# maropu/spark-data-repair-plugin

Hardware: AMD Instinct MI355X
Metric: repaired cells/sec (higher is better)
Workload: dtype f32 gradients (LightGBM's score_t), exact int64 fixed-point histogram sums, f64 scores

## Files before the change

### include/rgbm.h

```cpp
#ifndef RGBM_H_
#define RGBM_H_

#include <stddef.h>
#include <stdint.h>

#ifdef __cplusplus
extern "C" {
#endif

#define RGBM_OK 0
#define RGBM_ERR_ARG (-1)
#define RGBM_ERR_PARAM (-2)
#define RGBM_ERR_LABEL (-3)
#define RGBM_ERR_NO_DEVICE (-10)
#define RGBM_ERR_HIP (-11)
#define RGBM_ERR_NOMEM (-12)
#define RGBM_ERR_FORMAT (-20)

#define RGBM_OBJ_BINARY 0
#define RGBM_OBJ_MULTICLASS 1
#define RGBM_OBJ_REGRESSION 2

typedef struct rgbm_model rgbm_model;
typedef struct rgbm_table rgbm_table;
// ... 35 lines not shown
    int64_t level_atomics_per_row;
} rgbm_train_stats;

int rgbm_device_count(void);
int rgbm_release_cache(void);
const char* rgbm_last_error(void);
int rgbm_version(void);

int rgbm_train(const int32_t* X_colmajor, int64_t n, int32_t f, const int32_t* n_codes,
               const int32_t* y_code, int32_t n_y_codes, const double* y_value,
               const double* class_weight, const double* sample_weight,
               const rgbm_params* p, rgbm_model** out, rgbm_train_stats* stats );

int rgbm_predict(const rgbm_model* m, const int32_t* X_colmajor, int64_t n, int32_t f,
                 int32_t device_id, double* out);

int rgbm_repair_chain(const rgbm_model* const* models, int32_t T, const int32_t* target_col,
                      const int32_t* feat_cols, const int32_t* feat_off,
                      const int32_t* class_code, const int32_t* class_off,
                      int32_t* table_colmajor, int64_t n, int32_t c, int32_t device_id,
                      int32_t* out_label, double* out_prob);

int rgbm_table_create(const int32_t* codes_colmajor, int64_t n, int32_t c, const int32_t* n_codes,
                      int32_t device_id, rgbm_table** out);
int rgbm_table_set_column_kind(rgbm_table* t, int32_t col, int32_t kind);
int rgbm_table_set_column_values(rgbm_table* t, int32_t col, const double* values, int32_t n);
int rgbm_host_alloc(size_t bytes, void** out);
void rgbm_host_free(void* p);
void rgbm_table_free(rgbm_table* t);
int rgbm_table_train(const rgbm_table* t, int32_t target_col, const int32_t* feat_cols, int32_t f,
                     const double* y_value ,
                     const double* class_weight ,
                     const rgbm_params* p, rgbm_model** out, rgbm_train_stats* stats);
int rgbm_table_set_row_multiplicity(rgbm_table* t, const uint8_t* mult );
int rgbm_table_read_row_multiplicity(const rgbm_table* t, uint8_t* mult_out );
int rgbm_table_distinct_rows(const rgbm_table* t, rgbm_table** out, int64_t* n_out, int64_t* inverse_out );
int rgbm_table_distinct_view_info(const rgbm_table* t, int32_t* state, int64_t* rows, int64_t* builds);
int rgbm_distinct_view_eligible(int64_t rows, int32_t f, const rgbm_params* p, int32_t table_has_mult, int64_t min_rows);
typedef struct {
    const rgbm_table* table;
    int32_t target_col, n_features;
    const int32_t* feat_cols;
    const double* y_value;
    const double* class_weight;
    const rgbm_params* params;
    const rgbm_table* valid_table;
    int32_t* valid_label_out;
    double* valid_value_out;
} rgbm_fit_spec;
int rgbm_table_train_batch(const rgbm_fit_spec* fits, int32_t n_fits, rgbm_model** out_models , int32_t* out_status );
int rgbm_table_repair_chain(rgbm_table* t, const rgbm_model* const* models, int32_t T,
                            const int32_t* target_col, const int32_t* feat_cols, const int32_t* feat_off,
                            int64_t row_begin, int64_t n_rows, int32_t* out_label, double* out_prob);
int rgbm_table_read_column(const rgbm_table* t, int32_t col, int32_t* out );

int rgbm_table_detect_nulls(rgbm_table* t, const int32_t* cols, int32_t n_cols, int64_t* n_cells_out);
int rgbm_table_detect_cells(rgbm_table* t, const int32_t* cols, int32_t n_cols, const uint8_t* null_is_error ,
                            const int32_t* keep_lo, const int32_t* keep_hi ,
                            const uint64_t* const* flag_bits , int64_t* n_cells_out);
int rgbm_table_detect_constraint(rgbm_table* t, const int32_t* eq_cols, int32_t n_eq, int32_t iq_col,
                                 const int32_t* cell_cols, int32_t n_cell_cols,
                                 int64_t* n_rows_out , int64_t* n_cells_out);
#define RGBM_DC_EQ 0
#define RGBM_DC_IQ 1
#define RGBM_DC_LT 2
#define RGBM_DC_GT 3
typedef struct rgbm_dc_pred {
    int32_t op;
    int32_t left_col;
    int32_t right_col;
    int32_t reserved;
    const int32_t* left_rank;
    const int32_t* right_rank;
} rgbm_dc_pred;
int rgbm_table_detect_dc(rgbm_table* t, const rgbm_dc_pred* preds, int32_t n_preds, const int32_t* cell_cols, int32_t n_cell_cols,
                         int64_t max_pairs, int64_t* n_rows_out , int64_t* n_cells_out);
int rgbm_table_detect_row_bits(rgbm_table* t, const int32_t* cols, int32_t n_cols, const uint64_t* const* bits ,
                               const int32_t* cell_cols, int32_t n_cell_cols, int64_t* n_rows_out , int64_t* n_cells_out);
int rgbm_table_rows_of_cells(rgbm_table* t, const int64_t* rows, int64_t n_cells, int64_t* n_rows_out);
int rgbm_table_cells_fetch(const rgbm_table* t, int64_t* rows_out , int32_t* cols_out );
int rgbm_table_null_cells(rgbm_table* t, const int64_t* rows, const int32_t* cols, int64_t n_cells,
                          const int32_t* target_cols, int32_t n_targets);
int rgbm_table_read_cells(const rgbm_table* t, const int64_t* rows, const int32_t* cols, int64_t n_cells, int32_t* codes_out);
int rgbm_table_write_cells(rgbm_table* t, const int64_t* rows, const int32_t* cols, const int32_t* codes, int64_t n_cells);
int rgbm_table_gather_rows(const rgbm_table* t, const int64_t* rows, int64_t n_rows, rgbm_table** out);
int rgbm_table_count_codes(const rgbm_table* t, int32_t col, int64_t* counts_out ,
                           int64_t* n_null_out );
int rgbm_table_column_stats(const rgbm_table* t, const int32_t* cols, int32_t n_cols, const int32_t* const* len_lut,
                            int32_t n_bins, int64_t* stats_out, int32_t* edges_out);
int rgbm_table_create_dict(const int32_t* idx_colmajor, int64_t n, int32_t c, const int32_t* const* remap,
                           const int32_t* dict_size , int32_t device_id, rgbm_table** out);
int rgbm_table_repair_pmf(rgbm_table* t, const rgbm_model* m, int32_t target_col, const int32_t* feat_cols, int32_t f,
                          int32_t top_k, double threshold, const int32_t* cur_code, int64_t cap, int64_t* n_cells_out,
                          int64_t* rows_out , int32_t* class_out ,
                          double* prob_out , double* cur_prob_out );
int rgbm_table_repair_pmf_weighted(rgbm_table* t, const rgbm_model* m, int32_t target_col, const int32_t* feat_cols, int32_t f,
                                   int32_t top_k, double threshold, const int32_t* cur_code ,
                                   const int32_t* cost_row , const double* cost ,
                                   int64_t n_cost_rows, double weight, int32_t renormalise, int64_t cap, int64_t* n_cells_out,
                                   int64_t* rows_out , int32_t* class_out , double* prob_out ,
                                   double* cur_prob_out , double* top1_cost_out );
int rgbm_edit_distance(int32_t device_id, const int32_t* a_cp, const int64_t* a_off, int64_t n_a, const int32_t* b_cp,
                       const int64_t* b_off, int64_t n_b, int32_t* dist_out);
int rgbm_table_pair_counts(rgbm_table* t, const int32_t* pair_cols, int32_t n_pairs, const int32_t* const* luts ,
                           const int32_t* n_bins , int64_t* counts_out);
int rgbm_table_cell_domains(rgbm_table* t, int32_t target_col, const int64_t* rows, int64_t n_cells, const int32_t* pair_idx, int32_t k,
                            const int64_t* min_cnt , const uint8_t* single_ok , double beta, int64_t row_count,
                            uint8_t* weak_out, int32_t* top_out, double* top_prob_out, double* probs_out );
int rgbm_table_fd_map(const rgbm_table* t, int32_t x_col, int32_t y_col, int32_t* map_out );
int rgbm_table_rule_fill(rgbm_table* t, int32_t y_col, int32_t x_col , const int32_t* lut, int32_t n_lut, int64_t row_begin,
                         int64_t n_rows, int32_t* out_label );
int rgbm_nearest_values(int32_t device_id, const int32_t* a_cp, const int64_t* a_off, int64_t n_a, const int32_t* b_cp, const int64_t* b_off,
                        int64_t n_b, const double* cost , double threshold, int32_t* nearest_out );
int rgbm_lof_1d(int32_t device_id, const double* values , const int64_t* counts ,
                int32_t d, int32_t k , double threshold ,
                double* score_out , uint64_t* flag_bits_out , int64_t* info_out );
int rgbm_table_kmeans_assign(rgbm_table* t, const int32_t* cols, int32_t n_cols, const int64_t* code_off ,
                             int32_t k, const double* p , int64_t d_tot, const double* h ,
                             int32_t first ,
                             int64_t* counts_out , int64_t* sizes_out , int64_t* n_changed_out);
int rgbm_table_kmeans_read(const rgbm_table* t, int32_t* assign_out );
int rgbm_table_shape(const rgbm_table* t, int64_t* n_out, int32_t* c_out, int32_t* n_codes_out );

#define RGBM_COMM_ID_BYTES 128
#define RGBM_FLAG_ROW_SHARDED 1
#define RGBM_FLAG_WHOLE_TABLE 4
#define RGBM_FLAG_NO_MODEL 2
int rgbm_comm_unique_id(void* id_out );
int rgbm_comm_init(const void* id, int32_t rank, int32_t nranks, int32_t device_id);
int rgbm_comm_finalize(void);
int rgbm_comm_info(int32_t* info );
int rgbm_comm_count(int32_t* n_out );
int rgbm_comm_all_gather_sizes(const int64_t* mine, int32_t n, int64_t* all );
int rgbm_comm_all_gather_bytes(const void* send, int64_t my_bytes, int64_t block_bytes , void* recv );
int rgbm_table_repair_chain_gather(rgbm_table* t, const rgbm_model* const* models, int32_t T, const int32_t* target_col,
                                   const int32_t* feat_cols, const int32_t* feat_off, int64_t row_begin, int64_t n_rows, int64_t max_rows,
                                   int32_t* out_label, double* out_prob);
int rgbm_comm_gather_stats(int64_t* out );
int rgbm_local_group_create(int32_t nranks, int32_t device_id, void** group_out);
void rgbm_local_group_free(void* group);
int rgbm_comm_init_local(void* group, int32_t rank);

int rgbm_fusion_create(int32_t n_members, void** fusion_out);
int rgbm_fusion_join(void* fusion, int32_t member );
int rgbm_fusion_leave(int32_t failed );
int rgbm_fusion_info(void* fusion, int64_t* info );
int rgbm_fusion_free(void* fusion);

int rgbm_model_save(const rgbm_model* m, void* buf, size_t* len);
int rgbm_model_load(const void* buf, size_t len, rgbm_model** out);
void rgbm_model_free(rgbm_model* m);
int rgbm_model_info(const rgbm_model* m, int32_t* info);
int rgbm_model_predict_form(const rgbm_model* m, int32_t* out);
int rgbm_model_importance(const rgbm_model* m, int32_t type, double* out );

#ifdef __cplusplus
}
#endif
#endif
```

### spark-data-repair-plugin_amd/csrc/rgbm.hip

```cpp
#include <hip/hip_runtime.h>
#include <algorithm>
#include <atomic>
#include <condition_variable>
#include <chrono>
#include <cmath>
#include <cstdio>
#include <cstdlib>
#include <cstring>
#include <deque>
#include <map>
#include <memory>
#include <stdexcept>
#include <mutex>
#include <string>
#include <thread>
#include <vector>

#include "rgbm_host.h"
#include "rgbm_kernels.h"
#include "rgbm_level.h"
#include "rgbm_small.h"


namespace {
// ... 239 lines not shown
        const std::vector<double>* cv = (size_t)cols[f] < tab.col_values.size() ? &tab.col_values[cols[f]] : nullptr;
        find_bin(cnt.data() + cnt_off[f], ncod[f], n_train, p, ft, (cv && (int32_t)cv->size() == ncod[f] && ncod[f] > 0) ? cv->data() : nullptr);
        if ((size_t)cols[f] < tab.col_kind.size() && tab.col_kind[cols[f]] == 1) {
            const unsigned int* cf = cnt.data() + cnt_off[f];
            bool any = false;
            for (int32_t c = 0; c < ncod[f]; ++c) any |= cf[c] == 0;
            if (any) {
                ft.unseen.assign((size_t)(ncod[f] + 31) / 32, 0u);
                for (int32_t c = 0; c < ncod[f]; ++c) if (cf[c] == 0) ft.unseen[(size_t)c >> 5] |= 1u << (c & 31);
            }
        }
        fmeta[f].V = ft.V; fmeta[f].has_nan = ft.has_nan; fmeta[f].nbins = std::max(ft.V + ft.has_nan, 1); fmeta[f].hoff = totbins;
        totbins += fmeta[f].nbins;
        trivial[f] = (ft.V + ft.has_nan <= 1) || ft.V == 0;
        miss[f] = (uint8_t)(ft.has_nan ? ft.V : 0);
        lut_off[f + 1] = lut_off[f] + std::max(ncod[f], 1);
    }
    std::vector<uint8_t>& lut = h.lut; lut.assign(lut_off[F], 0);
    for (int f = 0; f < F; ++f) {
        const Feat& ft = model->feats[f];
        int b = 0;
        for (int c = 0; c < ncod[f]; ++c) { while (b < ft.V - 1 && c > ft.ub[b]) ++b; lut[lut_off[f] + c] = (uint8_t)(ft.V > 0 ? b : 0); }
    }
    const int nchunk = (F + 15) / 16; h.nchunk = nchunk;
    std::vector<ChunkMeta>& cmeta = h.cmeta; cmeta.assign(nchunk, ChunkMeta());
    size_t& lds_hist = h.lds_hist; lds_hist = 0;
    for (int ch = 0; ch < nchunk; ++ch) {
        ChunkMeta& cm = cmeta[ch]; cm.first_feat = ch * 16; cm.nfeat = std::min(16, F - ch * 16); cm.fast_slots = 0; cm.wide_bins = 0;
        for (int j = 0; j < cm.nfeat; ++j) {
            FeatMeta& m = fmeta[ch * 16 + j];
            int sh = 0; while (sh < 5 && (m.nbins << (sh + 1)) <= 256) ++sh;
            m.rep_shift = sh; m.fast_base = cm.fast_slots; m.wide_off = cm.wide_bins;
            cm.fast_slots += m.nbins << sh; cm.wide_bins += m.nbins;
        }
        lds_hist = std::max(lds_hist, (size_t)cm.fast_slots * 16);
    }

    const int nl = std::max({n_y, obj == 0 ? 2 : 1, obj == 1 ? K : 1});
    std::vector<double> tot(nl, 0.0);
    double w_max = 0.0;
    if (hls && hls->valid) { tot = hls->tot; tot.resize(nl, 0.0); w_max = hls->w_max; }
    else {
        for (int c = 0; c < n_y; ++c) {
            const double cw32 = class_weight ? (double)(float)class_weight[c] : 1.0;
            tot[c] = (double)ycnt[c] * cw32;
            if (ycnt[c]) w_max = std::max(w_max, cw32);
        }
    }
    if (!(w_max > 0.0)) w_max = 1.0;
    double sumw = 0.0;
    for (int c = 0; c < nl; ++c) sumw += tot[c];
    std::vector<double>& init = h.init; init.assign(K, 0.0);
    double ymin = 0.0, ymax = 0.0;
    const double keps = k_eps();
    if (obj == 2) {
        bool first = true; double suml = 0.0;
        for (int c = 0; c < n_y; ++c) {
            if (!ycnt[c]) continue;
            if (first) { ymin = ymax = y_value[c]; first = false; }
            ymin = std::min(ymin, y_value[c]); ymax = std::max(ymax, y_value[c]);
        }
        if (hls && hls->valid) suml = hls->suml; else for (int c = 0; c < nl; ++c) suml += tot[c] * (c < n_y ? y_value[c] : 0.0);
        init[0] = suml / sumw;
    } else if (obj == 0) {
        double pavg = tot[1] / sumw;
        if (pavg > 1.0 - keps) pavg = 1.0 - keps;
        if (pavg < keps) pavg = keps;
        init[0] = std::log(pavg / (1.0 - pavg));
    } else {
        for (int k = 0; k < K; ++k) { double pr = tot[k] / sumw; init[k] = std::log(pr > keps ? pr : keps); }
    }
    const double factor = obj == 1 ? (double)K / (double)(K - 1) : 1.0;
    double bound_g, bound_h;
    if (obj == 2) { bound_g = (ymax - ymin) * w_max; if (!(bound_g > 0.0)) bound_g = 1.0; bound_h = w_max; }
    else if (obj == 0) { bound_g = w_max; bound_h = 0.25 * w_max; }
    else { bound_g = w_max; bound_h = factor * 0.25 * w_max; }
    double wr = sumw / w_max;
    long long q_mult = 1;
    if (const char* th = std::getenv("RGBM_TEST_HOOKS")) if (std::atoi(th) != 0) if (const char* ev = std::getenv("RGBM_FX_ROWS")) {
        const double R = std::atof(ev);
        if (R > (double)n_train && R <= 4294967296.0 && n_train > 0) {
            wr *= R / (double)n_train; q_mult = ((long long)R + n_train - 1) / n_train;
            static std::atomic<bool> said{false};
            if (!said.exchange(true)) fprintf(stderr, "[rgbm] TEST HOOK active: RGBM_FX_ROWS=%s coarsens the fixed-point grid of every model trained by this process\n", ev);
        }
    }
    const int e_g = rg::fx_exponent(bound_g, wr), e_h = rg::fx_exponent(bound_h, wr);

    TrainConst& tc = h.tc; memset(&tc, 0, sizeof(tc));
    tc.sg = std::ldexp(1.0, e_g); tc.sh = std::ldexp(1.0, e_h); tc.inv_sg = std::ldexp(1.0, -e_g); tc.inv_sh = std::ldexp(1.0, -e_h);
    tc.l1 = p.lambda_l1; tc.l2 = p.lambda_l2; tc.min_gain_to_split = p.min_gain_to_split; tc.min_sum_hessian = p.min_sum_hessian_in_leaf;
    tc.learning_rate = p.learning_rate; tc.factor = factor; tc.min_data_in_leaf = p.min_data_in_leaf; tc.max_depth = p.max_depth;
    tc.num_leaves = p.num_leaves; tc.F = F; tc.K = K; tc.totbins = std::max(totbins, 1); tc.nchunk = nchunk; tc.objective = obj;
    tc.N = N; tc.n_train = n_train; tc.NG = N;
    tc.fx.c_g = 24 - rg::fx_ceil_log2(bound_g); tc.fx.c_h = 24 - rg::fx_ceil_log2(bound_h);
    tc.fx.e_g_min = e_g; tc.fx.e_h_min = e_h;
    tc.fx.e_g_max = 50 - rg::fx_ceil_log2(bound_g); tc.fx.e_h_max = 50 - rg::fx_ceil_log2(bound_h);
    tc.fx.q_mult = q_mult;
}

struct HostTrees { const int32_t *L, *feat, *theta, *dleft, *left, *right, *cnt; const double *gain, *val; const int32_t* any; };
size_t model_trees_begin(rgbm_model* model, const HostTrees& h, int NE, int K) {
    int n_iter = NE;
    for (int it = 0; it < NE; ++it) if (!h.any[it]) { n_iter = it > 0 ? it : 1; break; }
    model->n_iter = n_iter;
    const size_t nt = (size_t)n_iter * K;
    model->trees.clear(); model->trees.resize(nt);
    size_t total = 0;
    for (size_t t = 0; t < nt; ++t) total += Tree::doubles(std::max(h.L[t], 1));
    model->tree_arena.reset(new double[std::max<size_t>(total, 1)]);
    size_t off = 0;
    for (size_t t = 0; t < nt; ++t) { const int L = std::max(h.L[t], 1); model->trees[t].place(model->tree_arena.get() + off, L); off += Tree::doubles(L); }
    return nt;
}
void model_trees_fill(rgbm_model* model, const HostTrees& h, int NL, size_t t0, size_t t1) {
    for (size_t t = t0; t < t1; ++t) {
        Tree& tr = model->trees[t];
        const size_t n = (size_t)tr.L - 1, nb = t * (NL - 1), lb = t * NL;
        memcpy(tr.feat, h.feat + nb, 4 * n); memcpy(tr.theta, h.theta + nb, 4 * n); memcpy(tr.dleft, h.dleft + nb, 4 * n);
        memcpy(tr.left, h.left + nb, 4 * n); memcpy(tr.right, h.right + nb, 4 * n); memcpy(tr.gain, h.gain + nb, 8 * n);
        memcpy(tr.leaf_value, h.val + lb, 8 * (size_t)tr.L); memcpy(tr.leaf_count, h.cnt + lb, 4 * (size_t)tr.L);
    }
}
void model_from_trees(rgbm_model* model, const HostTrees& h, int NE, int K, int NL) {
    const size_t n = model_trees_begin(model, h, NE, K);
    model_trees_fill(model, h, NL, 0, n);
}

std::vector<uint8_t> make_used_masks(const rgbm_params& p, size_t NT, int F, const std::vector<uint8_t>& trivial) {
    std::vector<uint8_t> used(NT * F, 0);
    LgbRand sr((uint32_t)p.seed);
    sr.rnd16(); sr.rnd16(); sr.rnd16();
    LgbRand ff((uint32_t)sr.rnd16());
    std::vector<int> valid; for (int f = 0; f < F; ++f) if (!trivial[f]) valid.push_back(f);
    for (size_t t = 0; t < NT; ++t) {
        uint8_t* u = used.data() + t * F;
        if (p.feature_fraction < 1.0) {
            int cntf = (int)std::floor((double)valid.size() * p.feature_fraction + 0.5);
            if (cntf < 1) cntf = 1;
            for (int i : ff.sample((int)valid.size(), cntf)) u[valid[i]] = 1;
        } else for (int f : valid) u[f] = 1;
    }
    return used;
}

struct MtLaunch { int ch, slot0, nslots, route, T, G, gx, acc2, rot; };
struct LevelPassPlan {
    int root_gx = 8;
    std::vector<std::vector<MtLaunch>> mt;
    std::vector<int> mt_gx;
    size_t part_items = 0;
};

LevelPassPlan plan_level_passes(const RunSwitches& sw, const std::vector<rg::FeatMeta>& fmeta, const std::vector<rg::ChunkMeta>& cmeta,
                                long long N, int K, int max_depth, bool wm , int lds_bytes) {
    using namespace rg;
    const int nchunk = (int)cmeta.size();
    LevelPassPlan P;
    P.mt.resize(LV_MAX_DEPTH + 1); P.mt_gx.assign(LV_MAX_DEPTH + 1, 8);
    const long long ntiles = (N + LV_TILE - 1) / LV_TILE;
    {
        const long long cu_slots = 256, per = (long long)K * nchunk;
        const long long gmin = std::max<long long>(1, (N + (1ll << 22) - 1) >> 22);
        auto eff_of = [&](long long g) { const long long tot = g * per, rounds = (tot + cu_slots - 1) / cu_slots; return (double)tot / (double)(rounds * cu_slots); };
        const long long gfloor = std::max<long long>(8, (gmin + 7) / 8 * 8), gcap = std::max<long long>(gfloor, std::min<long long>(512, (ntiles + 7) / 8 * 8));
        long long g2 = gfloor; double best2 = -1.0;
        for (long long g = gfloor; g <= gcap; g += 8) {
            if (per >= 16 && (g * per < 3 * cu_slots || g * per > 5 * cu_slots)) continue;
            const double e = eff_of(g);
            if (e > best2 + 1e-9) { best2 = e; g2 = g; }
            if (e >= 0.99) break;
        }
        if (best2 < 0.0) for (long long g = gfloor; g <= gcap; g += 8) { const double e = eff_of(g); if (e > best2 + 1e-9) { best2 = e; g2 = g; } if (e >= 0.99) break; }
        if (sw.lv_blocks >= 1) g2 = (sw.lv_blocks + 7) / 8 * 8;
        P.root_gx = (int)g2;
    }
    for (int ch = 0; ch < nchunk; ++ch)
        if ((long long)lv_slots(fmeta.data() + cmeta[ch].first_feat, cmeta[ch].nfeat, 0) * 16 + LV_ROOT_FIXED > lds_bytes)
            throw std::invalid_argument("histogram of one node exceeds LDS");
    P.part_items = (size_t)K * P.root_gx;
    for (int level = 1; level < max_depth; ++level) {
        const int worst = 1 << (level - 1);
        int G_first = 1;
        bool acc2 = nchunk == 2 && sw.mt_acc2;
        if (acc2) {
            const long long nb2 = ((long long)lv_slots(fmeta.data() + cmeta[0].first_feat, cmeta[0].nfeat, 0) + lv_slots(fmeta.data() + cmeta[1].first_feat, cmeta[1].nfeat, 0)) * 16;
            if (nb2 > mt_hist_bytes(lds_bytes, MT_THREADS_ACC2, true, true, cmeta[1].nfeat > 15 || wm)) acc2 = false;
        }
        if (wm && nchunk == 2 && !acc2) throw std::invalid_argument("a two-chunk table with row multiplicities needs the one-pass level form (the multiplicity rides in the second record)");
        for (int ch = 0; ch < (acc2 ? 1 : nchunk); ++ch) {
            const FeatMeta* fm = fmeta.data() + cmeta[ch].first_feat;
            long long node_bytes = (long long)lv_slots(fm, cmeta[ch].nfeat, 0) * 16;
            if (acc2) node_bytes += (long long)lv_slots(fmeta.data() + cmeta[1].first_feat, cmeta[1].nfeat, 0) * 16;
            const int mt_thr = acc2 ? MT_THREADS_ACC2 : LV_THREADS;
            const bool li_arr = cmeta[acc2 ? 1 : ch].nfeat > 15 || wm;
            const long long hist_room = mt_hist_bytes(lds_bytes, mt_thr, acc2, acc2 , li_arr);
            long long cap = hist_room / std::max<long long>(node_bytes, 1);
            cap = std::min<long long>(cap, MT_MAX_NODES);
            if (cap < 1) throw std::invalid_argument("histogram of one node exceeds LDS");
            const int win = (int)std::min<long long>(worst, cap);
            const long long rep_target = std::max(1, sw.mt_rep);
            const long long t_nodes = std::max<long long>(win, cap / rep_target);
            int T = (int)std::max<long long>(1, std::min<long long>(std::min<long long>(t_nodes / win, MT_MAX_T), std::min<long long>(K, MT_RT_BUDGET / (2 * worst))));
            if (sw.mt_T >= 1) T = std::max(1, std::min(T, sw.mt_T));
            const bool plain1 = nchunk == 1 || acc2;
            const bool rot_full = cmeta[ch].nfeat >= 12 && (!acc2 || cmeta[1].nfeat >= 12);
            const long long rot_node_bytes = node_bytes + mt_rot_dummy(true) * 16;
            const long long cap_rot = std::min<long long>(hist_room / rot_node_bytes, MT_MAX_NODES);
            const long long T_rot = std::min<long long>(std::min<long long>(cap_rot / win, MT_MAX_T), std::min<long long>(K, MT_RT_BUDGET / (2 * worst)));
            const bool few_trees = T < sw.mt_rot_tmin && T_rot >= 2 * (long long)T;
            const bool rot = plain1 && (sw.mt_rot == 1 || (sw.mt_rot < 0 && rot_full && (cap * 2 < (long long)sw.mt_rot_copies2 * T * win || few_trees))) &&
                             (long long)T * win * rot_node_bytes <= hist_room;
            if (rot && sw.mt_T < 1) T = (int)std::max<long long>(T, T_rot);
            const int G = (K + T - 1) / T;
            if (ch == 0) G_first = G;
            for (int s0 = 0; s0 < worst; s0 += win)
                P.mt[level].push_back(MtLaunch{ch, s0, win, (ch == 0 && s0 == 0) ? 1 : 0, T, G, 0, acc2 ? 1 : 0, rot ? 1 : 0});
        }
        const long long gmin = std::max<long long>(1, (N + (1ll << 22) - 1) >> 22);
        const long long nwt = (N + MT_WT_ROWS - 1) / MT_WT_ROWS;
        const long long gx_lo = std::max<long long>(8, (gmin + 7) / 8 * 8), gx_hi = std::max<long long>(gx_lo, std::min<long long>(512, (nwt / (4 * (LV_THREADS / 64)) + 7) / 8 * 8));
        long long gx = gx_lo; double best = -1.0;
        for (long long g = gx_lo; g <= gx_hi; g += 8) {
            const long long tot = g * G_first, rounds = (tot + 255) / 256;
            const double eff = (double)tot / (double)(rounds * 256) - 0.01 * (double)rounds;
            if (eff > best + 1e-9) { best = eff; gx = g; }
            if (tot >= 256 && (double)tot / (double)(rounds * 256) >= 0.97) break;
        }
        if (sw.mt_blocks >= 1) gx = (sw.mt_blocks + 7) / 8 * 8;
        P.mt_gx[level] = (int)gx;
        for (auto& L : P.mt[level]) L.gx = (int)gx;
        P.part_items = std::max(P.part_items, (size_t)K * (size_t)gx * (size_t)worst);
    }
    return P;
}

struct JointRootPlan {
    bool on = false;
    std::vector<std::vector<int>> groups;
    std::vector<rg::FeatMeta> vfm; rg::ChunkMeta vcm;
    std::vector<rg::JointFeat> jf;
    std::vector<int16_t> binfeat;
};
JointRootPlan plan_joint_root(const std::vector<rg::FeatMeta>& fmeta, int totbins, bool wm, int lds_bytes) {
    using namespace rg;
    const int F = (int)fmeta.size();
    JointRootPlan J;
    std::vector<int> order(F); for (int f = 0; f < F; ++f) order[f] = f;
    std::stable_sort(order.begin(), order.end(), [&](int a, int b) { return fmeta[a].nbins > fmeta[b].nbins; });
    std::vector<int> prod;
    for (int f : order) {
        int best = -1;
        for (size_t g = 0; g < J.groups.size(); ++g)
            if ((long long)prod[g] * fmeta[f].nbins <= 256 && (best < 0 || prod[g] > prod[best])) best = (int)g;
        if (best < 0) { J.groups.emplace_back(); prod.push_back(1); best = (int)J.groups.size() - 1; }
        J.groups[best].push_back(f); prod[best] *= fmeta[f].nbins;
    }
    const int VF = (int)J.groups.size();
    if (VF > (wm ? 15 : 16) || VF > F - 2) return J;
    J.vfm.resize(VF); J.jf.resize(F); J.binfeat.assign(totbins, 0);
    ChunkMeta& vcm = J.vcm; vcm.first_feat = 0; vcm.nfeat = VF; vcm.fast_slots = 0; vcm.wide_bins = 0;
    for (int v = 0; v < VF; ++v) {
        FeatMeta& m = J.vfm[v]; memset(&m, 0, sizeof(m));
        m.V = prod[v]; m.has_nan = 0; m.nbins = prod[v]; m.hoff = vcm.wide_bins; m.wide_off = vcm.wide_bins;
        int sh = 0; while (sh < 5 && (m.nbins << (sh + 1)) <= 256) ++sh;
        m.rep_shift = sh; m.fast_base = vcm.fast_slots; vcm.fast_slots += m.nbins << sh; vcm.wide_bins += m.nbins;
        int stride = 1;
        for (int f : J.groups[v]) {
            JointFeat& j = J.jf[f]; memset(&j, 0, sizeof(j));
            j.voff = m.hoff; j.stride = stride; j.nbins = fmeta[f].nbins; j.nbv = prod[v]; j.hoff = fmeta[f].hoff; j.vbyte = v;
            stride *= fmeta[f].nbins;
            for (int b = 0; b < fmeta[f].nbins; ++b) J.binfeat[fmeta[f].hoff + b] = (int16_t)f;
        }
    }
    J.on = (long long)lv_slots(J.vfm.data(), VF, 0) * 16 + LV_ROOT_FIXED <= lds_bytes;
    return J;
}

#define RGBM_MT_FORMS(X) \
    X(0, rg::LV_THREADS, false, false, false)  \
    X(1, rg::LV_THREADS, false, false, false)  \
    X(1, rg::LV_THREADS, false, false, true)   \
    X(2, rg::LV_THREADS, false, false, false)  \
    X(2, rg::MT_THREADS_ACC2, true, true, false)  \
    X(2, rg::MT_THREADS_ACC2, true, true, true)
struct MtForm { int nchr, threads; bool acc2, spec, rot; };
constexpr MtForm MT_FORMS[] = {
#define RGBM_MT_FORM_ENTRY(NCHR, THR, ACC, SPEC, ROT) {NCHR, THR, ACC, SPEC, ROT},
    RGBM_MT_FORMS(RGBM_MT_FORM_ENTRY)
#undef RGBM_MT_FORM_ENTRY
};
using MtKernel = decltype(&rg::k_level_mt<1, false, true, rg::LV_THREADS, false, false, false>);
MtKernel mt_kernel(const MtForm& f, bool bag, bool route) {
#define RGBM_MT_FORM_KERNEL(NCHR, THR, ACC, SPEC, ROT) \
    if (f.nchr == NCHR && f.threads == THR && f.acc2 == ACC && f.spec == SPEC && f.rot == ROT) \
        return bag ? (route ? rg::k_level_mt<NCHR, true, true, THR, ACC, SPEC, ROT> : rg::k_level_mt<NCHR, true, false, THR, ACC, SPEC, ROT>) \
                   : (route ? rg::k_level_mt<NCHR, false, true, THR, ACC, SPEC, ROT> : rg::k_level_mt<NCHR, false, false, THR, ACC, SPEC, ROT>);
    RGBM_MT_FORMS(RGBM_MT_FORM_KERNEL)
#undef RGBM_MT_FORM_KERNEL
    throw std::logic_error("level pass: no such launch form");
}
void launch_level_mt(const MtForm& f, bool bag, bool route, dim3 grid, hipStream_t s, const uint4* rec, const float2* gh, uint8_t* node, const uint8_t* inbag,
                     const rg::LvPlan* plan, rg::HistBin* part, int32_t* count, const rg::FeatMeta* fmeta, const rg::ChunkMeta* cmeta, int32_t* err_flag,
                     const rg::FxScale* fxs, const rg::LevelConst& c) {
    hipLaunchKernelGGL(mt_kernel(f, bag, route), grid, dim3(f.threads), rg::LV_LDS_BYTES, s, rec, gh, node, inbag, plan, part, count, fmeta, cmeta, err_flag, fxs, c);
}
struct HistTimers {
    bool on; hipStream_t s;
    std::deque<rgh::Event> ev; std::vector<char> root;
    template <typename Fn> void timed(bool is_root, Fn&& fn) {
        if (!on) { fn(); return; }
        HIPCHK(hipEventRecord(ev.emplace_back().e, s));
        fn();
        HIPCHK(hipEventRecord(ev.emplace_back().e, s));
        root.push_back(is_root ? 1 : 0);
    }
};

struct LevelTrace {
    struct Rec { std::string name; int it, level; size_t off, bytes; };
    const char* dir; bool on; hipStream_t s;
    int lo = 44, hi = 44, cur_it = 0;
    std::vector<Rec> idx; size_t used = 0;
    DevBuf<unsigned char> buf;
    LevelTrace(bool level_mode, int K, hipStream_t stream) : dir(getenv("RGBM_TRACE")), s(stream) {
        on = dir && level_mode && (!getenv("RGBM_TRACE_K") || atoi(getenv("RGBM_TRACE_K")) == K);
        if (on && getenv("RGBM_TRACE_ITERS")) sscanf(getenv("RGBM_TRACE_ITERS"), "%d:%d", &lo, &hi);
    }
    void copy(const char* name, int level, const void* src, size_t bytes) {
        if (!on || cur_it < lo || cur_it > hi) return;
        if (used + bytes > buf.n) return;
        HIPCHK(hipMemcpyAsync(buf.p + used, src, bytes, hipMemcpyDeviceToDevice, s));
        idx.push_back({name, cur_it, level, used, bytes}); used += (bytes + 15) & ~(size_t)15;
    }
    void sum(const char* name, const void* src, size_t bytes) {
        if (!on || used + 16 > buf.n) return;
        HIPCHK(hipMemsetAsync(buf.p + used, 0, 8, s));
        rgh::trace_sum(src, bytes, (unsigned long long*)(buf.p + used), s);
        idx.push_back({name, cur_it, -1, used, 8}); used += 16;
    }
    void write(int target_col) {
        if (!on || !used) return;
        std::vector<unsigned char> h(used);
        HIPCHK(hipMemcpy(h.data(), buf.p, used, hipMemcpyDeviceToHost));
        char path[512];
        snprintf(path, sizeof(path), "%s/target%d.bin", dir, target_col);
        if (FILE* f = fopen(path, "wb")) { fwrite(h.data(), 1, h.size(), f); fclose(f); }
        snprintf(path, sizeof(path), "%s/target%d.idx", dir, target_col);
        if (FILE* f = fopen(path, "w")) { for (const auto& r : idx) fprintf(f, "%s %d %d %zu %zu\n", r.name.c_str(), r.it, r.level, r.off, r.bytes); fclose(f); }
    }
};

void fill_train_stats(rgbm_train_stats* stats, float total_ms, const HistTimers& timers, const HostTrees& h, const rgbm_params& p, bool level_mode, bool use_bagging,
                      int nranks , int64_t N, int64_t n_train, int F, int root_feats ,
                      int K, unsigned long long statrows) {
    const int NE = p.n_estimators, NL = p.num_leaves;
    memset(stats, 0, sizeof(*stats));
    stats->total_ms = total_ms;
    stats->hist_launches = (int64_t)timers.root.size();
    for (size_t i = 0; i < timers.root.size(); ++i) {
        float m2 = 0.f; HIPCHK(hipEventElapsedTime(&m2, timers.ev[2 * i].e, timers.ev[2 * i + 1].e));
        stats->hist_ms += m2; if (timers.root[i]) stats->root_ms += m2;
    }
    stats->trees = (int64_t)NE * K;
    const bool root_done = n_train >= (int64_t)p.min_data_in_leaf * 2;
    if (level_mode) {
        const int64_t root_rows = (root_done && !use_bagging) ? (int64_t)NE * K * n_train : 0;
        const int64_t rows_acc = (int64_t)(statrows / (unsigned long long)nranks);
        stats->hist_rows = rows_acc; stats->root_rows = root_rows / nranks;
        stats->root_atomics_per_row = 2 * (int64_t)root_feats; stats->level_atomics_per_row = 2 * (int64_t)F;
        stats->hist_bytes = rows_acc * ((int64_t)F + 8);
        return;
    }
    int64_t rows = 0, root_rows = 0;
    for (size_t t = 0; t < (size_t)NE * K; ++t) {
        const int L = h.L[t];
        const int32_t* left = h.left + t * (NL - 1); const int32_t* right = h.right + t * (NL - 1);
        if (root_done) { rows += N; root_rows += N; }
        std::vector<int64_t> fin(h.cnt + t * NL, h.cnt + t * NL + NL);
        std::vector<int64_t> nodecnt(std::max(L - 1, 1), 0);
        auto sub = [&](int ch) -> int64_t { return ch < 0 ? fin[~ch] : nodecnt[ch]; };
        for (int j = L - 2; j >= 0; --j) nodecnt[j] = sub(left[j]) + sub(right[j]);
        std::vector<int> node_depth(std::max(L - 1, 1), 0);
        for (int j = 0; j < L - 1; ++j) {
            const int lc = left[j], rc = right[j];
            if (lc >= 0) node_depth[lc] = node_depth[j] + 1;
            if (rc >= 0) node_depth[rc] = node_depth[j] + 1;
            const int64_t a = sub(lc), b = sub(rc);
            bool go = j + 2 < NL;
            if (p.max_depth > 0 && node_depth[j] + 1 >= p.max_depth) go = false;
            if (a < (int64_t)p.min_data_in_leaf * 2 && b < (int64_t)p.min_data_in_leaf * 2) go = false;
            if (go) rows += std::min(a, b);
        }
    }
    stats->hist_rows = rows; stats->root_rows = root_rows;
    stats->hist_bytes = rows * ((int64_t)F + 8) + (rows - root_rows) * 4;
}

void check_fit_args(const rgbm_table& tab, int32_t target_col, const int32_t* feat_cols, int32_t F, const double* y_value, const rgbm_params& p) {
    check_params(p);
    if (F <= 0) throw std::invalid_argument("no feature columns");
    if (target_col < 0 || target_col >= tab.c) throw std::invalid_argument("target column out of range");
    for (int f = 0; f < F; ++f) if (feat_cols[f] < 0 || feat_cols[f] >= tab.c) throw std::invalid_argument("feature column out of range");
    const int obj = p.objective, n_y = tab.n_codes[target_col];
    if (obj == 1 && n_y > p.num_class) throw std::out_of_range("target has more label codes than num_class");
    if (obj == 0 && n_y > 2) throw std::out_of_range("binary objective with more than 2 label codes");
    if (obj == 2 && !y_value) throw std::out_of_range("regression needs the y_value dictionary");
}

struct BinRecords {
    DevBuf<int32_t> cols, ncod; DevBuf<long long> cnt_off; DevBuf<unsigned int> cnt;
    DevBuf<rg::FeatMeta> fmeta; DevBuf<rg::ChunkMeta> cmeta; DevBuf<long long> lut_off; DevBuf<uint8_t> lut, miss; DevBuf<uint4> rec;
    void count_codes(const rgbm_table& tab, int32_t target_col, const int32_t* feat_cols, int32_t F, FitHost& h, hipStream_t s) {
        h.cols.assign(feat_cols, feat_cols + F); h.cols.push_back(target_col);
        h.ncod.resize(F + 1); h.cnt_off.assign(F + 2, 0);
        for (int f = 0; f <= F; ++f) { h.ncod[f] = tab.n_codes[h.cols[f]]; h.cnt_off[f + 1] = h.cnt_off[f] + std::max(h.ncod[f], 1); }
        cols.alloc(F + 1); ncod.alloc(F + 1); cnt_off.alloc(F + 2); cnt.alloc(h.cnt_off[F + 1]);
        cols.upload(h.cols.data(), F + 1, s); ncod.upload(h.ncod.data(), F + 1, s); cnt_off.upload(h.cnt_off.data(), F + 2, s); cnt.zero(s);
        const int gx = (int)std::min<int64_t>((tab.n + 255) / 256, 1024);
        hipLaunchKernelGGL(rg::k_count_codes, dim3(gx, F + 1), dim3(256), 0, s, tab.codes.p, (long long)tab.n, tab.codes.p + (long long)target_col * tab.n, cols.p, ncod.p,
                           cnt_off.p, cnt.p, tab.has_mult ? tab.mult.p : (const uint8_t*)nullptr);
    }
    void download_counts(FitHost& h, hipStream_t s) const { h.cnt.resize(cnt.n); cnt.download(h.cnt.data(), cnt.n, s); }
    void fill(const FitHost& h, long long N, hipStream_t s) {
        const int F = h.tc.F;
        fmeta.alloc(F); cmeta.alloc(h.nchunk); lut_off.alloc(F + 1); lut.alloc(h.lut.size()); miss.alloc(F);
        fmeta.upload(h.fmeta.data(), F, s); cmeta.upload(h.cmeta.data(), h.nchunk, s); lut_off.upload(h.lut_off.data(), F + 1, s);
        lut.upload(h.lut.data(), h.lut.size(), s); miss.upload(h.miss.data(), F, s);
        rec.alloc((size_t)h.nchunk * N);
    }
    void pack(const rgbm_table& t, const uint8_t* lut_, const uint8_t* miss_, uint4* out, const uint8_t* mult, hipStream_t s) const {
        hipLaunchKernelGGL(rg::k_pack_bins, dim3((unsigned)((t.n + 255) / 256)), dim3(256), 0, s, t.codes.p, (long long)t.n, 0ll, (long long)t.n, cols.p, ncod.p,
                           lut_off.p, lut_, miss_, (int)fmeta.n, (int)cmeta.n, out, mult);
    }
    void pack(const rgbm_table& tab, hipStream_t s) { pack(tab, lut.p, miss.p, rec.p, tab.has_mult ? tab.mult.p : (const uint8_t*)nullptr, s); }
};

struct BagState {
    DevBuf<unsigned int> blk, rand, bagcnt; DevBuf<int32_t> sorted_rows, oob; DevBuf<uint8_t> inbag;
    std::vector<unsigned int> seeds;
    long long off = 0, local = 0, nrb = 1;
    void order_rows(const int32_t* d_ycol, long long N, long long n_train, hipStream_t s) {
        const long long nblk = (N + 1023) / 1024;
        blk.alloc(nblk); sorted_rows.alloc(n_train); oob.alloc(n_train); inbag.alloc(N); bagcnt.alloc(2);
        hipLaunchKernelGGL(rg::k_block_count, dim3((unsigned)nblk), dim3(256), 0, s, d_ycol, N, blk.p);
        hipLaunchKernelGGL(rg::k_block_scan, dim3(1), dim3(1024), 0, s, blk.p, nblk);
        hipLaunchKernelGGL(rg::k_stable_compact, dim3((unsigned)nblk), dim3(256), 0, s, d_ycol, N, blk.p, sorted_rows.p);
    }
    void seed(const rgbm_params& p, long long bag_off, long long bag_local, hipStream_t s) {
        off = bag_off; local = bag_local;
        nrb = std::max<long long>(1, (off + local + 1023) / 1024 - off / 1024);
        LgbRand sr2((uint32_t)p.seed); sr2.rnd16();
        const int bagging_seed = sr2.rnd16();
        seeds.resize(nrb);
        for (long long b = 0; b < nrb; ++b) seeds[b] = (unsigned int)(bagging_seed + off / 1024 + b);
        rand.alloc(nrb); rand.upload(seeds.data(), nrb, s);
    }
};

struct TreeBlock {
    DevBuf<int32_t> L, feat, theta, dleft, left, right, cnt, any; DevBuf<double> gain, val;
    void alloc(size_t NT, int NL, int NE, hipStream_t s) {
        const size_t nn = NT * (size_t)(NL - 1), nl = NT * (size_t)NL;
        any.alloc(NE); any.zero(s);
        L.alloc(NT); feat.alloc(nn); theta.alloc(nn); dleft.alloc(nn); left.alloc(nn); right.alloc(nn); cnt.alloc(nl); gain.alloc(nn); val.alloc(nl);
        cnt.zero(s); val.zero(s);
    }
    rg::TreeOut out() const { return rg::TreeOut{L.p, feat.p, theta.p, dleft.p, left.p, right.p, gain.p, val.p, cnt.p}; }
    void host_layout(size_t (&off)[11]) const {
        const size_t bytes[10] = {L.n * 4, feat.n * 4, theta.n * 4, dleft.n * 4, left.n * 4, right.n * 4, cnt.n * 4, gain.n * 8, val.n * 8, any.n * 4};
        off[0] = 0;
        for (int i = 0; i < 10; ++i) off[i + 1] = off[i] + ((bytes[i] + 63) & ~(size_t)63);
    }
    size_t host_bytes() const { size_t off[11]; host_layout(off); return off[10]; }
    HostTrees download(char* base, hipStream_t s) const {
        size_t off[11]; host_layout(off);
        auto get = [&](const auto& buf, int i) { auto* h = reinterpret_cast<decltype(buf.p)>(base + off[i]); buf.download(h, buf.n, s); return h; };
        return HostTrees{get(L, 0), get(feat, 1), get(theta, 2), get(dleft, 3), get(left, 4), get(right, 5), get(cnt, 6), get(gain, 7), get(val, 8), get(any, 9)};
    }
};

struct FitState {
    const rgbm_table& tab; const rgbm_params& p; hipStream_t s; const int32_t F;
    const RunSwitches sw = read_switches();
    const int K = p.objective == 1 ? p.num_class : 1, NL = p.num_leaves, NE = p.n_estimators; const int64_t N = tab.n;
    const bool use_bagging = p.bagging_freq > 0 && p.bagging_fraction < 1.0;
    const bool level_mode = p.max_depth >= 1 && p.max_depth <= rg::LV_MAX_DEPTH && F <= 255 && sw.grower != 2;
    const bool dp = (p.reserved & RGBM_FLAG_ROW_SHARDED) != 0;
    const int32_t* d_ycol; const uint8_t* d_mult = tab.has_mult ? tab.mult.p : (const uint8_t*)nullptr;
    FitHost h; BinRecords bins;
    DevBuf<int32_t> base;
    DevBuf<unsigned int> counter;
    DevBuf<float2> gh;
    DevBuf<double> score, init;
    DevBuf<unsigned long long> fxq;
    DevBuf<rg::FxScale> fxs;
    DevBuf<unsigned long long> qpart; long long fx_parts = 0; bool fx_fused = false;
    TreeBlock trees;
    DevBuf<double> cw, yv, sw_rows; DevBuf<uint8_t> used;
    BagState bag; DevBuf<unsigned int> bagcnt_g;
    const unsigned int* n_in_ptr = nullptr;
    DevBuf<int32_t> it;
    HistTimers timers;

    FitState(const rgbm_table& tab_, int32_t target_col, int32_t F_, const rgbm_params& p_, bool timed, hipStream_t s_)
        : tab(tab_), p(p_), s(s_), F(F_), d_ycol(tab_.codes.p + (long long)target_col * tab_.n), timers{timed, s_} {}

    int grad_gx() const { return (int)std::min<long long>((N + 255) / 256, 4096); }
    bool mc_tile() const { return p.objective == 1 && K >= 16 && K <= 112; }
    bool mc_rows() const { return p.objective == 1 && K < 16; }
    void alloc_fx_parts() {
        if (sw.fx_separate || (p.objective == 1 && !mc_tile() && !mc_rows())) return;
        fx_fused = true; fx_parts = mc_tile() ? (N + 63) / 64 : (mc_rows() ? ((N + 255) / 256) * 4 : (long long)grad_gx());
        qpart.alloc((size_t)fx_parts * K * 2);
    }
    void enqueue_grad(uint8_t* node0, long long NS);
    void enqueue_bagging();
};

struct LevelGrower {
    FitState& st; hipStream_t s;
    int root_feats;
    unsigned long long statrows = 0;
    rg::LevelConst lc, lcj; LevelPassPlan passes;
    const int n_hnodes = (1 << st.p.max_depth) - 1;
    bool use_reduce = false;
    bool joint_root = false; int vtotbins = 0;
    DevBuf<rg::FeatMeta> vfmeta; DevBuf<rg::ChunkMeta> vcmeta; DevBuf<uint4> rec_j; DevBuf<rg::HistBin> part_j, red_j; DevBuf<rg::JointFeat> jf; DevBuf<int16_t> binfeat;
    DevBuf<uint8_t> node; DevBuf<rg::LvPlan> plan; DevBuf<rg::SNode> snodes; DevBuf<rg::Cand> lcand;
    DevBuf<rg::HistBin> part, lpool, part_red; DevBuf<int32_t> count, count_g, err, leafnode; DevBuf<double> ndelta; DevBuf<unsigned long long> d_statrows;
    const int score_gx = (int)std::max<long long>(1, std::min<long long>((st.N + 1023) / 1024, (2048 + st.K - 1) / st.K));
    LevelTrace trace;
    int32_t h_err = 0;

    explicit LevelGrower(FitState& st_) : st(st_), s(st_.s), root_feats(st_.F), trace(true, st_.K, st_.s) {
        using namespace rg;
        memset(&lc, 0, sizeof(lc)); memset(&lcj, 0, sizeof(lcj));
        lc.lds_bytes = LV_LDS_BYTES;
        if (st.sw.lv_lds >= 65536 && st.sw.lv_lds <= LV_LDS_BYTES) lc.lds_bytes = st.sw.lv_lds;
        lc.nchunk = st.h.nchunk; lc.K = st.K; lc.F = st.F; lc.totbins = st.h.tc.totbins;
        lc.num_leaves = st.NL; lc.max_depth = st.p.max_depth; lc.min_data_in_leaf = st.p.min_data_in_leaf; lc.N = st.N; lc.NS = (st.N + 255) & ~255ll; lc.NG = lc.NS;
        lc.sib_local = (st.dp && comm_rank() == 0) ? 1 : 0;
        lc.has_mult = st.tab.has_mult ? 1u : 0u;
        passes = plan_level_passes(st.sw, st.h.fmeta, st.h.cmeta, st.N, st.K, st.p.max_depth, st.tab.has_mult, lc.lds_bytes);
        lc.gx = passes.root_gx; lc.xcd_blocks = 1; lc.max_built = 1;
        node.alloc((size_t)st.K * lc.NS);
        HIPCHK(hipMemsetAsync(node.p, 0xFF, (size_t)st.K * lc.NS, s));
        plan.alloc(st.K); snodes.alloc((size_t)st.K * 256); lcand.alloc((size_t)st.K * 256 * st.F);
        part.alloc(passes.part_items * st.h.tc.totbins); lpool.alloc((size_t)st.K * n_hnodes * st.h.tc.totbins);
        count.alloc((size_t)st.K * 256); use_reduce = st.dp || lc.gx > 4;
        if (st.dp) count_g.alloc((size_t)st.K * 256);
        const int max_built_all = 1 << std::max(0, st.p.max_depth - 2);
        part_red.alloc((size_t)st.K * max_built_all * st.h.tc.totbins + (size_t)st.K * 128 );
        leafnode.alloc((size_t)st.K * LV_MAX_LEAVES); err.alloc(1); err.zero(s); ndelta.alloc((size_t)st.K * 256); d_statrows.alloc(1); d_statrows.zero(s);
        if (st.sw.joint_root && ((long long)st.K * st.N >= (1ll << 21) || (st.tab.has_mult && st.h.nchunk == 2))) {
            const JointRootPlan jp = plan_joint_root(st.h.fmeta, st.h.tc.totbins, st.tab.has_mult, lc.lds_bytes);
            if (jp.on) {
                const int VF = (int)jp.vfm.size();
                joint_root = true; vtotbins = jp.vcm.wide_bins;
                vfmeta.alloc(VF); vfmeta.upload(jp.vfm.data(), VF, s); vcmeta.alloc(1); vcmeta.upload(&jp.vcm, 1, s);
                jf.alloc(st.F); jf.upload(jp.jf.data(), st.F, s); binfeat.alloc(jp.binfeat.size()); binfeat.upload(jp.binfeat.data(), jp.binfeat.size(), s);
                rec_j.alloc((size_t)st.N);
                hipLaunchKernelGGL(k_pack_joint, dim3((unsigned)((st.N + 255) / 256)), dim3(256), 0, s, st.bins.rec.p, (long long)st.N, st.F, jf.p, rec_j.p, st.tab.has_mult ? st.h.nchunk - 1 : -1);
                part_j.alloc((size_t)st.K * lc.gx * vtotbins); red_j.alloc((size_t)st.K * vtotbins + (size_t)st.K * 128 );
                lcj = lc; lcj.nchunk = 1; lcj.F = VF; lcj.totbins = vtotbins; lcj.max_built = 1;
                use_reduce = true; root_feats = VF;
                HIPCHK(hipStreamSynchronize(s));
            }
        }
        if (st.tab.has_mult && st.h.nchunk == 2 && !joint_root)
            throw std::invalid_argument("a two-chunk table with row multiplicities needs the joint-bin root pass (its record carries the multiplicity); this feature set does not pack into 15 groups");
        if (st.sw.timing) {
            fprintf(stderr, "[rgbm] root: gx %d joint %d groups %d\n", lc.gx, joint_root ? 1 : 0, joint_root ? lcj.F : 0);
            for (int level = 1; level < st.p.max_depth; ++level) for (const auto& L : passes.mt[level])
                fprintf(stderr, "[rgbm] level %d launch: chunk %d slots %d..%d route %d T %d G %d gx %d acc2 %d rot %d\n", level, L.ch, L.slot0, L.slot0 + L.nslots - 1, L.route, L.T, L.G, L.gx, L.acc2, L.rot);
        }
        rgh::once_per_device(st.tab.device, rgh::ONCE_LEVEL_LDS, [] {
            HIPCHK(hipFuncSetAttribute((const void*)rg::k_level_root, hipFuncAttributeMaxDynamicSharedMemorySize, rg::LV_LDS_BYTES));
            for (const MtForm& f : MT_FORMS) for (int bag = 0; bag < 2; ++bag) for (int route = 0; route < 2; ++route)
                HIPCHK(hipFuncSetAttribute((const void*)mt_kernel(f, bag != 0, route != 0), hipFuncAttributeMaxDynamicSharedMemorySize, rg::LV_LDS_BYTES));
        });
        if (trace.on) trace.buf.alloc(((size_t)st.K * n_hnodes * st.h.tc.totbins * 16 + (size_t)st.K * 256 * (sizeof(SNode) + 4) + (size_t)st.K * sizeof(LvPlan) + 4096) * (size_t)(st.p.max_depth + 1) * (size_t)(trace.hi - trace.lo + 1) + (size_t)st.NE * 64 + 4096);
    }

    void trace_level(int level) {
        trace.copy("count", level, count.p, (size_t)st.K * 256 * 4);
        trace.copy("plan", level, plan.p, (size_t)st.K * sizeof(rg::LvPlan));
        trace.copy("snodes", level, snodes.p, (size_t)st.K * 256 * sizeof(rg::SNode));
        trace.copy("lpool", level, lpool.p, (size_t)st.K * n_hnodes * st.h.tc.totbins * 16);
    }
    std::pair<const rg::HistBin*, rg::LevelConst> exchange(bool root, int nb, const rg::LevelConst& lp) {
        using namespace rg;
        if (root && !use_reduce) return {part.p, lp};
        if (root && joint_root) {
            hipLaunchKernelGGL(k_level_reduce, dim3((vtotbins + 63) / 64, 1, st.K), dim3(256), 0, s, part_j.p, red_j.p, plan.p, count.p, 1, 1, lcj);
            hipLaunchKernelGGL(k_level_marginal, dim3((st.h.tc.totbins + 255) / 256, st.K), dim3(256), 0, s, red_j.p, part_red.p, plan.p, count.p, jf.p, binfeat.p, vtotbins, lc);
        } else
            hipLaunchKernelGGL(k_level_reduce, dim3((st.h.tc.totbins + 63) / 64, nb, st.K), dim3(256), 0, s, part.p, part_red.p, plan.p, count.p, root ? 1 : 0, nb, lp);
        if (st.dp) {
            const size_t nh = (size_t)st.K * nb * st.h.tc.totbins * 2;
            all_reduce(part_red.p, nh + (size_t)st.K * 256, AR_I64, s);
            hipLaunchKernelGGL(k_counts_unpack, dim3(st.K), dim3(256), 0, s, reinterpret_cast<const long long*>(part_red.p) + nh, count_g.p);
        }
        LevelConst r = lp; r.gx = 1; r.max_built = nb;
        return {part_red.p, r};
    }
    void enqueue_iteration(int it) {
        using namespace rg;
        const TreeOut to = st.trees.out();
        trace.cur_it = it;
        trace.sum("gh", st.gh.p, (size_t)st.K * st.h.tc.NG * 8);
        hipLaunchKernelGGL(k_level_init, dim3(st.K), dim3(64), 0, s, plan.p, snodes.p, count.p, st.n_in_ptr, (long long)st.h.n_train, st.fxq.p, st.h.tc.fx, st.fxs.p, lc);
        int32_t* cntg = st.dp ? count_g.p : count.p;
        st.timers.timed(true, [&]() {
            if (joint_root)
                hipLaunchKernelGGL(k_level_root, dim3((unsigned)lc.gx * (unsigned)st.K, 1, 1), dim3(LV_THREADS), lc.lds_bytes, s, rec_j.p, st.gh.p, node.p, plan.p, part_j.p,
                                   vfmeta.p, vcmeta.p, st.fxs.p, lcj);
            else
                hipLaunchKernelGGL(k_level_root, dim3((unsigned)lc.gx * (unsigned)st.K, 1, st.h.nchunk), dim3(LV_THREADS), lc.lds_bytes, s, st.bins.rec.p, st.gh.p, node.p, plan.p, part.p,
                                   st.bins.fmeta.p, st.bins.cmeta.p, st.fxs.p, lc);
        });
        {
            auto ex = exchange(true, 1, lc);
            hipLaunchKernelGGL(k_level_split<true>, dim3((st.F + 3) / 4, 1, st.K), dim3(256), 0, s, ex.first, lpool.p, plan.p, snodes.p, cntg, count.p, st.bins.fmeta.p,
                               st.used.p, lcand.p, d_statrows.p, st.it.p, n_hnodes, st.fxs.p, st.h.tc, ex.second);
            trace_level(0);
        }
        for (int level = 1; level < st.p.max_depth; ++level) {
            hipLaunchKernelGGL(k_level_plan, dim3(st.K), dim3(256), 0, s, plan.p, snodes.p, lcand.p, st.bins.fmeta.p, level, st.h.tc, lc);
            LevelConst lp = lc;
            lp.xcd_blocks = 0; lp.gx = passes.mt_gx[level]; lp.max_built = 1 << (level - 1);
            for (const MtLaunch& L : passes.mt[level]) {
                LevelConst l1 = lp;
                l1.mt_T = L.T; l1.mt_G = L.G; l1.mt_ch = L.ch; l1.mt_slot0 = L.slot0; l1.mt_nslots = L.nslots; l1.mt_route = L.route; l1.mt_sparse = st.sw.mt_sparse ? 1 : 0;
                const bool acc2 = L.acc2 != 0;
                const MtForm form{acc2 ? 2 : (st.h.nchunk <= 2 ? st.h.nchunk : 0), acc2 ? MT_THREADS_ACC2 : LV_THREADS, acc2, acc2, L.rot != 0};
                st.timers.timed(false, [&]() {
                    launch_level_mt(form, st.use_bagging, L.route != 0, dim3((unsigned)L.G * (unsigned)L.gx), s, st.bins.rec.p, st.gh.p, node.p, st.bag.inbag.p,
                                    plan.p, part.p, count.p, st.bins.fmeta.p, st.bins.cmeta.p, err.p, st.fxs.p, l1);
                });
            }
            auto ex = exchange(false, 1 << (level - 1), lp);
            hipLaunchKernelGGL(k_level_split<false>, dim3((st.F + 1) / 2, 1 << (level - 1), st.K), dim3(256), 0, s, ex.first, lpool.p, plan.p, snodes.p,
                               cntg, count.p, st.bins.fmeta.p, st.used.p, lcand.p, d_statrows.p, st.it.p, n_hnodes, st.fxs.p, st.h.tc, ex.second);
            trace_level(level);
        }
        hipLaunchKernelGGL(k_level_plan, dim3(st.K), dim3(256), 0, s, plan.p, snodes.p, lcand.p, st.bins.fmeta.p, st.p.max_depth, st.h.tc, lc);
        hipLaunchKernelGGL(k_level_replay, dim3(st.K), dim3(64), 0, s, plan.p, snodes.p, cntg, to, st.init.p, ndelta.p, leafnode.p, st.trees.any.p, err.p, st.it.p, st.h.tc);
        hipLaunchKernelGGL(k_level_final, dim3(score_gx, st.K), dim3(256), 0, s, st.bins.rec.p, node.p, st.bag.inbag.p, plan.p, to, ndelta.p, st.score.p, count.p, st.it.p, lc);
        if (st.dp) { hipLaunchKernelGGL(k_copy_i32, dim3(st.K), dim3(256), 0, s, count.p, count_g.p, (long long)st.K * 256); all_reduce(count_g.p, (size_t)st.K * 256, AR_I32, s); }
        hipLaunchKernelGGL(k_level_leafcount, dim3(st.K), dim3(LV_MAX_LEAVES), 0, s, plan.p, cntg, leafnode.p, to, st.it.p, st.h.tc);
        trace_level(st.p.max_depth);
        trace.sum("score", st.score.p, (size_t)st.K * st.N * 8); trace.sum("node", node.p, (size_t)st.K * lc.NS);
        hipLaunchKernelGGL(k_next_iteration, dim3(1), dim3(1), 0, s, st.it.p);
    }
    void enqueue_report() { err.download(&h_err, 1, s); d_statrows.download(&statrows, 1, s); }
    void report(int32_t target_col) {
        trace.write(target_col);
        if (h_err & 2) throw std::runtime_error("level grower: a level pass was launched with more built nodes / route entries than its workgroup tables hold (sizing violated)");
        if (h_err) throw std::runtime_error("level grower: a node outside the speculative expansion was selected (expansion bound violated)");
    }
};

struct LeafwiseGrower {
    FitState& st; hipStream_t s;
    DevBuf<int32_t> idx0, idx1, sorted; DevBuf<rg::HistBin> pool; DevBuf<rg::TreeState> state; DevBuf<rg::Leaf> leaves; DevBuf<rg::Cand> cand; DevBuf<double> upd;
    const long long root_tiles = (st.N + rg::TILE_ROWS - 1) / rg::TILE_ROWS;
    const int hist_gx = (int)std::max<long long>(1, std::min<long long>(root_tiles, (1536 + (long long)st.K * st.h.nchunk - 1) / ((long long)st.K * st.h.nchunk)));
    const int part_gx = (int)std::max<long long>(1, std::min<long long>((st.h.n_train + 1023) / 1024, (1024 + st.K - 1) / st.K));
    const int upd_gx = (int)std::max<long long>(1, std::min<long long>((st.h.n_train + 255) / 256, (2048 + st.K - 1) / st.K));
    const size_t upd_lds = (size_t)(3 * st.NL + (st.NL & 1)) * 4 + (size_t)st.NL * 8;

    explicit LeafwiseGrower(FitState& st_) : st(st_), s(st_.s) {
        idx0.alloc((size_t)st.K * st.h.n_train); idx1.alloc((size_t)st.K * st.h.n_train);
        pool.alloc((size_t)st.K * st.NL * st.h.tc.totbins);
        state.alloc(st.K); leaves.alloc((size_t)st.K * st.NL); cand.alloc((size_t)st.K * 2 * st.F);
        upd.alloc((size_t)st.K * st.NL); sorted.alloc((size_t)st.K * st.NL * 3);
        if (st.h.lds_hist > 64 * 1024)
            rgh::once_per_device(st.tab.device, rgh::ONCE_HIST_LDS, [] { HIPCHK(hipFuncSetAttribute((const void*)rg::k_hist, hipFuncAttributeMaxDynamicSharedMemorySize, 160 * 1024)); });
        if (st.h.lds_hist > 160 * 1024) throw std::invalid_argument("histogram working set exceeds LDS");
    }
    void enqueue_iteration(int it) {
        using namespace rg;
        const TreeOut to = st.trees.out();
        const uint8_t* usedp = st.used.p + (size_t)it * st.K * st.F;
        hipLaunchKernelGGL(k_init_iter, dim3(st.K), dim3(64), 0, s, state.p, leaves.p, pool.p, to, st.n_in_ptr, it, st.h.tc);
        for (int step = 0; step < st.NL - 1; ++step) {
            st.timers.timed(step == 0, [&]() {
                hipLaunchKernelGGL(k_hist, dim3(hist_gx, st.K, st.h.nchunk), dim3(256), st.h.lds_hist, s, st.bins.rec.p, st.gh.p, idx0.p, idx1.p, st.base.p,
                                   state.p, pool.p, st.bins.fmeta.p, st.bins.cmeta.p, st.fxs.p, st.h.tc);
            });
            hipLaunchKernelGGL(k_split_find, dim3((st.F + 3) / 4, st.K), dim3(256), 0, s, pool.p, state.p, leaves.p, st.bins.fmeta.p, usedp, cand.p, st.fxs.p, st.h.tc);
            hipLaunchKernelGGL(k_tree_step, dim3(st.K), dim3(64), 0, s, state.p, leaves.p, cand.p, pool.p, st.bins.fmeta.p, to, it, st.h.tc);
            hipLaunchKernelGGL(k_partition, dim3(part_gx, st.K), dim3(256), 0, s, reinterpret_cast<const uint8_t*>(st.bins.rec.p), idx0.p, idx1.p, st.base.p, state.p, st.h.tc);
            hipLaunchKernelGGL(k_finish_split, dim3(st.K), dim3(64), 0, s, state.p, leaves.p, to, it, st.h.tc);
        }
        hipLaunchKernelGGL(k_finalize_tree, dim3(st.K), dim3(64), 0, s, state.p, leaves.p, to, st.init.p, upd.p, sorted.p, st.trees.any.p, it, st.h.tc);
        hipLaunchKernelGGL(k_score_update, dim3(upd_gx, st.K), dim3(256), upd_lds, s, state.p, leaves.p, sorted.p, upd.p, idx0.p, idx1.p, st.base.p, st.score.p, st.n_in_ptr, st.h.tc);
        if (st.use_bagging)
            hipLaunchKernelGGL(k_score_update_oob, dim3(upd_gx, st.K), dim3(256), 0, s, reinterpret_cast<const uint8_t*>(st.bins.rec.p), st.bag.oob.p, st.bag.bagcnt.p,
                               state.p, to, st.bins.fmeta.p, upd.p, st.score.p, it, st.h.tc);
    }
};

void FitState::enqueue_grad(uint8_t* node0, long long NS) {
    using namespace rg;
    if (p.objective == 0) hipLaunchKernelGGL(k_grad<0>, dim3(grad_gx()), dim3(256), 0, s, score.p, d_ycol, yv.p, cw.p, sw_rows.p, bag.inbag.p, gh.p, node0, NS, qpart.p, d_mult, h.tc);
    else if (mc_rows())
        hipLaunchKernelGGL(k_grad_mc_rows<256>, dim3((unsigned)((N + 255) / 256)), dim3(256), (size_t)K * 256 * 8, s, score.p, d_ycol, cw.p, sw_rows.p, bag.inbag.p, gh.p, node0, NS, qpart.p, d_mult, h.tc);
    else if (mc_tile())
        hipLaunchKernelGGL(k_grad_mc, dim3((unsigned)((N + 63) / 64)), dim3(256), (size_t)(K * 64 + 320) * 8, s, score.p, d_ycol, cw.p, sw_rows.p, bag.inbag.p, gh.p, node0, NS, qpart.p, d_mult, h.tc);
    else if (p.objective == 1) hipLaunchKernelGGL(k_grad<1>, dim3(grad_gx()), dim3(256), 0, s, score.p, d_ycol, yv.p, cw.p, sw_rows.p, bag.inbag.p, gh.p, node0, NS, (unsigned long long*)nullptr, d_mult, h.tc);
    else hipLaunchKernelGGL(k_grad<2>, dim3(grad_gx()), dim3(256), 0, s, score.p, d_ycol, yv.p, cw.p, sw_rows.p, bag.inbag.p, gh.p, node0, NS, qpart.p, d_mult, h.tc);
    if (fx_fused) {
        const long long total = fx_parts * K * 2;
        const unsigned gx = (unsigned)std::max<long long>(1, std::min<long long>(256, (total + 8191) / 8192));
        hipLaunchKernelGGL(k_fx_reduce, dim3(gx), dim3(256), (size_t)K * 2 * 8, s, qpart.p, fx_parts, 2 * K, fxq.p);
    } else {
        const unsigned gx = (unsigned)std::max<long long>(1, std::min<long long>(128, (N + 4095) / 4096));
        hipLaunchKernelGGL(k_fx_measure, dim3(gx, K), dim3(256), 0, s, gh.p, (long long)N, (long long)h.tc.NG, h.tc.fx, fxq.p, d_mult);
    }
    if (dp) all_reduce(fxq.p, (size_t)K * 2, AR_I64, s);
    if (!level_mode) hipLaunchKernelGGL(k_fx_scale, dim3(1), dim3(256), 0, s, fxq.p, K, h.tc.fx, fxs.p);
}
void FitState::enqueue_bagging() {
    using namespace rg;
    hipLaunchKernelGGL(k_bagging, dim3((unsigned)((bag.nrb + 63) / 64)), dim3(64), 0, s, bag.rand.p, bag.local, p.bagging_fraction, bag.sorted_rows.p, bag.inbag.p, bag.bagcnt.p,
                       bag.off, (long long)h.n_train);
    hipLaunchKernelGGL(k_bag_lists, dim3((unsigned)((std::max<long long>(bag.local, 1) + 255) / 256)), dim3(256), 0, s, bag.sorted_rows.p, bag.local, bag.inbag.p, base.p, bag.oob.p, bag.bagcnt.p);
    if (dp) {
        hipLaunchKernelGGL(k_copy_i32, dim3(1), dim3(256), 0, s, reinterpret_cast<const int32_t*>(bag.bagcnt.p), reinterpret_cast<int32_t*>(bagcnt_g.p), 2ll);
        all_reduce(bagcnt_g.p, 2, AR_U32, s);
    }
}

rgbm_model* train_core(const rgbm_table& tab, int32_t target_col, const int32_t* feat_cols, int32_t F,
                       const double* y_value, const double* class_weight, const double* sample_weight_host,
                       const HostLabelStats* hls, const rgbm_params& p, rgbm_train_stats* stats, bool view_stats = false) {
    using namespace rg;
    check_fit_args(tab, target_col, feat_cols, F, y_value, p);
    if (F > 65535) throw std::invalid_argument("more than 65535 feature columns");
    StreamGuard sg_; hipStream_t s = sg_.s;
    rgh::Event ev_begin, ev_end;
    HIPCHK(hipEventRecord(ev_begin.e, s));

    FitState st(tab, target_col, F, p, stats != nullptr, s);
    auto now = []() { return std::chrono::duration<double, std::milli>(std::chrono::steady_clock::now().time_since_epoch()).count(); };
    const double t_start = now();
    st.bins.count_codes(tab, target_col, feat_cols, F, st.h, s);
    if (st.dp) {
        if (comm_kind() == 0) throw std::invalid_argument("row-sharded training requested but this thread has no communicator (rgbm_comm_init)");
        all_reduce(st.bins.cnt.p, st.bins.cnt.n, AR_U32, s);
    }
    st.bins.download_counts(st.h, s);
    if (st.dp) stream_sync_watchdog(s); else HIPCHK(hipStreamSynchronize(s));
    fit_setup(tab, y_value, class_weight, hls, p, F, st.h);
    if (p.objective == 2) y_value = st.h.yv32.data();
    const int n_y = st.h.ncod[F];

    const double t_bins = now();
    st.bins.fill(st.h, st.N, s);
    if (tab.has_mult && (!st.level_mode || st.h.nchunk > 2 || (F % 16) == 0 || sample_weight_host || st.use_bagging))
        throw std::invalid_argument("a table with row multiplicities trains with the level grower (1 <= max_depth <= 7), at most 32 features of which the last 16-feature "
                                    "chunk holds at most 15, without bagging and without per-row weights");
    st.bins.pack(tab, s);
    if (st.dp && (!st.level_mode || sample_weight_host))
        throw std::invalid_argument("row-sharded training supports the level grower (1 <= max_depth <= 7) without per-row weights");
    st.counter.alloc(1); st.counter.zero(s);
    if (!st.level_mode || st.use_bagging) {
        st.base.alloc(st.h.n_train);
        hipLaunchKernelGGL(k_iota_train, dim3((unsigned)((st.N + 255) / 256)), dim3(256), 0, s, st.d_ycol, (long long)st.N, st.base.p, st.counter.p);
    }
    if (st.level_mode) st.h.tc.NG = (st.N + 255) & ~255ll;
    st.gh.alloc((size_t)st.K * st.h.tc.NG); st.gh.zero(s);
    st.score.alloc((size_t)st.K * st.N); st.init.alloc(st.K);
    st.init.upload(st.h.init.data(), st.K, s);
    st.fxq.alloc((size_t)st.K * 2); st.fxq.zero(s);
    st.fxs.alloc(st.K);
    hipLaunchKernelGGL(k_init_score, dim3((unsigned)((st.N + 255) / 256)), dim3(256), 0, s, st.score.p, (long long)st.N, st.K, st.init.p);
    const size_t NT = (size_t)st.NE * st.K;
    st.trees.alloc(NT, st.NL, st.NE, s);
    std::unique_ptr<LevelGrower> lg; std::unique_ptr<LeafwiseGrower> lw;
    if (st.level_mode) lg.reset(new LevelGrower(st)); else lw.reset(new LeafwiseGrower(st));
    if (class_weight) { st.cw.alloc(n_y); st.cw.upload(class_weight, n_y, s); }
    if (y_value) { st.yv.alloc(n_y); st.yv.upload(y_value, n_y, s); }
    if (sample_weight_host) { st.sw_rows.alloc(st.N); st.sw_rows.upload(sample_weight_host, st.N, s); }

// ... 884 lines not shown
        HIPCHK(hipMemcpy(table, codes.p, (size_t)n * c * sizeof(int32_t), hipMemcpyDeviceToHost));
        return RGBM_OK;
    });
}

RGBM_EXPORT int rgbm_table_set_row_multiplicity(rgbm_table* t, const uint8_t* mult) {
    if (!t) return fail(RGBM_ERR_ARG, "rgbm_table_set_row_multiplicity: bad argument");
    return guarded([&]() {
        use_device(t->device);
        rgh::ViewWrite view_wr(t);
        if (!mult) { t->has_mult = false; t->mult_total = 0; return RGBM_OK; }
        int64_t tot = 0;
        for (int64_t i = 0; i < t->n; ++i) { if (mult[i] == 0) throw std::invalid_argument("rgbm_table_set_row_multiplicity: a multiplicity of 0"); tot += mult[i]; }
        if (tot >= (1ll << 31) - 4096) throw std::invalid_argument("rgbm_table_set_row_multiplicity: the expanded table has more than 2^31 rows");
        StreamGuard sg;
        t->mult.alloc((size_t)t->n);
        t->mult.upload(mult, (size_t)t->n, sg.s);
        HIPCHK(hipStreamSynchronize(sg.s));
        t->has_mult = true; t->mult_total = tot;
        return RGBM_OK;
    });
}

RGBM_EXPORT int rgbm_table_repair_chain(rgbm_table* t, const rgbm_model* const* models, int32_t T, const int32_t* target_col,
                                        const int32_t* feat_cols, const int32_t* feat_off, int64_t row_begin, int64_t n_rows,
                                        int32_t* out_label, double* out_prob) {
    if (!t || !models || T < 0 || !target_col || !feat_cols || !feat_off || row_begin < 0 || n_rows < 0 || row_begin + n_rows > t->n)
        return fail(RGBM_ERR_ARG, "rgbm_table_repair_chain: bad argument");
    if (n_rows == 0 || T == 0) return RGBM_OK;
    return guarded([&]() {
        use_device(t->device);
        rgh::ViewWrite view_wr(t);
        StreamGuard sg;
        return chain_device(const_cast<rgbm_model* const*>(models), T, target_col, feat_cols, feat_off, nullptr, nullptr, t->codes.p, t->n, row_begin, n_rows,
                            t->device, sg.s, out_label, out_prob);
    });
}

RGBM_EXPORT int rgbm_model_save(const rgbm_model* m, void* buf, size_t* len) {
    if (!m || !len) return fail(RGBM_ERR_ARG, "rgbm_model_save: bad argument");
    return guarded([&]() {
        const size_t need = serialised_size(*m);
        if (!buf) { *len = need; return RGBM_OK; }
        if (*len < need) { *len = need; return fail(RGBM_ERR_ARG, "rgbm_model_save: buffer too small"); }
        serialise_into(*m, (uint8_t*)buf); *len = need;
        return RGBM_OK;
    });
}

RGBM_EXPORT int rgbm_model_load(const void* buf, size_t len, rgbm_model** out) {
    if (!buf || !out) return fail(RGBM_ERR_ARG, "rgbm_model_load: bad argument");
    return guarded([&]() {
        const uint8_t* p = (const uint8_t*)buf; const uint8_t* end = p + len;
        auto need = [&](size_t n) { if ((size_t)(end - p) < n) throw std::length_error("truncated model"); };
        try {
            need(28); int32_t hdr[7]; memcpy(hdr, p, 28); p += 28;
            if (hdr[0] != 0x4D424752 || (hdr[1] != 1 && hdr[1] != 2)) return fail(RGBM_ERR_FORMAT, "rgbm_model_load: bad magic/version");
            std::unique_ptr<rgbm_model> m(new rgbm_model());
            m->objective = hdr[2]; m->num_class = hdr[3]; m->K = hdr[4]; m->n_iter = hdr[5]; m->F = hdr[6];
            if (m->F < 0 || m->K < 1 || m->n_iter < 0 || m->F > 65535) return fail(RGBM_ERR_FORMAT, "rgbm_model_load: bad header");
            if (m->objective < 0 || m->objective > 2 || m->num_class < 1) return fail(RGBM_ERR_FORMAT, "rgbm_model_load: bad objective / num_class");
            if (m->objective == 1 ? m->K != m->num_class : m->K != 1) return fail(RGBM_ERR_FORMAT, "rgbm_model_load: class-tree count does not match the objective");
            if (m->objective == 0 && m->num_class != 2) return fail(RGBM_ERR_FORMAT, "rgbm_model_load: binary model with num_class != 2");
            if ((unsigned long long)m->n_iter * (unsigned long long)m->K > (unsigned long long)(end - p) / 16ull) return fail(RGBM_ERR_FORMAT, "rgbm_model_load: tree count exceeds the buffer");
            m->feats.resize(m->F);
            for (Feat& f : m->feats) {
                need(12); int32_t h3[3]; memcpy(h3, p, 12); p += 12;
                f.n_codes = h3[0]; f.V = h3[1]; f.has_nan = h3[2];
                if (f.V < 0 || f.V > 255) return fail(RGBM_ERR_FORMAT, "rgbm_model_load: bad bin count");
                need(4 * (size_t)f.V); f.ub.resize(f.V); memcpy(f.ub.data(), p, 4 * (size_t)f.V); p += 4 * (size_t)f.V;
                if (hdr[1] == 2) {
                    need(4); int32_t nw; memcpy(&nw, p, 4); p += 4;
                    if (nw < 0 || (nw != 0 && (f.n_codes < 0 || nw != (f.n_codes + 31) / 32))) return fail(RGBM_ERR_FORMAT, "rgbm_model_load: bad unseen-category bitmap");
                    need(4 * (size_t)nw); f.unseen.resize(nw); memcpy(f.unseen.data(), p, 4 * (size_t)nw); p += 4 * (size_t)nw;
                }
            }
            m->trees.resize((size_t)m->n_iter * m->K);
            std::vector<uint8_t> refs;
            for (Tree& t : m->trees) {
                int32_t L_; need(4); memcpy(&L_, p, 4); p += 4;
                if (L_ < 1 || L_ > 32767) return fail(RGBM_ERR_FORMAT, "rgbm_model_load: bad leaf count");
                const size_t n = (size_t)L_ - 1;
                need(n * 28 + (size_t)L_ * 12);
                t.alloc(L_);
                auto rd32 = [&](int32_t* v, size_t k) { memcpy(v, p, 4 * k); p += 4 * k; };
                auto rd64 = [&](double* v, size_t k) { memcpy(v, p, 8 * k); p += 8 * k; };
                rd32(t.feat, n); rd32(t.theta, n); rd32(t.dleft, n); rd32(t.left, n); rd32(t.right, n); rd64(t.gain, n);
                rd64(t.leaf_value, t.L); rd32(t.leaf_count, t.L);
                for (size_t j = 0; j < n; ++j) {
                    if (t.feat[j] < 0 || t.feat[j] >= m->F) return fail(RGBM_ERR_FORMAT, "rgbm_model_load: node feature out of range");
                    if (t.theta[j] < -1 || t.theta[j] > 254) return fail(RGBM_ERR_FORMAT, "rgbm_model_load: node threshold out of range");
                    auto okc = [&](int ch) { return ch < 0 ? (~ch) < t.L : ch < (int)n && ch > (int)j; };
                    if (!okc(t.left[j]) || !okc(t.right[j])) return fail(RGBM_ERR_FORMAT, "rgbm_model_load: bad child link");
                }
                refs.assign(n + (size_t)t.L, 0);
                bool tree_ok = true;
                for (size_t j = 0; j < n; ++j)
                    for (int ch : {t.left[j], t.right[j]}) if (++refs[ch < 0 ? n + (size_t)(~ch) : (size_t)ch] > 1) tree_ok = false;
                for (size_t j = 1; j < refs.size(); ++j) if (refs[j] != 1) tree_ok = false;
                if (!tree_ok) return fail(RGBM_ERR_FORMAT, "rgbm_model_load: child links do not form a tree");
            }
            *out = m.release();
            return RGBM_OK;
        } catch (const std::length_error&) { return fail(RGBM_ERR_FORMAT, "rgbm_model_load: truncated buffer"); }
    });
}

RGBM_EXPORT int rgbm_table_repair_chain_gather(rgbm_table* t, const rgbm_model* const* models, int32_t T, const int32_t* target_col,
                                               const int32_t* feat_cols, const int32_t* feat_off, int64_t row_begin, int64_t n_rows, int64_t max_rows,
                                               int32_t* out_label, double* out_prob) {
    if (!t || !models || T < 1 || !target_col || !feat_cols || !feat_off || row_begin < 0 || n_rows < 0 || row_begin + n_rows > t->n || max_rows < n_rows || max_rows < 1 || !out_label || !out_prob)
        return fail(RGBM_ERR_ARG, "rgbm_table_repair_chain_gather: bad argument");
    return guarded([&]() {
        use_device(t->device);
        rgh::ViewWrite view_wr(t);
        const int nr = std::max(1, comm_nranks());
        StreamGuard sg; hipStream_t s = sg.s;
        const size_t blk = (size_t)T * (size_t)max_rows;
        DevBuf<int32_t> d_lab(blk), d_lab_all(blk * (size_t)nr); DevBuf<double> d_prob(blk), d_prob_all(blk * (size_t)nr);
        d_lab.zero(s); d_prob.zero(s);
        if (n_rows > 0)
            chain_device(const_cast<rgbm_model* const*>(models), T, target_col, feat_cols, feat_off, nullptr, nullptr, t->codes.p, t->n, row_begin, n_rows,
                         t->device, s, nullptr, nullptr, d_lab.p, d_prob.p, (long long)max_rows);
        const auto t0 = std::chrono::steady_clock::now();
        all_gather_on(d_lab.p, d_lab_all.p, blk * sizeof(int32_t), s);
        all_gather_on(d_prob.p, d_prob_all.p, blk * sizeof(double), s);
        HIPCHK(hipMemcpyAsync(out_label, d_lab_all.p, blk * (size_t)nr * sizeof(int32_t), hipMemcpyDeviceToHost, s));
        HIPCHK(hipMemcpyAsync(out_prob, d_prob_all.p, blk * (size_t)nr * sizeof(double), hipMemcpyDeviceToHost, s));
        stream_sync_watchdog(s);
        rgh::GatherStats& G = rgh::gather_stats();
        G.bytes += (long long)(blk * (size_t)nr * 12); G.calls += 2;
        G.ns += std::chrono::duration_cast<std::chrono::nanoseconds>(std::chrono::steady_clock::now() - t0).count();
        return RGBM_OK;
    });
}

RGBM_EXPORT void rgbm_model_free(rgbm_model* m) { delete m; }

RGBM_EXPORT int rgbm_model_info(const rgbm_model* m, int32_t* info) {
    if (!m || !info) return fail(RGBM_ERR_ARG, "rgbm_model_info: bad argument");
    info[0] = m->objective; info[1] = m->num_class; info[2] = m->K; info[3] = m->n_iter; info[4] = m->F;
    return RGBM_OK;
}

RGBM_EXPORT int rgbm_model_predict_form(const rgbm_model* m, int32_t* out) {
    if (!m || !out) return fail(RGBM_ERR_ARG, "rgbm_model_predict_form: bad argument");
    return guarded([&]() {
        const PredictForm pf = predict_form(m);
        out[0] = pf.form; out[1] = pf.mw; out[2] = pf.tw; out[3] = pf.tb; out[4] = (int32_t)pf.lds;
        return RGBM_OK;
    });
}

RGBM_EXPORT int rgbm_model_importance(const rgbm_model* m, int32_t type, double* out) {
    if (!m || !out) return fail(RGBM_ERR_ARG, "rgbm_model_importance: bad argument");
    for (int f = 0; f < m->F; ++f) out[f] = 0.0;
    for (const Tree& t : m->trees) for (int j = 0; j < t.L - 1; ++j) out[t.feat[j]] += type == 0 ? 1.0 : t.gain[j];
    return RGBM_OK;
}

}
```

### spark-data-repair-plugin_amd/csrc/rgbm_level.h

```cpp
#pragma once
#include "rgbm_kernels.h"

namespace rg {

constexpr int LV_INACTIVE = 255;
constexpr int LV_MAX_EXP = 64;
constexpr int LV_MAX_BUILT = 32;
constexpr int LV_CNT_REP = 16;
constexpr int LV_THREADS = 1024;
constexpr int LV_TILE = 2 * LV_THREADS;
constexpr int LV_LDS_TOTAL = 160 * 1024;
constexpr int LV_LDS_BYTES = LV_LDS_TOTAL;
constexpr int LV_MAX_DEPTH = 7;
constexpr int LV_MAX_LEAVES = 128;

constexpr int MT_MAX_T = 64;
constexpr int MT_MAX_NODES = 128;
constexpr int MT_RT_BUDGET = 256;
constexpr int MT_MAX_RT = MT_RT_BUDGET + MT_MAX_T;
constexpr int MT_WT_ROWS = 256;
constexpr int MT_RING_PLAIN = 128;
constexpr int MT_RING_SPEC = 128;
__host__ __device__ constexpr int mt_ring(bool spec) { return spec ? MT_RING_SPEC : MT_RING_PLAIN; }
constexpr int MT_CNT_REP = 4;

constexpr int MT_THREADS_ACC2 = 768;
#ifndef MT_CONSUMERS_N
#define MT_CONSUMERS_N 4
#endif
constexpr int MT_CONSUMERS = MT_CONSUMERS_N;

struct SNode {
    long long Gq, Hq;
    double pmin;
    int32_t count, depth, parent, is_left;
    int32_t left, right;
    int32_t best_feature, searched;
    int32_t hslot, pad;
    Cand best;
};

struct LvPlan {
    int32_t n_nodes, lvl_first, lvl_end, n_exp, n_built, live_rows , pad1, pad2, pad3, done, error, child_first, n_hslots, pad4;
    long long n_in;
    uint8_t exp[LV_MAX_EXP];
    uint8_t built_is_left[LV_MAX_EXP];
    uint32_t route0[256];
    uint32_t route1[256];
};

struct LevelConst {
    int32_t gx;
    int32_t max_built;
    int32_t nchunk, K, F, totbins, num_leaves, max_depth, min_data_in_leaf, lds_bytes;
    int32_t sib_local;
    int32_t xcd_blocks;
    int32_t mt_T, mt_G, mt_ch, mt_slot0, mt_nslots, mt_route;
    int32_t mt_sparse;
    uint32_t has_mult;
    long long N, NS, NG;
};

__device__ __forceinline__ uint32_t rec_byte(const uint4& r, int j) {
    uint32_t w = (j < 8) ? ((j < 4) ? r.x : r.y) : ((j < 12) ? r.z : r.w);
    return (w >> (8 * (j & 3))) & 0xFFu;
}

constexpr int LV_MAX_Q = 11;
__host__ __device__ inline int lv_shift(int nbins, int q) {
    int l = 0; while ((1 << l) < nbins) ++l;
    int s = q - l;
    return s < 0 ? 0 : (s > 5 ? 5 : s);
}

__host__ __device__ inline int lv_slots(const FeatMeta* fm, int nfeat, int q) {
    int t = 0;
    for (int j = 0; j < nfeat; ++j) t += fm[j].nbins << lv_shift(fm[j].nbins, q);
    return t;
}

__host__ __device__ constexpr int mt_rot_dummy(bool rot) { return rot ? 4 : 0; }
__host__ __device__ inline int mt_shift(int nbins, int q, bool rot) { return rot ? (q < 0 ? 0 : (q > 2 ? 2 : q)) : lv_shift(nbins, q); }
__host__ __device__ inline int mt_slots(const FeatMeta* fm, int nfeat, int q, bool rot) {
    int t = 0;
    for (int j = 0; j < nfeat; ++j) t += fm[j].nbins << mt_shift(fm[j].nbins, q, rot);
    return t;
}
__host__ __device__ constexpr int mt_max_q(bool rot) { return rot ? 2 : LV_MAX_Q; }

constexpr int LV_ROOT_FIXED = 256;
#if !defined(MT_SPARSE_DIV_N)
#define MT_SPARSE_DIV_N 16
#endif
constexpr long long MT_SPARSE_DIV = MT_SPARSE_DIV_N;
__host__ __device__ constexpr long long mt_fixed_bytes(int threads, bool acc2, bool spec = false, bool li = true ) {
    return ((!acc2 && !spec) ? (long long)MT_MAX_T * 8  : 0) + (long long)MT_MAX_T * 32 + MT_MAX_NODES + 16 + 512 + 256 + (long long)(MT_MAX_T + 2) * 8 + (long long)MT_MAX_RT * 8 + (long long)MT_MAX_NODES * MT_CNT_REP * 4 + (long long)MT_MAX_NODES * 8 +
           (long long)(threads / 64 - (spec ? MT_CONSUMERS : 0)) * mt_ring(spec) * ((acc2 ? 32 : 16) + 8 + (li ? 2 : 0)) + 256;
}
__host__ __device__ constexpr long long mt_hd(int threads, bool acc2, bool spec) { return ((LV_LDS_TOTAL - mt_fixed_bytes(threads, acc2, spec, false)) / 2) & ~15ll; }
__host__ __device__ constexpr long long mt_hist_bytes(long long lds_bytes, int threads, bool acc2, bool spec, bool li) {
    const long long fixed = mt_fixed_bytes(threads, acc2, spec, li), hd = mt_hd(threads, acc2, spec);
    const long long room_h = (long long)LV_LDS_TOTAL - fixed - hd;
    const long long x = hd < room_h ? hd : room_h;
    const long long a = lds_bytes - fixed;
    return a < 2 * x ? a : 2 * x;
}

__global__ __launch_bounds__(64) void k_level_init(LvPlan* __restrict__ plan, SNode* __restrict__ nodes, int32_t* __restrict__ count,
                                                   const unsigned int* __restrict__ n_in_ptr, long long n_train,
                                                   unsigned long long* __restrict__ Q, FxGrid fx, FxScale* __restrict__ fxs, LevelConst c) {
    const int k = blockIdx.x, lane = lane_id();
    if (lane == 0) {
        const int e_g = fx_tree_exponent(Q[2 * k], fx.q_mult, fx.c_g, fx.e_g_min, fx.e_g_max);
        const int e_h = fx_tree_exponent(Q[2 * k + 1], fx.q_mult, fx.c_h, fx.e_h_min, fx.e_h_max);
        FxScale f; f.sg = fx_pow2(e_g); f.sh = fx_pow2(e_h); f.inv_sg = fx_pow2(-e_g); f.inv_sh = fx_pow2(-e_h);
        fxs[k] = f;
        Q[2 * k] = 0ull; Q[2 * k + 1] = 0ull;
    }
    LvPlan* pp = &plan[k];
    const long long n_in = n_in_ptr ? (long long)n_in_ptr[0] : n_train;
    for (int i = lane; i < 256; i += 64) { pp->route0[i] = 0; pp->route1[i] = 0xFFFFFFFFu; count[(long long)k * 256 + i] = 0; }
    if (lane == 0) {
        pp->n_nodes = 1; pp->lvl_first = 0; pp->lvl_end = 1; pp->n_exp = 0; pp->n_built = 1;
        pp->error = 0; pp->child_first = 1; pp->n_hslots = 1; pp->n_in = n_in;
        pp->done = (n_in < (long long)c.min_data_in_leaf * 2) ? 1 : 0;
        SNode r; memset(&r, 0, sizeof(r));
        r.count = (int)n_in; r.depth = 0; r.parent = -1; r.left = -1; r.right = -1; r.best_feature = -1; r.searched = 0; r.hslot = 0;
        r.best.gain = -INFINITY; r.pmin = -INFINITY;
        nodes[(long long)k * 256] = r;
    }
}

__global__ __launch_bounds__(LV_THREADS, 1) void k_level_root(const uint4* __restrict__ rec, const float2* __restrict__ gh, const uint8_t* __restrict__ node,
                                                              const LvPlan* __restrict__ plan, HistBin* __restrict__ part,
                                                              const FeatMeta* __restrict__ fmeta, const ChunkMeta* __restrict__ cmeta,
                                                              const FxScale* __restrict__ fxs , LevelConst c) {
    extern __shared__ __attribute__((aligned(16))) unsigned char smem[];
    int k, bx, nbx;
    if (c.xcd_blocks) { const unsigned id = blockIdx.x, r = id >> 3; k = (int)(r % (unsigned)c.K); bx = (int)(r / (unsigned)c.K) * 8 + (int)(id & 7u); nbx = c.gx; }
    else { k = blockIdx.y; bx = blockIdx.x; nbx = gridDim.x; }
    const int ch = blockIdx.z;
    if (plan[k].done) return;
    const double sg_k = fxs[k].sg, sh_k = fxs[k].sh;
    const ChunkMeta cm = cmeta[ch];
    const FeatMeta* fm = fmeta + cm.first_feat;
    const int tid = threadIdx.x, lane = tid & 63, nfeat = cm.nfeat;
    int s = LV_MAX_Q;
    while (s > 0 && (long long)lv_slots(fm, nfeat, s) * 16 + LV_ROOT_FIXED > c.lds_bytes) --s;
    int sh[16], fbase[16], spn = 0;
#pragma unroll
    for (int j = 0; j < 16; ++j) {
        if (j < nfeat) { sh[j] = lv_shift(fm[j].nbins, s); fbase[j] = spn; spn += fm[j].nbins << sh[j]; }
        else { sh[j] = 0; fbase[j] = 0; }
    }
    unsigned long long* hist_g = reinterpret_cast<unsigned long long*>(smem);
    unsigned long long* hist_h = hist_g + spn;
    for (int i = tid; i < 2 * spn; i += LV_THREADS) hist_g[i] = 0ull;
    int cj[16], sh3[16];
#pragma unroll
    for (int j = 0; j < 16; ++j) { sh3[j] = sh[j] + 3; cj[j] = (fbase[j] + (lane & ((1 << sh[j]) - 1))) * 8; }
    const int hdelta = spn;
    __syncthreads();

    const long long N = c.N;
    const uint8_t* node_in = node + (long long)k * c.NS;
    const uint4* recc = rec + (long long)ch * N;
    const float2* ghk = gh + (long long)k * c.NG;
    const long long ntiles_all = (N + LV_TILE - 1) / LV_TILE;
    const long long tbeg = c.xcd_blocks ? ntiles_all * bx / nbx : bx;
    const long long ntiles = c.xcd_blocks ? ntiles_all * (bx + 1) / nbx : ntiles_all;
    const long long tstep = c.xcd_blocks ? 1 : nbx;

    constexpr int RPT = LV_TILE / LV_THREADS;
    int cur_n[RPT], nxt_n[RPT]; uint4 cur_r[RPT], nxt_r[RPT]; float2 cur_g[RPT], nxt_g[RPT];
    auto fetch = [&](long long t, int (&fn)[RPT], uint4 (&fr)[RPT], float2 (&fg)[RPT]) __attribute__((always_inline)) {
        const bool tv = t < ntiles;
        const long long pb = tv ? t * LV_TILE : 0;
        const long long left_rows = N - pb;
        const unsigned lim = (unsigned)(left_rows < LV_TILE ? left_rows : LV_TILE) - 1u;
#pragma unroll
        for (int q = 0; q < RPT; ++q) {
            const unsigned o = (unsigned)(q * LV_THREADS + tid);
            const unsigned oc = o < lim ? o : lim;
            typedef float v2f __attribute__((ext_vector_type(2)));
            const int nv = (int)__builtin_nontemporal_load(node_in + pb + oc);
            fr[q] = (recc + pb)[oc];
            const v2f gv = __builtin_nontemporal_load(reinterpret_cast<const v2f*>(ghk + pb + oc));
            fg[q] = make_float2(gv.x, gv.y);
            fn[q] = (tv && o <= lim) ? nv : LV_INACTIVE;
        }
    };
    auto accumulate = [&](bool on, const uint4& r, const float2& g) __attribute__((always_inline)) {
        if (on && (g.x != 0.0f || g.y != 0.0f)) {
            unsigned long long gq = (unsigned long long)fx_from_f32(g.x, sg_k), hq = (unsigned long long)fx_from_f32(g.y, sh_k);
            if (c.has_mult) { const unsigned long long m = r.w >> 24; gq *= m; hq *= m; }
            unsigned char* hb = reinterpret_cast<unsigned char*>(hist_g);
            const uint32_t w[4] = {r.x, r.y, r.z, r.w};
#define LV_ATOM(j) { const uint32_t code_ = (w[(j) >> 2] >> (8 * ((j) & 3))) & 0xFFu; \
                     unsigned long long* p_ = reinterpret_cast<unsigned long long*>(hb + cj[j] + (int)(code_ << sh3[j])); \
                     atomicAdd(p_, gq); atomicAdd(p_ + hdelta, hq); }
#pragma unroll
            for (int j = 0; j < 16; ++j) if (j < nfeat) LV_ATOM(j);
#undef LV_ATOM
        }
    };
    long long t = tbeg;
    fetch(t, cur_n, cur_r, cur_g);
    while (t < ntiles) {
        fetch(t + tstep, nxt_n, nxt_r, nxt_g);
#pragma unroll
        for (int q = 0; q < RPT; ++q) accumulate(cur_n[q] != LV_INACTIVE, cur_r[q], cur_g[q]);
        t += tstep; if (t >= ntiles) break;
        fetch(t + tstep, cur_n, cur_r, cur_g);
#pragma unroll
        for (int q = 0; q < RPT; ++q) accumulate(nxt_n[q] != LV_INACTIVE, nxt_r[q], nxt_g[q]);
        t += tstep;
    }
    __syncthreads();
    HistBin* dst = part + (((long long)k * c.gx + bx) * c.max_built) * c.totbins;
    for (int j = 0; j < nfeat; ++j) {
        const int shj = lv_shift(fm[j].nbins, s);
        int fb = 0;
        for (int q = 0; q < j; ++q) fb += fm[q].nbins << lv_shift(fm[q].nbins, s);
        for (int b = tid; b < fm[j].nbins; b += LV_THREADS) {
            long long tg = 0, th = 0;
            const unsigned long long* sg_ = hist_g + fb + (b << shj); const unsigned long long* sh_ = hist_h + fb + (b << shj);
            for (int r2 = 0; r2 < (1 << shj); ++r2) { tg += (long long)sg_[r2]; th += (long long)sh_[r2]; }
            HistBin o; o.g = tg; o.h = th;
            dst[fm[j].hoff + b] = o;
        }
    }
}

struct MtTree { int32_t base, nlev, rt_off, slot0, nb, live, child_first, k; };

template <int NCHR , bool BAG,
          bool ROUTE ,
          int THREADS , bool ACC2 ,
          bool SPEC ,
          bool ROTP = false >
__global__ __launch_bounds__(THREADS, 1) void k_level_mt(const uint4* __restrict__ rec, const float2* __restrict__ gh, uint8_t* __restrict__ node ,
                                                         const uint8_t* __restrict__ inbag, const LvPlan* __restrict__ plan, HistBin* __restrict__ part,
                                                         int32_t* __restrict__ count, const FeatMeta* __restrict__ fmeta, const ChunkMeta* __restrict__ cmeta,
                                                         int32_t* __restrict__ err_flag,
                                                         const FxScale* __restrict__ fxs , LevelConst c) {
    static_assert(!ACC2 || NCHR == 2, "a two-chunk pass keeps both records in registers");
    static_assert(ACC2 == SPEC && THREADS == (ACC2 ? MT_THREADS_ACC2 : LV_THREADS) && (!ROTP || NCHR == 1 || ACC2) && (NCHR == 0 || NCHR == 1 || NCHR == 2),
                  "k_level_mt: not one of the six launch forms");
    constexpr int WAVES = THREADS / 64;
    constexpr int NCONS = SPEC ? MT_CONSUMERS : 0, NPROD = WAVES - NCONS;
    constexpr int NACC = ACC2 ? 2 : 1;
    constexpr int NRINGS = SPEC ? NPROD : WAVES;
    constexpr int MT_RING = mt_ring(SPEC);
    constexpr bool ROT = ROTP;
    constexpr bool SPARSE = (NCHR == 1) && !ACC2 && !SPEC;
    extern __shared__ __attribute__((aligned(16))) unsigned char smem[];
    const unsigned id = blockIdx.x;
    const int xl = (int)(id & 7u), bslot = (int)(id >> 3);
    const int grp = bslot % c.mt_G, rb = (bslot / c.mt_G) * 8 + xl;
    const int k0 = grp * c.mt_T;
    const int nk = (c.K - k0) < c.mt_T ? (c.K - k0) : c.mt_T;
    const int tid = threadIdx.x, lane = tid & 63, wave = tid >> 6;
    const int ch = ACC2 ? 0 : c.mt_ch;
    constexpr bool route = ROUTE;
    const ChunkMeta cm = cmeta[ch];
    const ChunkMeta cm1 = cmeta[ACC2 ? 1 : ch];
    const FeatMeta* fm = fmeta + cm.first_feat;
    const FeatMeta* fm1 = fmeta + cm1.first_feat;
    const int nfeat = cm.nfeat, nfeat1 = ACC2 ? cm1.nfeat : 0;
    const int wb = cm.wide_bins + (ACC2 ? cm1.wide_bins : 0);
    const bool li_in_rec = (ACC2 ? nfeat1 : nfeat) <= 15 && !c.has_mult;

    MtTree* ti = reinterpret_cast<MtTree*>(smem);
    uint8_t* nd_tree = smem + MT_MAX_T * 32;
    int32_t* scal = reinterpret_cast<int32_t*>(nd_tree + MT_MAX_NODES);
    int32_t* ftab = scal + 4;
    uint32_t* rsync = reinterpret_cast<uint32_t*>(ftab + 128);
#define RS_LOAD(i) __hip_atomic_load(rsync + (i), __ATOMIC_RELAXED, __HIP_MEMORY_SCOPE_WORKGROUP)
#define RS_STORE(i, v) __hip_atomic_store(rsync + (i), (uint32_t)(v), __ATOMIC_RELAXED, __HIP_MEMORY_SCOPE_WORKGROUP)
    uint2* tpk = reinterpret_cast<uint2*>(ftab + 128 + 64);
    uint2* rt = tpk + MT_MAX_T + 2;
    int32_t* cnt = reinterpret_cast<int32_t*>(rt + MT_MAX_RT);
    uint2* nd_sc = reinterpret_cast<uint2*>(cnt + MT_MAX_NODES * MT_CNT_REP);
    uint4* ring_rec_all = reinterpret_cast<uint4*>(nd_sc + MT_MAX_NODES);
    uint4* ring_rec1_all = ring_rec_all + (ACC2 ? NRINGS * MT_RING : 0);
    uint2* ring_gh_all = reinterpret_cast<uint2*>(ring_rec1_all + NRINGS * MT_RING);
    uint16_t* ring_li_all = reinterpret_cast<uint16_t*>(ring_gh_all + NRINGS * MT_RING);
    size_t off = reinterpret_cast<unsigned char*>(ring_li_all + (li_in_rec ? 0 : NRINGS * MT_RING)) - smem;
    off = (off + 15) & ~(size_t)15;
    unsigned long long* xmask = reinterpret_cast<unsigned long long*>(smem + off);
    if (!ACC2 && !SPEC) off += (size_t)MT_MAX_T * 8;
    unsigned long long* hist_g = reinterpret_cast<unsigned long long*>(smem + off);
    constexpr int MT_HD = (int)mt_hd(THREADS, ACC2, SPEC);
    const long long avail = mt_hist_bytes(c.lds_bytes, THREADS, ACC2, SPEC, !li_in_rec);
    if (tid == 0 && ((long long)off > mt_fixed_bytes(THREADS, ACC2, SPEC, !li_in_rec) || (long long)off + MT_HD + avail / 2 > (long long)LV_LDS_TOTAL)) atomicOr(err_flag, 2);

    if (tid < 64) {
        MtTree t; t.base = 0; t.nlev = 0; t.nb = 0; t.live = 0; t.child_first = 0; t.k = k0 + lane; t.slot0 = 0; t.rt_off = 0;
        if (lane < nk) {
            const LvPlan* pp = &plan[k0 + lane];
            const bool live = !pp->done && pp->n_exp > 0;
            t.live = live ? 1 : 0;
            t.child_first = pp->child_first;
            t.base = live ? (route ? (int)pp->exp[0] : pp->child_first) : 0;
            t.nlev = live ? (route ? pp->child_first - (int)pp->exp[0] : 2 * pp->n_exp) : 0;
            int nb = live ? pp->n_built - c.mt_slot0 : 0;
            if (nb > c.mt_nslots) nb = c.mt_nslots;
            t.nb = nb < 0 ? 0 : nb;
        }
        bool sparse_t = false;
        if (SPARSE && lane < nk && t.live && t.nlev <= 64) {
            const LvPlan* pp = &plan[k0 + lane];
            const long long lr = route ? (long long)pp->live_rows : 0ll;
            sparse_t = route && lr * MT_SPARSE_DIV < pp->n_in && c.mt_sparse != 0;
        }
        const int ntab = lane < nk ? (route ? (t.live ? t.child_first : 0) : t.nlev) + 1 : 0;
        int inc_nb = t.nb, inc_rt = ntab;
#pragma unroll
        for (int o = 1; o < 64; o <<= 1) { const int a = __shfl_up(inc_nb, o), b2 = __shfl_up(inc_rt, o); if (lane >= o) { inc_nb += a; inc_rt += b2; } }
        t.slot0 = inc_nb - t.nb; t.rt_off = inc_rt - ntab;
        const int total = __shfl(inc_nb, 63), rt_total = __shfl(inc_rt, 63);
        const unsigned long long livem = __ballot(t.live != 0);
        const bool ok = total <= MT_MAX_NODES && rt_total <= MT_MAX_RT;
        if (!ok) { t.live = 0; t.nb = 0; t.nlev = 0; if (lane == 0) atomicOr(err_flag, 2); }
        const bool dead_t = lane < nk && (!t.live || (!route && t.nb == 0));
        const unsigned long long dmask = __ballot(lane < nk && !sparse_t && !dead_t), smask = __ballot(lane < nk && sparse_t && !dead_t), zmask = __ballot(dead_t);
        const int nkd_ = __popcll(dmask), nks_ = __popcll(smask);
        const unsigned long long below = (1ull << lane) - 1ull;
        const int pos = lane >= nk ? lane : (dead_t ? nkd_ + nks_ + __popcll(zmask & below) : (sparse_t ? nkd_ + __popcll(smask & below) : __popcll(dmask & below)));
        if (lane < nk) ti[pos] = t;
        tpk[pos] = make_uint2((uint32_t)t.base | (uint32_t)t.nlev << 8 | (uint32_t)(ntab > 0 ? ntab - 1 : 0) << 17 | (t.live && lane < nk ? 1u << 31 : 0u), (uint32_t)t.rt_off | (uint32_t)t.k << 16);
        if (lane < 2) tpk[64 + lane] = make_uint2(0u, 0u);
        if (SPARSE) xmask[lane] = 0ull;
        if (lane == 0) {
            int s = mt_max_q(ROT);
            const int tot = ok ? total : 0;
            while (s > 0 && (long long)tot * (mt_slots(fm, nfeat, s, ROT) + (ACC2 ? mt_slots(fm1, nfeat1, s, ROT) : 0) + mt_rot_dummy(ROT)) * 16 > avail) --s;
            const int spn0 = mt_slots(fm, nfeat, s, ROT) + (ACC2 ? mt_slots(fm1, nfeat1, s, ROT) : 0) + mt_rot_dummy(ROT);
            if ((long long)tot * spn0 * 16 > avail) atomicOr(err_flag, 2);
            scal[0] = tot; scal[1] = s; scal[2] = spn0; scal[3] = ((ok && livem != 0ull) ? 1 : 0) | nkd_ << 8 | (nkd_ + nks_) << 16;
        }
    }
    __syncthreads();
    if (!(scal[3] & 1)) return;
    const int total = __builtin_amdgcn_readfirstlane(scal[0]), s = __builtin_amdgcn_readfirstlane(scal[1]), spn = __builtin_amdgcn_readfirstlane(scal[2]);
    if (!route && total == 0) return;
    const int nkd = __builtin_amdgcn_readfirstlane((scal[3] >> 8) & 0xFF), nke = __builtin_amdgcn_readfirstlane((scal[3] >> 16) & 0xFF);
    for (int kk = 0; kk < nk; ++kk) {
        const MtTree t = ti[kk];
        const LvPlan* pp = &plan[t.k];
        const int ntab_k = (route ? (t.live ? t.child_first : 0) : t.nlev) + 1;
        for (int i = tid; i < ntab_k; i += THREADS) {
            const int n = route ? i : t.base + i;
            uint2 e;
            if (route) {
                const bool cur = i < ntab_k - 1 && n >= t.base;
                const uint32_t w0 = cur ? pp->route0[n] : 0u; const uint32_t w1 = cur ? pp->route1[n] : 0u;
                if (w0 & (1u << 24)) {
                    const int ls = (int)((w1 >> 16) & 0xFFu) - c.mt_slot0, rs = (int)(w1 >> 24) - c.mt_slot0;
                    const bool lb = ((w1 >> 16) & 0xFFu) != 0xFFu && ls >= 0 && ls < t.nb, rbb = (w1 >> 24) != 0xFFu && rs >= 0 && rs < t.nb;
                    const uint32_t theta1 = (w0 >> 8) & 0xFFu, nanbin = (w0 >> 16) & 0xFFu, dleft = (w0 >> 25) & 1u;
                    uint32_t offb, thr;
                    if (nanbin != 255u && dleft) { offb = nanbin; thr = (theta1 - 1u - nanbin) & 0xFFu; }
                    else if (theta1 == 0u) { offb = 255u; thr = 0u; }
                    else { offb = 0u; thr = theta1 - 1u; }
                    const uint32_t f = w0 & 0xFFu;
                    e = make_uint2((NCHR == 0 ? f : (f & 7u) | ((f >> 4) & 1u) << 30 | ((f >> 3) & 1u) << 31) | thr << 8 | offb << 16 | 1u << 24,
                                   (w1 & 0xFFu) | (lb ? (uint32_t)(t.slot0 + ls) : 0xFFu) << 8 | ((w1 >> 8) & 0xFFu) << 16 | (rbb ? (uint32_t)(t.slot0 + rs) : 0xFFu) << 24);
                    if (SPARSE && kk >= nkd && kk < nke && n - t.base < 64) atomicOr(&xmask[kk], 1ull << (n - t.base));
                } else {
                    const uint32_t self = i < ntab_k - 1 ? (uint32_t)n : (uint32_t)LV_INACTIVE;
                    e = make_uint2(0u, self | 0xFF00u | self << 16 | 0xFF000000u);
                }
            } else {
                const int ei = i >> 1, ls = ei - c.mt_slot0;
                const bool mine = i < ntab_k - 1 && (pp->built_is_left[ei] ? 0 : 1) == (i & 1) && ls >= 0 && ls < t.nb;
                e = make_uint2(mine ? 1u : 0u, mine ? (uint32_t)(t.slot0 + ls) : 0xFFu);
            }
            rt[t.rt_off + i] = e;
        }
        const uint2 sc_k = make_uint2((uint32_t)__double2hiint(fxs[t.k].sg), (uint32_t)__double2hiint(fxs[t.k].sh));
        for (int i = tid; i < t.nb; i += THREADS) { nd_tree[t.slot0 + i] = (uint8_t)kk; nd_sc[t.slot0 + i] = sc_k; }
    }
    for (int i = tid; i < total * MT_CNT_REP; i += THREADS) cnt[i] = 0;
    if (tid < 48) rsync[tid] = 0u;
    unsigned long long* hist_h = hist_g + MT_HD / 8;
    for (int i = tid; i < total * spn; i += THREADS) { hist_g[i] = 0ull; hist_h[i] = 0ull; }
    unsigned long long sh3p[NACC];
    int cj[NACC][16];
    {
        int o = 0;
#pragma unroll
        for (int a = 0; a < NACC; ++a) {
            const FeatMeta* fa = a == 0 ? fm : fm1;
            const int na = a == 0 ? nfeat : nfeat1;
            unsigned long long pk = 0ull;
#pragma unroll
            for (int j = 0; j < 16; ++j) {
                int shj = 0, fb = 0;
                if (j < na) { shj = mt_shift(fa[j].nbins, s, ROT); fb = o; o += fa[j].nbins << shj; }
                pk |= (unsigned long long)(shj + 3) << (4 * j); cj[a][j] = (fb + (lane & ((1 << shj) - 1))) * 8;
                if (tid == 0) {
                    const int q = a * 16 + j;
                    const int wide = (a == 0 ? 0 : cm.wide_bins) + (j < na ? fa[j].wide_off : 0);
                    ftab[q] = j < na ? wide : 0x7FFFFFFF; ftab[32 + q] = fb; ftab[64 + q] = shj; ftab[96 + q] = j < na ? fa[j].hoff - wide : 0;
                }
            }
            sh3p[a] = (unsigned long long)(unsigned)__builtin_amdgcn_readfirstlane((int)(unsigned)pk) |
                      (unsigned long long)(unsigned)__builtin_amdgcn_readfirstlane((int)(unsigned)(pk >> 32)) << 32;
        }
    }
    constexpr int hdelta = MT_HD / 8;
    __syncthreads();
    uint32_t rmask[NACC][4];
    const int rot_sh = mt_shift(1, s, ROT) + 3;
    if (ROT) {
        const int r16 = lane & 15, c4 = lane >> 4;
        const int spn_valid = spn - mt_rot_dummy(ROT);
#pragma unroll
        for (int a = 0; a < NACC; ++a) {
            const int na = a == 0 ? nfeat : nfeat1;
#pragma unroll
            for (int w = 0; w < 4; ++w) rmask[a][w] = 0u;
#pragma unroll
            for (int j = 0; j < 16; ++j) {
                const int f = (j + r16) & 15;
                const bool fv = f < na;
                cj[a][j] = fv ? (ftab[32 + a * 16 + f] + (c4 & ((1 << (rot_sh - 3)) - 1))) * 8 : (spn_valid + c4) * 8;
                rmask[a][j >> 2] |= fv ? (0xFFu << (8 * (j & 3))) : 0u;
            }
        }
    }

    const int my_ring = __builtin_amdgcn_readfirstlane(wave < NRINGS ? wave : 0);
    uint4* ring_rec = ring_rec_all + my_ring * MT_RING;
    uint4* ring_rec1 = ring_rec1_all + my_ring * MT_RING;
    uint2* ring_gh = ring_gh_all + my_ring * MT_RING;
    uint16_t* ring_li = ring_li_all + my_ring * MT_RING;
    int r_head = 0, r_cnt = 0;
    const unsigned long long lane_lt = (1ull << lane) - 1ull;
    const unsigned spn8 = (unsigned)spn * 8u;
    const uint2 tpk_v = tpk[lane];
    auto tree_entry = [&](int kk) __attribute__((always_inline)) -> uint2 {
        const int kc = kk < 64 ? kk : 63;
        const uint32_t x = (uint32_t)__builtin_amdgcn_readlane((int)tpk_v.x, kc), y = (uint32_t)__builtin_amdgcn_readlane((int)tpk_v.y, kc);
        return kk < nkd ? make_uint2(x, y) : make_uint2(0u, 0u);
    };

    auto run_batch_of = [&](int rid, int head, int nb) __attribute__((always_inline)) {
        __builtin_amdgcn_fence(__ATOMIC_RELEASE, "wavefront");
        const bool on = lane < nb;
        const int pos = rid * MT_RING + ((head + lane) & (MT_RING - 1));
        const uint4 r = ring_rec_all[pos]; const uint2 g = ring_gh_all[pos];
        uint4 r1 = make_uint4(0, 0, 0, 0);
        if (ACC2) r1 = ring_rec1_all[pos];
        unsigned li;
        if (li_in_rec) li = (ACC2 ? r1.w : r.w) >> 24; else li = ring_li_all[pos];
        unsigned long long shp[NACC];
#pragma unroll
        for (int a = 0; a < NACC; ++a) { shp[a] = sh3p[a]; asm volatile("" : "+s"(shp[a])); }
        if (on) {
            const uint2 sc = nd_sc[li];
            unsigned long long gq = (unsigned long long)fx_from_f32(__uint_as_float(g.x), __hiloint2double((int)sc.x, 0)),
                               hq = (unsigned long long)fx_from_f32(__uint_as_float(g.y), __hiloint2double((int)sc.y, 0));
            int mrow = 1;
            if (c.has_mult) { mrow = (int)((ACC2 ? r1.w : r.w) >> 24); gq *= (unsigned long long)mrow; hq *= (unsigned long long)mrow; }
            if (ch == 0) atomicAdd(&cnt[li * MT_CNT_REP + (lane & (MT_CNT_REP - 1))], mrow);
            unsigned char* hb = reinterpret_cast<unsigned char*>(hist_g) + li * spn8;
            uint32_t w[4] = {r.x, r.y, r.z, r.w};
            uint32_t w1[4] = {r1.x, r1.y, r1.z, r1.w};
            if (ROT) {
                auto rot16 = [&](uint32_t (&x)[4], const uint32_t (&mk)[4]) __attribute__((always_inline)) {
                    const bool d1 = (lane & 4) != 0, d2 = (lane & 8) != 0;
                    const uint32_t a0 = d1 ? x[1] : x[0], a1 = d1 ? x[2] : x[1], a2 = d1 ? x[3] : x[2], a3 = d1 ? x[0] : x[3];
                    const uint32_t b0 = d2 ? a2 : a0, b1 = d2 ? a3 : a1, b2 = d2 ? a0 : a2, b3 = d2 ? a1 : a3;
                    const uint32_t sb = (uint32_t)(lane & 3);
                    x[0] = __builtin_amdgcn_alignbyte(b1, b0, sb) & mk[0]; x[1] = __builtin_amdgcn_alignbyte(b2, b1, sb) & mk[1];
                    x[2] = __builtin_amdgcn_alignbyte(b3, b2, sb) & mk[2]; x[3] = __builtin_amdgcn_alignbyte(b0, b3, sb) & mk[3];
                };
                rot16(w, rmask[0]);
                if (ACC2) rot16(w1, rmask[NACC - 1]);
            }
#if defined(MT_DBL_ATOM)
#define MT_ATOMIC_ADD(p, v) { atomicAdd(p, (v) - 1ull); atomicAdd(p, 1ull); }
#else
#define MT_ATOMIC_ADD(p, v) atomicAdd(p, v)
#endif
#define MT_ATOM(A, W, j) { unsigned long long* p_ = reinterpret_cast<unsigned long long*>(hb + cj[A][j] + (int)(((W[(j) >> 2] >> (8 * ((j) & 3))) & 0xFFu) << (ROT ? rot_sh : (int)((shp[A] >> (4 * (j))) & 15ull)))); \
                           MT_ATOMIC_ADD(p_, gq); MT_ATOMIC_ADD(p_ + hdelta, hq); }
            if (ROT) {
                MT_ATOM(0, w, 0); MT_ATOM(0, w, 1); MT_ATOM(0, w, 2); MT_ATOM(0, w, 3); MT_ATOM(0, w, 4); MT_ATOM(0, w, 5); MT_ATOM(0, w, 6); MT_ATOM(0, w, 7);
                MT_ATOM(0, w, 8); MT_ATOM(0, w, 9); MT_ATOM(0, w, 10); MT_ATOM(0, w, 11); MT_ATOM(0, w, 12); MT_ATOM(0, w, 13); MT_ATOM(0, w, 14); MT_ATOM(0, w, 15);
                if (ACC2) {
                    MT_ATOM(NACC - 1, w1, 0); MT_ATOM(NACC - 1, w1, 1); MT_ATOM(NACC - 1, w1, 2); MT_ATOM(NACC - 1, w1, 3); MT_ATOM(NACC - 1, w1, 4); MT_ATOM(NACC - 1, w1, 5);
                    MT_ATOM(NACC - 1, w1, 6); MT_ATOM(NACC - 1, w1, 7); MT_ATOM(NACC - 1, w1, 8); MT_ATOM(NACC - 1, w1, 9); MT_ATOM(NACC - 1, w1, 10); MT_ATOM(NACC - 1, w1, 11);
                    MT_ATOM(NACC - 1, w1, 12); MT_ATOM(NACC - 1, w1, 13); MT_ATOM(NACC - 1, w1, 14); MT_ATOM(NACC - 1, w1, 15);
                }
            } else
            if (nfeat >= 15) {
                MT_ATOM(0, w, 0); MT_ATOM(0, w, 1); MT_ATOM(0, w, 2); MT_ATOM(0, w, 3); MT_ATOM(0, w, 4); MT_ATOM(0, w, 5); MT_ATOM(0, w, 6); MT_ATOM(0, w, 7);
                MT_ATOM(0, w, 8); MT_ATOM(0, w, 9); MT_ATOM(0, w, 10); MT_ATOM(0, w, 11); MT_ATOM(0, w, 12); MT_ATOM(0, w, 13); MT_ATOM(0, w, 14);
                if (nfeat == 16) MT_ATOM(0, w, 15);
            } else {
#pragma unroll
                for (int j = 0; j < 14; ++j) if (j < nfeat) MT_ATOM(0, w, j);
            }
            if (!ROT && ACC2) {
                if (nfeat1 >= 15) {
                    MT_ATOM(NACC - 1, w1, 0); MT_ATOM(NACC - 1, w1, 1); MT_ATOM(NACC - 1, w1, 2); MT_ATOM(NACC - 1, w1, 3); MT_ATOM(NACC - 1, w1, 4); MT_ATOM(NACC - 1, w1, 5);
                    MT_ATOM(NACC - 1, w1, 6); MT_ATOM(NACC - 1, w1, 7); MT_ATOM(NACC - 1, w1, 8); MT_ATOM(NACC - 1, w1, 9); MT_ATOM(NACC - 1, w1, 10); MT_ATOM(NACC - 1, w1, 11);
                    MT_ATOM(NACC - 1, w1, 12); MT_ATOM(NACC - 1, w1, 13); MT_ATOM(NACC - 1, w1, 14);
                    if (nfeat1 == 16) MT_ATOM(NACC - 1, w1, 15);
                } else {
#pragma unroll
                    for (int j = 0; j < 14; ++j) if (j < nfeat1) MT_ATOM(NACC - 1, w1, j);
                }
            }
#undef MT_ATOM
#undef MT_ATOMIC_ADD
        }
    };
    auto run_batch = [&](int nb) __attribute__((always_inline)) {
        run_batch_of(wave, r_head, nb);
        r_head = (r_head + nb) & (MT_RING - 1); r_cnt -= nb;
    };

    if (SPEC && wave >= NPROD) {
        const int cw = wave - NPROD;
        constexpr int NR = SPEC ? (NPROD + MT_CONSUMERS - 1) / MT_CONSUMERS : 1;
        uint32_t head[NR];
#pragma unroll
        for (int i = 0; i < NR; ++i) head[i] = 0u;
        for (;;) {
            bool any = false, all_done = true;
#pragma unroll
            for (int i = 0; i < NR; ++i) {
                const int rid = cw + i * MT_CONSUMERS;
                if (rid >= NPROD) continue;
                const uint32_t done = (uint32_t)__builtin_amdgcn_readfirstlane((int)RS_LOAD(32 + rid));
                asm volatile("" ::: "memory");
                const uint32_t tail = (uint32_t)__builtin_amdgcn_readfirstlane((int)RS_LOAD(rid));
                asm volatile("" ::: "memory");
                uint32_t avail = tail - head[i];
                while (avail >= 64u) { run_batch_of(rid, (int)head[i], 64); head[i] += 64u; avail -= 64u; any = true; }
                if (done && avail > 0u) { run_batch_of(rid, (int)head[i], (int)avail); head[i] += avail; avail = 0u; any = true; }
                if (any) { asm volatile("" ::: "memory"); if (lane == 0) RS_STORE(16 + rid, head[i]); }
                if (!done || avail > 0u) all_done = false;
            }
            if (all_done) break;
            if (!any) __builtin_amdgcn_s_sleep(4);
        }
    }

    uint32_t p_tail = 0u, p_head_seen = 0u;
    const long long N = c.N, NS = c.NS, NG = c.NG;
    const long long nwt_all = (N + MT_WT_ROWS - 1) / MT_WT_ROWS;
    const long long wt_lo = nwt_all * rb / c.gx, wt_hi = nwt_all * (rb + 1) / c.gx;
    const uint8_t* rec8 = reinterpret_cast<const uint8_t*>(rec);
    const uint4* rec_acc = rec + (long long)ch * N;
    typedef float v4f __attribute__((ext_vector_type(4)));

    auto load_rec = [&](long long wt, uint4 (&ra)[4], uint4 (&r1)[4], uint32_t& bagmask) __attribute__((always_inline)) {
        const long long tile0 = wt * MT_WT_ROWS;
// ... 83 lines not shown
                if (SPEC) p_tail += (uint32_t)__popcll(m);
                else { r_cnt += (int)__popcll(m); if (r_cnt >= 64) run_batch(64); }
            }
        }
        if (SPEC) { asm volatile("" ::: "memory"); if (lane == 0) RS_STORE(wave, p_tail); }
    };
    auto stage_c = [&](const long long row0, const uint4 (&ra)[4], const uint4 (&r1)[4], uint32_t bagmask, uint32_t n4, const float4 g0, const float4 g1,
                       const uint2 (&e)[4], const uint2 tq) __attribute__((always_inline)) {
        if ((tq.x >> 31) == 0u) return;
        uint32_t liv[4];
        if (ROUTE) route4(row0, ra, r1, n4, e, tq, liv);
        else {
#pragma unroll
            for (int j = 0; j < 4; ++j) liv[j] = e[j].y & 0xFFu;
        }
        append4(ra, r1, bagmask, g0, g1, liv);
    };

    if (wave < NPROD) {
        const int nkw = nkd;
        {
            const long long my_first = wt_lo + __builtin_amdgcn_readfirstlane(wave);
            const long long ntile_w = (nkw > 0 && my_first < wt_hi) ? (wt_hi - my_first + NPROD - 1) / NPROD : 0;
            const long long Q = ntile_w * nkw;
            if (Q > 0) {
                struct TS { uint32_t n4; float4 g0, g1; };
                TS S0, S1, S2;
                uint2 e_cur[4];
                bool cross = false;
                long long wt_c = my_first, wt_n = my_first, wt_l = my_first; int kk_c = 0, kk_n = 0, kk_l = 0;
                auto fwd = [&](long long& wt, int& kk) __attribute__((always_inline)) { if (++kk == nkw) { kk = 0; wt += NPROD; } };
                if (Q > 1) fwd(wt_n, kk_n);
                wt_l = wt_n; kk_l = kk_n;
                if (Q > 2) fwd(wt_l, kk_l);
                uint4 ra[4], r1[4], rn[4], r1n[4]; uint32_t bagmask, bagmask_n = 0u;
                load_rec(wt_c, ra, r1, bagmask);
#pragma unroll
                for (int j = 0; j < 4; ++j) { rn[j] = ra[j]; r1n[j] = r1[j]; }
                load_tree(wt_c, kk_c, S0.n4, S0.g0, S0.g1);
                load_tree(wt_n, kk_n, S1.n4, S1.g0, S1.g1);
                lookup(S0.n4, tree_entry(kk_c), e_cur);
                long long q = 0;
                auto step = [&](TS& cur, TS& nxt, TS& in) __attribute__((always_inline)) {
                    load_tree(wt_l, kk_l, in.n4, in.g0, in.g1);
                    if (cross) {
#pragma unroll
                        for (int j = 0; j < 4; ++j) { ra[j] = rn[j]; r1[j] = r1n[j]; }
                        bagmask = bagmask_n;
                    }
                    if (kk_c == 0 && wt_c + NPROD < wt_hi) load_rec(wt_c + NPROD, rn, r1n, bagmask_n);
                    const uint2 tq_c = tree_entry(kk_c);
                    const bool live = (tq_c.x >> 31) != 0u;
                    uint32_t liv[4] = {0xFFu, 0xFFu, 0xFFu, 0xFFu};
                    if (ROUTE) { if (live) route4(wt_c * MT_WT_ROWS + lane * 4, ra, r1, cur.n4, e_cur, tq_c, liv); }
                    else {
#pragma unroll
                        for (int j = 0; j < 4; ++j) liv[j] = e_cur[j].y & 0xFFu;
                    }
                    lookup(nxt.n4, tree_entry(kk_n), e_cur);
                    if (live) append4(ra, r1, bagmask, cur.g0, cur.g1, liv);
                    cross = wt_n != wt_c;
                    wt_c = wt_n; kk_c = kk_n; wt_n = wt_l; kk_n = kk_l;
                    if (q + 3 < Q) fwd(wt_l, kk_l);
                    ++q;
                };
                while (q < Q) {
                    step(S0, S1, S2);
                    if (q < Q) step(S1, S2, S0);
                    if (q < Q) step(S2, S0, S1);
                }
            }
        }
    }
    if (!SPEC) {
        if (SPARSE && nkd < nke) {
            const long long row_lo = wt_lo * MT_WT_ROWS, row_hi = (wt_hi * MT_WT_ROWS < N) ? wt_hi * MT_WT_ROWS : N;
            const long long nst = (wt_hi * MT_WT_ROWS - row_lo + 1023) / 1024;
            for (int kk = nkd; kk < nke; ++kk) {
                const uint32_t tq0 = (uint32_t)__builtin_amdgcn_readlane((int)tpk_v.x, kk < 64 ? kk : 63), tq1 = (uint32_t)__builtin_amdgcn_readlane((int)tpk_v.y, kk < 64 ? kk : 63);
                const uint2 tq = make_uint2(tq0, tq1);
                const uint32_t base = tq0 & 0xFFu, nlev = (tq0 >> 8) & 0x1FFu;
                const unsigned long long xm_v = xmask[kk];
                const unsigned long long xm = (unsigned long long)(uint32_t)__builtin_amdgcn_readfirstlane((int)(uint32_t)xm_v) | (unsigned long long)(uint32_t)__builtin_amdgcn_readfirstlane((int)(uint32_t)(xm_v >> 32)) << 32;
                const uint8_t* nd_k = node + (long long)(tq1 >> 16) * NS;
                const float2* gh_k = gh + (long long)(tq1 >> 16) * NG;
                int sp_cnt = 0;
                uint32_t pend = 0u;
                auto sparse_batch = [&](int nb) __attribute__((always_inline)) {
                    const bool on = lane < nb;
                    const uint32_t g = pend;
                    const long long row0 = on ? (long long)g * 4 : row_lo;
                    uint4 ra[4], r1[4]; uint32_t bagmask = BAG ? 0u : 0xFu;
#pragma unroll
                    for (int j = 0; j < 4; ++j) {
                        long long rr = row0 + j; if (rr >= N) rr = N - 1;
                        ra[j] = rec_acc[rr]; r1[j] = make_uint4(0, 0, 0, 0);
                        if (BAG) bagmask |= (inbag[rr] ? 1u : 0u) << j;
                    }
                    const uint32_t n4 = on ? *reinterpret_cast<const uint32_t*>(nd_k + row0) : 0xFFFFFFFFu;
                    const float4 g0 = *reinterpret_cast<const float4*>(gh_k + row0), g1 = *reinterpret_cast<const float4*>(gh_k + row0 + 2);
                    uint2 e[4];
                    lookup(n4, tq, e);
                    stage_c(row0, ra, r1, bagmask, n4, g0, g1, e, tq);
                    sp_cnt = 0;
                };
                auto load16 = [&](long long st) __attribute__((always_inline)) -> uint4 {
                    const long long r16 = row_lo + st * 1024 + lane * 16;
                    uint4 v = make_uint4(0xFFFFFFFFu, 0xFFFFFFFFu, 0xFFFFFFFFu, 0xFFFFFFFFu);
                    if (st < nst && r16 < row_hi) v = *reinterpret_cast<const uint4*>(nd_k + r16);
                    return v;
                };
                uint4 n16 = load16(wave);
                for (long long st = wave; st < nst; st += WAVES) {
                    const long long r16 = row_lo + st * 1024 + lane * 16;
                    const uint4 nxt = load16(st + WAVES);
                    const long long left = row_hi - r16;
                    const int nvalid = left >= 16 ? 16 : (left > 0 ? (int)left : 0);
                    const uint32_t w4[4] = {n16.x, n16.y, n16.z, n16.w};
#pragma unroll
                    for (int d = 0; d < 4; ++d) {
                        bool hit = false;
#pragma unroll
                        for (int j = 0; j < 4; ++j) {
                            const uint32_t idx = ((w4[d] >> (8 * j)) & 0xFFu) - base;
                            hit = hit || (idx < nlev && ((xm >> (idx & 63u)) & 1ull) != 0ull && d * 4 + j < nvalid);
                        }
                        const unsigned long long m = __ballot(hit);
                        if (m != 0ull) {
                            const int np = (int)__popcll(m), r_hit = (int)__popcll(m & lane_lt);
                            const int dest = hit ? sp_cnt + r_hit : sp_cnt + np + (lane - r_hit);
                            const uint32_t rx = (uint32_t)__builtin_amdgcn_ds_permute((dest & 63) << 2, (int)(uint32_t)((r16 + d * 4) >> 2));
                            const int rel = (lane - sp_cnt) & 63;
                            if (sp_cnt + np < 64) { if (rel < np) pend = rx; sp_cnt += np; }
                            else {
                                const int rem = sp_cnt + np - 64;
                                if (rel < 64 - sp_cnt) pend = rx;
                                sparse_batch(64);
                                if (lane < rem) pend = rx;
                                sp_cnt = rem;
                            }
                        }
                    }
                    n16 = nxt;
                }
                if (sp_cnt > 0) sparse_batch(sp_cnt);
            }
        }
    }
    if (SPEC) { if (wave < NPROD) { asm volatile("" ::: "memory"); if (lane == 0) { RS_STORE(wave, p_tail); asm volatile("" ::: "memory"); RS_STORE(32 + wave, 1u); } } }
#undef RS_LOAD
#undef RS_STORE
    else while (r_cnt > 0) run_batch(r_cnt < 64 ? r_cnt : 64);
    __syncthreads();
    constexpr int NQ = NACC * 16;
    for (int i = tid; i < total * wb; i += THREADS) {
        const int ln = i / wb, b = i - ln * wb;
        const MtTree t = ti[nd_tree[ln]];
        int j = 0;
#pragma unroll
        for (int q = 1; q < NQ; ++q) j += (b >= ftab[q]) ? 1 : 0;
        const int shb = ftab[64 + j], s0 = ftab[32 + j] + ((b - ftab[j]) << shb);
        long long tg = 0, th = 0;
        const unsigned long long* sg_ = hist_g + (size_t)ln * spn + s0; const unsigned long long* sh_ = hist_h + (size_t)ln * spn + s0;
        for (int r2 = 0; r2 < (1 << shb); ++r2) { tg += (long long)sg_[r2]; th += (long long)sh_[r2]; }
        HistBin o; o.g = tg; o.h = th;
        part[(((long long)t.k * c.gx + rb) * c.max_built + (c.mt_slot0 + ln - t.slot0)) * c.totbins + ftab[96 + j] + b] = o;
    }
    if (ch == 0) {
        for (int ln = tid; ln < total; ln += THREADS) {
            int tot = 0;
            for (int r2 = 0; r2 < MT_CNT_REP; ++r2) tot += cnt[ln * MT_CNT_REP + r2];
            const MtTree t = ti[nd_tree[ln]];
            const int ei = c.mt_slot0 + ln - t.slot0;
            if (tot) atomicAdd(&count[(long long)t.k * 256 + t.child_first + 2 * ei + (plan[t.k].built_is_left[ei] ? 0 : 1)], tot);
        }
    }
}

__global__ __launch_bounds__(256) void k_level_reduce(const HistBin* __restrict__ part, HistBin* __restrict__ red, const LvPlan* __restrict__ plan,
                                                      const int32_t* __restrict__ count, int is_root, int nb, LevelConst c) {
    __shared__ long long sg[4][64], sh[4][64];
    const int k = blockIdx.z, bslot = blockIdx.y, bl = threadIdx.x & 63, xl = threadIdx.x >> 6;
    const int b = blockIdx.x * 64 + bl;
    if (blockIdx.x == 0 && blockIdx.y == 0)
        reinterpret_cast<long long*>(red + (long long)c.K * nb * c.totbins)[(long long)k * 256 + threadIdx.x] = (long long)count[(long long)k * 256 + threadIdx.x];
    const LvPlan* pp = &plan[k];
    const int n_built = pp->done ? 0 : (is_root ? 1 : pp->n_built);
    long long ag = 0, ah = 0;
    if (b < c.totbins && bslot < n_built) {
        const HistBin* src = part + (((long long)k * c.gx) * c.max_built + bslot) * c.totbins + b;
        const long long xs = (long long)c.max_built * c.totbins;
#pragma unroll 8
        for (int x = xl; x < c.gx; x += 4) { const HistBin v = src[x * xs]; ag += v.g; ah += v.h; }
    }
    sg[xl][bl] = ag; sh[xl][bl] = ah;
    __syncthreads();
    if (xl == 0 && b < c.totbins) {
        HistBin acc; acc.g = sg[0][bl] + sg[1][bl] + sg[2][bl] + sg[3][bl]; acc.h = sh[0][bl] + sh[1][bl] + sh[2][bl] + sh[3][bl];
        red[((long long)k * nb + bslot) * c.totbins + b] = acc;
    }
}

struct JointFeat { int32_t voff , stride, nbins , nbv , hoff, vbyte , pad0, pad1; };

__global__ __launch_bounds__(256) void k_pack_joint(const uint4* __restrict__ rec, long long N, int F, const JointFeat* __restrict__ jf, uint4* __restrict__ rec_joint,
                                                    int mult_chunk = -1 ) {
    const long long i = (long long)blockIdx.x * 256 + threadIdx.x;
    if (i >= N) return;
    const uint8_t* rec8 = reinterpret_cast<const uint8_t*>(rec);
    uint32_t w[4] = {0, 0, 0, 0};
    for (int f = 0; f < F; ++f) {
        const uint32_t bin = rec8[((long long)(f >> 4) * N + i) * 16 + (f & 15)];
        const int vb = jf[f].vbyte;
        w[vb >> 2] += (bin * (uint32_t)jf[f].stride) << (8 * (vb & 3));
    }
    if (mult_chunk >= 0) w[3] = (w[3] & 0x00FFFFFFu) | ((uint32_t)rec8[((long long)mult_chunk * N + i) * 16 + 15] << 24);
    rec_joint[i] = make_uint4(w[0], w[1], w[2], w[3]);
}

__global__ __launch_bounds__(256) void k_level_marginal(const HistBin* __restrict__ red_j , HistBin* __restrict__ red, const LvPlan* __restrict__ plan,
                                                        const int32_t* __restrict__ count, const JointFeat* __restrict__ jf, const int16_t* __restrict__ bin_feat ,
                                                        int vtotbins, LevelConst c) {
    const int k = blockIdx.y;
    if (blockIdx.x == 0)
        reinterpret_cast<long long*>(red + (long long)c.K * c.totbins)[(long long)k * 256 + threadIdx.x] = (long long)count[(long long)k * 256 + threadIdx.x];
    const int b = blockIdx.x * 256 + threadIdx.x;
    if (b >= c.totbins) return;
    HistBin acc; acc.g = 0; acc.h = 0;
    if (!plan[k].done) {
        const JointFeat f = jf[bin_feat[b]];
        const int digit = b - f.hoff;
        const int period = f.stride * f.nbins;
        const HistBin* src = red_j + (long long)k * vtotbins + f.voff;
        for (int base = digit * f.stride; base < f.nbv; base += period)
            for (int lo = 0; lo < f.stride; ++lo) { const HistBin v = src[base + lo]; acc.g += v.g; acc.h += v.h; }
    }
    red[(long long)k * c.totbins + b] = acc;
}

__global__ __launch_bounds__(256) void k_counts_unpack(const long long* __restrict__ cnt64, int32_t* __restrict__ count_g) {
    const long long i = (long long)blockIdx.x * 256 + threadIdx.x;
    count_g[i] = (int32_t)cnt64[i];
}

template <bool ROOT>
__global__ __launch_bounds__(256) void k_level_split(const HistBin* __restrict__ part, HistBin* __restrict__ pool, LvPlan* __restrict__ plan,
                                                     SNode* __restrict__ nodes, int32_t* __restrict__ count, int32_t* __restrict__ count_local,
                                                     const FeatMeta* __restrict__ fmeta, const uint8_t* __restrict__ used_all ,
                                                     Cand* __restrict__ cand , unsigned long long* __restrict__ stat_rows,
                                                     const int32_t* __restrict__ itp ,
                                                     int n_hnodes, const FxScale* __restrict__ fxs, TrainConst c_model, LevelConst lc) {
    const int k = blockIdx.z, pi = blockIdx.y;
    const TrainConst c = tree_const(c_model, fxs, k);
    const uint8_t* used = used_all + (long long)(*itp) * c.K * c.F;
    const int wv = threadIdx.x >> 6;
    const int f = ROOT ? blockIdx.x * 4 + wv : blockIdx.x * 2 + (wv >> 1);
    const int side = wv & 1;
    const LvPlan* pp = &plan[k];
    if (pp->done) return;
    if (!ROOT && pi >= pp->n_exp) return;
    if (f >= c.F) return;
    const int lane = lane_id();
    const FeatMeta fm = fmeta[f];
    SNode* nk = nodes + (long long)k * 256;
    Cand* ck = cand + (long long)k * 256 * c.F;
    HistBin* pk = pool + (long long)k * n_hnodes * c.totbins;
    const bool is_used = used[(long long)k * c.F + f] != 0;
    long long ag[4], ah[4];
    const int bslot = ROOT ? 0 : pi;
#pragma unroll
    for (int j = 0; j < 4; ++j) { ag[j] = 0; ah[j] = 0; }
    for (int x = 0; x < lc.gx; ++x) {
        const HistBin* src = part + (((long long)k * lc.gx + x) * lc.max_built + bslot) * c.totbins + fm.hoff;
#pragma unroll
        for (int j = 0; j < 4; ++j) { const int b = lane * 4 + j; if (b < fm.nbins) { const HistBin v = src[b]; ag[j] += v.g; ah[j] += v.h; } }
    }
    if (ROOT) {
        HistBin* h0 = pk + fm.hoff;
        long long sg_ = 0, sh_ = 0;
#pragma unroll
        for (int j = 0; j < 4; ++j) { const int b = lane * 4 + j; if (b < fm.nbins) { HistBin v; v.g = ag[j]; v.h = ah[j]; h0[b] = v; } sg_ += ag[j]; sh_ += ah[j]; }
#pragma unroll
        for (int o = 32; o >= 1; o >>= 1) { sg_ += __shfl_xor(sg_, o); sh_ += __shfl_xor(sh_, o); }
        if (f == 0 && lane == 0) { nk[0].Gq = sg_; nk[0].Hq = sh_; nk[0].searched = 1; atomicAdd(stat_rows, (unsigned long long)pp->n_in); }
        if (!is_used) { if (lane == 0) ck[f].gain = -INFINITY; return; }
        scan_child(ag, ah, fm, sg_, sh_, pp->n_in, c, &ck[f]);
        return;
    }
    const int p = pp->exp[pi];
    const SNode P = nk[p];
    const int l = P.left, r = P.right;
    const bool bl = pp->built_is_left[pi] != 0;
    const int me = side == 0 ? l : r;
    const bool i_am_built = (side == 0) == bl;
    const HistBin* hp = pk + (long long)P.hslot * c.totbins + fm.hoff;
    HistBin* hm = pk + (long long)nk[me].hslot * c.totbins + fm.hoff;
    if (!i_am_built) {
#pragma unroll
        for (int j = 0; j < 4; ++j) {
            const int b = lane * 4 + j;
            if (b < fm.nbins) { const HistBin par = hp[b]; ag[j] = par.g - ag[j]; ah[j] = par.h - ah[j]; } else { ag[j] = 0; ah[j] = 0; }
        }
    }
#pragma unroll
    for (int j = 0; j < 4; ++j) { const int b = lane * 4 + j; if (b < fm.nbins) { HistBin v; v.g = ag[j]; v.h = ah[j]; hm[b] = v; } }
    int nl = count[(long long)k * 256 + l], nr = count[(long long)k * 256 + r];
    {
        const int nb = bl ? nl : nr, ns = P.count - nb;
        if (bl) nr = ns; else nl = ns;
        if (f == 0 && lane == 0 && side == 0) {
            const int sib = bl ? r : l;
            count[(long long)k * 256 + sib] = ns;
            if (lc.sib_local && count_local != count) count_local[(long long)k * 256 + sib] = ns;
// ... 305 lines not shown
```

### spark-data-repair-plugin_amd/repair/_native.py

```python
import ctypes as C
import os

import numpy as np

_HERE = os.path.dirname(os.path.abspath(__file__))
LIB_PATH = os.path.join(_HERE, "..", "lib", "librepairgbm.so")


class RepairGbmError(RuntimeError):
    pass


class RgbmParams(C.Structure):
    _fields_ = [
        ("objective", C.c_int32), ("num_class", C.c_int32),
        ("n_estimators", C.c_int32), ("num_leaves", C.c_int32), ("max_depth", C.c_int32), ("max_bin", C.c_int32),
        ("min_data_in_leaf", C.c_int32), ("min_data_in_bin", C.c_int32), ("bagging_freq", C.c_int32), ("seed", C.c_int32),
        ("device_id", C.c_int32), ("reserved", C.c_int32),
        ("learning_rate", C.c_double), ("lambda_l1", C.c_double), ("lambda_l2", C.c_double), ("min_gain_to_split", C.c_double),
        ("min_sum_hessian_in_leaf", C.c_double), ("bagging_fraction", C.c_double), ("feature_fraction", C.c_double),
    ]


class RgbmTrainStats(C.Structure):
    _fields_ = [
        ("hist_ms", C.c_double), ("total_ms", C.c_double), ("hist_launches", C.c_int64), ("hist_rows", C.c_int64),
        ("hist_bytes", C.c_int64), ("root_rows", C.c_int64), ("root_ms", C.c_double), ("trees", C.c_int64),
        ("route_ms", C.c_double), ("route_launches", C.c_int64), ("root_atomics_per_row", C.c_int64), ("level_atomics_per_row", C.c_int64),
    ]

    def as_dict(self):
        return {k: getattr(self, k) for k, _ in self._fields_}


PARAM_DEFAULTS = dict(objective=1, num_class=2, n_estimators=300, num_leaves=31, max_depth=7, max_bin=255,
                      min_data_in_leaf=20, min_data_in_bin=3, bagging_freq=0, seed=42, device_id=0, reserved=0,
                      learning_rate=0.01, lambda_l1=0.0, lambda_l2=0.0, min_gain_to_split=0.0,
                      min_sum_hessian_in_leaf=1e-3, bagging_fraction=1.0, feature_fraction=1.0)


FLAG_ROW_SHARDED = 1
FLAG_NO_MODEL = 2
FLAG_WHOLE_TABLE = 4
VIEW_STATES = ("none", "built", "not worth it", "cannot")


def make_params(**kw):
    d = dict(PARAM_DEFAULTS)
    kw = dict(kw)
    if kw.pop("row_sharded", False):
        d["reserved"] = d.get("reserved", 0) | FLAG_ROW_SHARDED
    if kw.pop("whole_table", False):
        d["reserved"] = d.get("reserved", 0) | FLAG_WHOLE_TABLE
    if not kw.pop("want_model", True):
        d["reserved"] = d.get("reserved", 0) | FLAG_NO_MODEL
    for k, v in kw.items():
        if k not in d:
            raise TypeError("unknown parameter %r" % k)
        d[k] = v
    return RgbmParams(**d)


_lib = None


def lib():
    global _lib
    if _lib is None:
        path = os.path.abspath(os.environ.get("RGBM_LIB_PATH") or LIB_PATH)
        if not os.path.exists(path):
            raise RepairGbmError("librepairgbm.so is not built (%s); run `python __graft_entry__.py` or `make -C "
                                 "spark-data-repair-plugin_amd/csrc`" % path)
        l = C.CDLL(path)
        l.rgbm_last_error.restype = C.c_char_p
        for name in ("rgbm_device_count", "rgbm_version", "rgbm_release_cache", "rgbm_train", "rgbm_predict", "rgbm_repair_chain",
                     "rgbm_table_create", "rgbm_table_train", "rgbm_table_train_batch", "rgbm_table_repair_chain", "rgbm_table_read_column",
                     "rgbm_model_save", "rgbm_model_load", "rgbm_model_info", "rgbm_model_importance", "rgbm_model_predict_form",
                     "rgbm_comm_unique_id", "rgbm_comm_init", "rgbm_comm_finalize", "rgbm_comm_info", "rgbm_comm_count",
                     "rgbm_local_group_create", "rgbm_comm_init_local",
                     "rgbm_table_detect_nulls", "rgbm_table_detect_constraint", "rgbm_table_rows_of_cells", "rgbm_table_cells_fetch",
                     "rgbm_table_null_cells", "rgbm_table_gather_rows", "rgbm_table_count_codes", "rgbm_table_create_dict",
                     "rgbm_table_shape", "rgbm_table_repair_pmf", "rgbm_table_read_cells", "rgbm_table_repair_pmf_weighted",
                     "rgbm_edit_distance", "rgbm_table_pair_counts", "rgbm_table_cell_domains", "rgbm_table_fd_map", "rgbm_table_rule_fill",
                     "rgbm_nearest_values", "rgbm_table_detect_cells", "rgbm_table_distinct_rows",
                     "rgbm_table_read_row_multiplicity", "rgbm_table_detect_dc", "rgbm_table_detect_row_bits",
                     "rgbm_table_kmeans_assign", "rgbm_table_kmeans_read", "rgbm_lof_1d", "rgbm_table_column_stats"):
            getattr(l, name).restype = C.c_int
        for name in ("rgbm_table_distinct_view_info", "rgbm_distinct_view_eligible"):
            if hasattr(l, name):
                getattr(l, name).restype = C.c_int
        l.rgbm_local_group_free.restype = None
        l.rgbm_table_free.restype = None
        l.rgbm_model_free.restype = None
        l.rgbm_host_free.restype = None
        _lib = l
    return _lib


EXPORTED_SYMBOLS = [
    "rgbm_device_count", "rgbm_last_error", "rgbm_version", "rgbm_release_cache", "rgbm_train", "rgbm_predict", "rgbm_repair_chain",
    "rgbm_table_create", "rgbm_table_free", "rgbm_table_train", "rgbm_table_train_batch", "rgbm_table_repair_chain", "rgbm_table_read_column",
    "rgbm_model_save", "rgbm_model_load", "rgbm_model_free", "rgbm_model_info", "rgbm_model_importance",
    "rgbm_comm_unique_id", "rgbm_comm_init", "rgbm_comm_finalize", "rgbm_comm_info", "rgbm_comm_count",
    "rgbm_local_group_create", "rgbm_local_group_free", "rgbm_comm_init_local",
    "rgbm_comm_all_gather_sizes", "rgbm_comm_all_gather_bytes", "rgbm_table_repair_chain_gather", "rgbm_comm_gather_stats",
    "rgbm_fusion_create", "rgbm_fusion_join", "rgbm_fusion_leave", "rgbm_fusion_info", "rgbm_fusion_free",
    "rgbm_table_detect_nulls", "rgbm_table_detect_constraint", "rgbm_table_rows_of_cells", "rgbm_table_cells_fetch",
    "rgbm_table_null_cells", "rgbm_table_gather_rows", "rgbm_table_count_codes", "rgbm_table_create_dict", "rgbm_table_shape",
    "rgbm_table_repair_pmf", "rgbm_table_read_cells", "rgbm_table_write_cells", "rgbm_host_alloc", "rgbm_host_free",
    "rgbm_table_set_column_values", "rgbm_table_set_column_kind", "rgbm_table_set_row_multiplicity",
    "rgbm_table_repair_pmf_weighted", "rgbm_edit_distance", "rgbm_table_pair_counts", "rgbm_table_cell_domains",
    "rgbm_table_fd_map", "rgbm_table_rule_fill", "rgbm_nearest_values", "rgbm_table_detect_cells",
    "rgbm_table_distinct_rows", "rgbm_table_read_row_multiplicity", "rgbm_table_detect_dc", "rgbm_table_detect_row_bits", "rgbm_model_predict_form",
    "rgbm_table_kmeans_assign", "rgbm_table_kmeans_read", "rgbm_table_distinct_view_info", "rgbm_distinct_view_eligible",
    "rgbm_table_column_stats",
]
EXPORTED_SYMBOLS_WITH_DIGITS = ["rgbm_lof_1d"]

COMM_ID_BYTES = 128


def comm_unique_id():
    buf = (C.c_ubyte * COMM_ID_BYTES)()
    _check(lib().rgbm_comm_unique_id(buf), "rgbm_comm_unique_id")
    return bytes(buf)


def comm_init(uid, rank, nranks, device_id=0):
    buf = (C.c_ubyte * COMM_ID_BYTES).from_buffer_copy(bytes(uid))
    _check(lib().rgbm_comm_init(buf, C.c_int32(rank), C.c_int32(nranks), C.c_int32(device_id)), "rgbm_comm_init")


def comm_finalize():
    _check(lib().rgbm_comm_finalize(), "rgbm_comm_finalize")


def comm_info():
    a = np.zeros(3, np.int32)
    _check(lib().rgbm_comm_info(_p(a, C.c_int32)), "rgbm_comm_info")
    return dict(kind=int(a[0]), rank=int(a[1]), nranks=int(a[2]))


def model_trees(blob):
    import struct
    hdr = struct.unpack_from("7i", blob, 0)
    ver, K, n_iter, F = hdr[1], hdr[4], hdr[5], hdr[6]
    p = 28
    for _ in range(F):
        _, V, _ = struct.unpack_from("3i", blob, p); p += 12 + 4 * V
        if ver == 2:
            nw, = struct.unpack_from("i", blob, p); p += 4 + 4 * nw
    trees = []
    for _ in range(K * n_iter):
        L, = struct.unpack_from("i", blob, p); p += 4
        n = L - 1
        t = {}
        for name in ("feat", "theta", "dleft", "left", "right"):
            t[name] = np.frombuffer(blob, np.int32, n, p); p += 4 * n
        t["gain"] = np.frombuffer(blob, np.float64, n, p); p += 8 * n
        t["leaf_value"] = np.frombuffer(blob, np.float64, L, p); p += 8 * L
        t["leaf_count"] = np.frombuffer(blob, np.int32, L, p); p += 4 * L
        trees.append(t)
    return K, n_iter, trees


def needed_built_rows(blob, max_depth):
    _, _, trees = model_trees(blob)
    total = 0
    for tr in trees:
        n = len(tr["feat"])
        if n == 0:
            continue
        left, right, lc = tr["left"], tr["right"], tr["leaf_count"]
        cnt = np.zeros(n, np.int64)
        for j in range(n - 1, -1, -1):
            a, b = int(left[j]), int(right[j])
            cnt[j] = (cnt[a] if a >= 0 else int(lc[~a])) + (cnt[b] if b >= 0 else int(lc[~b]))
        depth = np.zeros(n, np.int32)
        for j in range(n):
            a, b = int(left[j]), int(right[j])
            if a >= 0:
                depth[a] = depth[j] + 1
            if b >= 0:
                depth[b] = depth[j] + 1
            if depth[j] + 1 < max_depth:
                ca = cnt[a] if a >= 0 else int(lc[~a]); cb = cnt[b] if b >= 0 else int(lc[~b])
                total += int(min(ca, cb))
    return total


def comm_count():
    n = C.c_int32(0)
    _check(lib().rgbm_comm_count(C.byref(n)), "rgbm_comm_count")
    return int(n.value)


def comm_all_gather_sizes(values):
    v = np.ascontiguousarray(values, np.int64).reshape(-1)
    out = np.zeros((max(1, comm_info()["nranks"]), v.size), np.int64)
    _check(lib().rgbm_comm_all_gather_sizes(_p(v, C.c_int64), C.c_int32(v.size), _p(out, C.c_int64)), "rgbm_comm_all_gather_sizes")
    return out


def comm_all_gather_bytes(payload):
    mine = np.frombuffer(bytes(payload), np.uint8) if not isinstance(payload, np.ndarray) else np.ascontiguousarray(payload).view(np.uint8).reshape(-1)
    sizes = comm_all_gather_sizes([mine.size])[:, 0]
    block = int(max(int(sizes.max()), 1))
    recv = np.zeros((len(sizes), block), np.uint8)
    _check(lib().rgbm_comm_all_gather_bytes(_p(mine, C.c_uint8) if mine.size else None, C.c_int64(mine.size), C.c_int64(block), _p(recv, C.c_uint8)),
           "rgbm_comm_all_gather_bytes")
    return [recv[r, :int(sizes[r])].copy() for r in range(len(sizes))]


def comm_gather_stats():
    a = np.zeros(3, np.int64)
    _check(lib().rgbm_comm_gather_stats(_p(a, C.c_int64)), "rgbm_comm_gather_stats")
    return dict(bytes=int(a[0]), seconds=float(a[1]) * 1e-9, collectives=int(a[2]))


class FusionGroup:

    def __init__(self, n_members):
        self.h = C.c_void_p()
        _check(lib().rgbm_fusion_create(C.c_int32(n_members), C.byref(self.h)), "rgbm_fusion_create")
        self.n_members = n_members

    class _Member:
        def __init__(self, group, j):
            self.group, self.j = group, j

        def __enter__(self):
            _check(lib().rgbm_fusion_join(self.group.h, C.c_int32(self.j)), "rgbm_fusion_join")
            return self

        def __exit__(self, et, ev, tb):
            lib().rgbm_fusion_leave(C.c_int32(0 if et is None else 1))
            return False

    def member(self, j):
        return FusionGroup._Member(self, j)

    def info(self):
        a = np.zeros(4, np.int64)
        _check(lib().rgbm_fusion_info(self.h, _p(a, C.c_int64)), "rgbm_fusion_info")
        return dict(collectives=int(a[0]), parts=int(a[1]), members_in=int(a[2]), broken=bool(a[3]))

    def close(self):
        if self.h:
            _check(lib().rgbm_fusion_free(self.h), "rgbm_fusion_free")
            self.h = C.c_void_p()


class LocalGroup:

    def __init__(self, nranks, device_id=0):
        self.h = C.c_void_p()
        _check(lib().rgbm_local_group_create(C.c_int32(nranks), C.c_int32(device_id), C.byref(self.h)), "rgbm_local_group_create")
        self.nranks = nranks

    def join(self, rank):
        _check(lib().rgbm_comm_init_local(self.h, C.c_int32(rank)), "rgbm_comm_init_local")

    def __del__(self):
        h, self.h = getattr(self, "h", None), None
        if h and _lib is not None:
            _lib.rgbm_local_group_free(h)


def _check(rc, what):
    if rc != 0:
        err = RepairGbmError("%s failed (%d): %s" % (what, rc, lib().rgbm_last_error().decode("utf-8", "replace")))
        err.code = rc
        raise err


def device_count():
    return int(lib().rgbm_device_count())


def release_cache():
    _check(lib().rgbm_release_cache(), "rgbm_release_cache")


def _p(a, t):
    return a.ctypes.data_as(C.POINTER(t)) if a is not None else None


def _i32(a):
    return None if a is None else np.ascontiguousarray(a, np.int32)


def _f64(a):
    return None if a is None else np.ascontiguousarray(a, np.float64)


class Model:

    def __init__(self, handle):
        self.h = handle

    def __del__(self):
        h, self.h = getattr(self, "h", None), None
        if h and _lib is not None:
            _lib.rgbm_model_free(h)

    def info(self):
        a = np.zeros(5, np.int32)
        _check(lib().rgbm_model_info(self.h, _p(a, C.c_int32)), "rgbm_model_info")
        return dict(objective=int(a[0]), num_class=int(a[1]), K=int(a[2]), n_iter=int(a[3]), F=int(a[4]))

    def save(self):
        n = C.c_size_t(0)
        _check(lib().rgbm_model_save(self.h, None, C.byref(n)), "rgbm_model_save")
        buf = bytearray(max(n.value, 1))
        _check(lib().rgbm_model_save(self.h, (C.c_char * len(buf)).from_buffer(buf), C.byref(n)), "rgbm_model_save")
        return bytes(buf[:n.value]) if n.value != len(buf) else bytes(buf)

    @staticmethod
    def load(b):
        h = C.c_void_p()
        arr = np.frombuffer(b, np.uint8)
        _check(lib().rgbm_model_load(arr.ctypes.data_as(C.c_void_p), C.c_size_t(len(b)), C.byref(h)), "rgbm_model_load")
        return Model(h)

    def importance(self, kind="gain"):
        out = np.zeros(self.info()["F"], np.float64)
        _check(lib().rgbm_model_importance(self.h, C.c_int32(0 if kind == "split" else 1), _p(out, C.c_double)), "rgbm_model_importance")
        return out

    def predict_form(self):
        a = np.zeros(5, np.int32)
        _check(lib().rgbm_model_predict_form(self.h, _p(a, C.c_int32)), "rgbm_model_predict_form")
        return dict(form=("fixed", "dynamic", "walk")[int(a[0])], MW=int(a[1]), TW=int(a[2]), tb=int(a[3]), lds=int(a[4]))

    def predict(self, X, device_id=0):
        X = _i32(X)
        F, n = X.shape
        inf = self.info()
        ncol = 1 if inf["objective"] == 2 else inf["num_class"]
        out = np.zeros((n, ncol), np.float64)
        _check(lib().rgbm_predict(self.h, _p(X, C.c_int32), C.c_int64(n), C.c_int32(F), C.c_int32(device_id), _p(out, C.c_double)), "rgbm_predict")
        return out


def train(X, n_codes, y_code, n_y_codes, y_value=None, class_weight=None, sample_weight=None, want_stats=False, **params):
    X = _i32(X)
    F, N = X.shape
    n_codes, y_code = _i32(n_codes), _i32(y_code)
    yv, cw, sw = _f64(y_value), _f64(class_weight), _f64(sample_weight)
    p = make_params(**params)
    h = C.c_void_p()
    st = RgbmTrainStats()
    _check(lib().rgbm_train(_p(X, C.c_int32), C.c_int64(N), C.c_int32(F), _p(n_codes, C.c_int32), _p(y_code, C.c_int32),
                            C.c_int32(n_y_codes), _p(yv, C.c_double), _p(cw, C.c_double), _p(sw, C.c_double),
                            C.byref(p), C.byref(h), C.byref(st) if want_stats else None), "rgbm_train")
    m = Model(h)
    return (m, st.as_dict()) if want_stats else m


class RgbmFitSpec(C.Structure):
    _fields_ = [("table", C.c_void_p), ("target_col", C.c_int32), ("n_features", C.c_int32), ("feat_cols", C.POINTER(C.c_int32)),
                ("y_value", C.POINTER(C.c_double)), ("class_weight", C.POINTER(C.c_double)), ("params", C.POINTER(RgbmParams)),
                ("valid_table", C.c_void_p), ("valid_label_out", C.POINTER(C.c_int32)), ("valid_value_out", C.POINTER(C.c_double))]


def distinct_view_eligible(rows, f, table_has_mult=False, min_rows=0, **params):
    p = make_params(**params)
    r = lib().rgbm_distinct_view_eligible(C.c_int64(rows), C.c_int32(f), C.byref(p), C.c_int32(1 if table_has_mult else 0), C.c_int64(min_rows))
    if r < 0:
        _check(r, "rgbm_distinct_view_eligible")
    return bool(r)


def train_batch(fits):
    n = len(fits)
    if n == 0:
        return []
    specs = (RgbmFitSpec * n)()
    keep = []
    for i, f in enumerate(fits):
        f = dict(f)
        tab = f.pop("table")
        fc = _i32(f.pop("feat_cols"))
        yv, cw = _f64(f.pop("y_value", None)), _f64(f.pop("class_weight", None))
        target = int(f.pop("target_col"))
        vtab = f.pop("valid_table", None)
        vlab = np.zeros(vtab.n, np.int32) if vtab is not None else None
        vval = np.zeros(vtab.n, np.float64) if vtab is not None else None
        f.setdefault("device_id", tab.device_id)
        p = make_params(**f)
        keep.append((tab, fc, yv, cw, p, vtab, vlab, vval))
        specs[i].valid_table = vtab.h if vtab is not None else None
        specs[i].valid_label_out = _p(vlab, C.c_int32)
        specs[i].valid_value_out = _p(vval, C.c_double)
        specs[i].table = tab.h
        specs[i].target_col = target
        specs[i].n_features = len(fc)
        specs[i].feat_cols = _p(fc, C.c_int32)
        specs[i].y_value = _p(yv, C.c_double)
        specs[i].class_weight = _p(cw, C.c_double)
        specs[i].params = C.pointer(p)
    handles = (C.c_void_p * n)()
    status = np.zeros(n, np.int32)
    _check(lib().rgbm_table_train_batch(specs, C.c_int32(n), handles, _p(status, C.c_int32)), "rgbm_table_train_batch")
    out = []
    failing = [i for i in range(n) if status[i] != 0]
    last_msg = lib().rgbm_last_error().decode("utf-8", "replace") if failing else ""
    for i in range(n):
        if status[i] == 0 and (handles[i] or (keep[i][5] is not None and keep[i][4].reserved & FLAG_NO_MODEL)):
            m = Model(C.c_void_p(handles[i])) if handles[i] else None
            out.append(m if keep[i][5] is None else (m, keep[i][6], keep[i][7]))
        else:
            why = last_msg if (failing and i == failing[-1]) else ("status %d" % int(status[i]) if status[i] != 0 else "no model returned")
            out.append(RepairGbmError("fit %d of the batch failed (%d): %s" % (i, int(status[i]), why)))
    return out


def _chain_args(models, feat_cols, class_codes):
    T = len(models)
    arr = (C.c_void_p * max(T, 1))(*[m.h for m in models])
    fo = np.zeros(T + 1, np.int32)
    co = np.zeros(T + 1, np.int32)
    for t in range(T):
        fo[t + 1] = fo[t] + len(feat_cols[t])
        if class_codes is not None:
            co[t + 1] = co[t] + len(class_codes[t])
    fc = _i32(np.concatenate([np.asarray(f, np.int32) for f in feat_cols])) if T else np.zeros(1, np.int32)
    cc = None
    if class_codes is not None:
        cc = _i32(np.concatenate([np.asarray(c, np.int32) for c in class_codes] + [np.zeros(1, np.int32)]))
    return arr, fc, fo, cc, co


def repair_chain(models, target_col, feat_cols, class_codes, table, device_id=0):
    T = len(models)
    Cc, n = table.shape
    assert table.dtype == np.int32 and table.flags.c_contiguous
    arr, fc, fo, cc, co = _chain_args(models, feat_cols, class_codes)
    tc = _i32(target_col)
    lab = np.zeros((T, n), np.int32)
    prob = np.zeros((T, n), np.float64)
    _check(lib().rgbm_repair_chain(arr, C.c_int32(T), _p(tc, C.c_int32), _p(fc, C.c_int32), _p(fo, C.c_int32), _p(cc, C.c_int32),
                                   _p(co, C.c_int32), _p(table, C.c_int32), C.c_int64(n), C.c_int32(Cc), C.c_int32(device_id),
                                   _p(lab, C.c_int32), _p(prob, C.c_double)), "rgbm_repair_chain")
    return lab, prob


class _PinnedBlock:

    def __init__(self, nbytes):
        p = C.c_void_p()
        _check(lib().rgbm_host_alloc(C.c_size_t(nbytes), C.byref(p)), "rgbm_host_alloc")
        self.p, self.nbytes = p, nbytes
        self.__array_interface__ = {"shape": (nbytes,), "typestr": "|u1", "data": (p.value, False), "version": 3}

    def __del__(self):
        if getattr(self, "p", None):
            lib().rgbm_host_free(self.p)
            self.p = None


def pinned_empty(shape, dtype=np.int32):
    n = int(np.prod(shape)) * np.dtype(dtype).itemsize
    return np.asarray(_PinnedBlock(max(n, 1)))[:n].view(dtype).reshape(shape)


def pack_code_points(strings):
    strings = [str(s) for s in strings]
    off = np.zeros(len(strings) + 1, np.int64)
    if strings:
        np.cumsum([len(s) for s in strings], out=off[1:])
    cp = np.frombuffer("".join(strings).encode("utf-32-le", "surrogatepass"), dtype="<u4").astype(np.int32)
    return cp, off


def edit_distance(a, b, device_id=0):
    a_cp, a_off = pack_code_points(a)
    b_cp, b_off = pack_code_points(b)
    out = np.zeros((len(a_off) - 1, len(b_off) - 1), np.int32)
    _check(lib().rgbm_edit_distance(C.c_int32(device_id), _p(a_cp, C.c_int32), _p(a_off, C.c_int64), C.c_int64(len(a_off) - 1),
                                    _p(b_cp, C.c_int32), _p(b_off, C.c_int64), C.c_int64(len(b_off) - 1), _p(out, C.c_int32)),
           "rgbm_edit_distance")
    return out


def nearest_values(a=None, b=None, cost=None, threshold=0.0, device_id=0):
    if cost is not None:
        m = _f64(cost)
        if m.ndim != 2:
            raise ValueError("cost must be a [n_a][n_b] matrix")
        out = np.full(m.shape[0], -1, np.int32)
        _check(lib().rgbm_nearest_values(C.c_int32(device_id), None, None, C.c_int64(m.shape[0]), None, None, C.c_int64(m.shape[1]),
                                         _p(m, C.c_double), C.c_double(threshold), _p(out, C.c_int32)), "rgbm_nearest_values")
        return out
    a_cp, a_off = pack_code_points(a)
    b_cp, b_off = pack_code_points(b)
    out = np.full(len(a_off) - 1, -1, np.int32)
    _check(lib().rgbm_nearest_values(C.c_int32(device_id), _p(a_cp, C.c_int32), _p(a_off, C.c_int64), C.c_int64(len(a_off) - 1),
                                     _p(b_cp, C.c_int32), _p(b_off, C.c_int64), C.c_int64(len(b_off) - 1), None, C.c_double(threshold),
                                     _p(out, C.c_int32)), "rgbm_nearest_values")
    return out


def lof_1d(values, counts, k=20, threshold=1.5, want_scores=True, device_id=0):
    v = _f64(values).reshape(-1)
    m = np.ascontiguousarray(counts, np.int64).reshape(-1)
    if len(v) != len(m):
        raise ValueError("values and counts must have one length")
    score = np.zeros(len(v), np.float64) if want_scores else None
    bits = np.zeros((len(v) + 63) // 64, np.uint64)
    info = np.zeros(2, np.int64)
    _check(lib().rgbm_lof_1d(C.c_int32(device_id), _p(v, C.c_double), _p(m, C.c_int64), C.c_int32(len(v)), C.c_int32(int(k)),
                             C.c_double(threshold), _p(score, C.c_double) if want_scores else None, _p(bits, C.c_uint64),
                             _p(info, C.c_int64)), "rgbm_lof_1d")
    return score, bits, int(info[0]), int(info[1])

# ... 371 lines not shown
```

Measured before the change: 1.703 million.

## Precompute histogram layouts on host and choose grid sizes with a cost model

Per-chunk root and multi-tree histogram layouts (quantisation level, shifts, feature bases, a bin-to-feature table) are now built once on the host and uploaded. The kernels read these tables instead of recomputing them per block, and a direct bin_feat lookup replaces a linear scan over feature boundaries. Grid sizes for the root and level passes now come from an analytic time model instead of occupancy efficiency. The change also vectorises LDS zeroing and spreads per-tree table setup across waves. A planning introspection API is exported as well, and the new cost model may choose different grids.

```diff
diff --git a/include/rgbm.h b/include/rgbm.h
--- a/include/rgbm.h
+++ b/include/rgbm.h
@@ -211,6 +211,7 @@
 void rgbm_model_free(rgbm_model* m);
 int rgbm_model_info(const rgbm_model* m, int32_t* info);
 int rgbm_model_predict_form(const rgbm_model* m, int32_t* out);
+int rgbm_level_pass_plan(const int32_t* nbins, int32_t f, int64_t n_rows, int32_t k, int32_t max_depth, int32_t with_mult, double* out, int32_t out_len, int32_t* n_out);
 int rgbm_model_importance(const rgbm_model* m, int32_t type, double* out );
 
 #ifdef __cplusplus
diff --git a/spark-data-repair-plugin_amd/csrc/rgbm.hip b/spark-data-repair-plugin_amd/csrc/rgbm.hip
--- a/spark-data-repair-plugin_amd/csrc/rgbm.hip
+++ b/spark-data-repair-plugin_amd/csrc/rgbm.hip
@@ -415,6 +415,18 @@
     size_t part_items = 0;
 };
 
+struct PassCost { double t_fix_us, t_row_ns, t_pair_ns; };
+constexpr PassCost MT_COST_REP{14.0, 0.2, 0.75};
+constexpr PassCost MT_COST_ROT{14.0, 1.0, 0.5};
+constexpr PassCost ROOT_PASS_COST{8.0, 1.2, 0.0};
+inline const PassCost& mt_pass_cost(bool , bool rot) { return rot ? MT_COST_ROT : MT_COST_REP; }
+inline double pass_model_us(long long workgroups, double rows_per_block, int T, const PassCost& c) {
+    const long long rounds = (workgroups + 255) / 256;
+    return (double)rounds * (c.t_fix_us + rows_per_block * (c.t_row_ns + (double)T * c.t_pair_ns) * 1e-3);
+}
+
+inline int level_lds_bytes(const RunSwitches& sw) { return (sw.lv_lds >= 65536 && sw.lv_lds <= rg::LV_LDS_BYTES) ? sw.lv_lds : rg::LV_LDS_BYTES; }
+
 LevelPassPlan plan_level_passes(const RunSwitches& sw, const std::vector<rg::FeatMeta>& fmeta, const std::vector<rg::ChunkMeta>& cmeta,
                                 long long N, int K, int max_depth, bool wm , int lds_bytes) {
     using namespace rg;
@@ -425,16 +437,15 @@
     {
         const long long cu_slots = 256, per = (long long)K * nchunk;
         const long long gmin = std::max<long long>(1, (N + (1ll << 22) - 1) >> 22);
-        auto eff_of = [&](long long g) { const long long tot = g * per, rounds = (tot + cu_slots - 1) / cu_slots; return (double)tot / (double)(rounds * cu_slots); };
+        auto time_of = [&](long long g) { return pass_model_us(g * per, (double)N / (double)g, 1, ROOT_PASS_COST); };
         const long long gfloor = std::max<long long>(8, (gmin + 7) / 8 * 8), gcap = std::max<long long>(gfloor, std::min<long long>(512, (ntiles + 7) / 8 * 8));
         long long g2 = gfloor; double best2 = -1.0;
-        for (long long g = gfloor; g <= gcap; g += 8) {
-            if (per >= 16 && (g * per < 3 * cu_slots || g * per > 5 * cu_slots)) continue;
-            const double e = eff_of(g);
-            if (e > best2 + 1e-9) { best2 = e; g2 = g; }
-            if (e >= 0.99) break;
-        }
-        if (best2 < 0.0) for (long long g = gfloor; g <= gcap; g += 8) { const double e = eff_of(g); if (e > best2 + 1e-9) { best2 = e; g2 = g; } if (e >= 0.99) break; }
+        for (int pass = 0; pass < 2 && best2 < 0.0; ++pass)
+            for (long long g = gfloor; g <= gcap; g += 8) {
+                if (pass == 0 && per >= 16 && (g * per < 3 * cu_slots || g * per > 5 * cu_slots)) continue;
+                const double t = time_of(g);
+                if (best2 < 0.0 || t < best2 * (1.0 - 1e-9)) { best2 = t; g2 = g; }
+            }
         if (sw.lv_blocks >= 1) g2 = (sw.lv_blocks + 7) / 8 * 8;
         P.root_gx = (int)g2;
     }
@@ -444,7 +455,6 @@
     P.part_items = (size_t)K * P.root_gx;
     for (int level = 1; level < max_depth; ++level) {
         const int worst = 1 << (level - 1);
-        int G_first = 1;
         bool acc2 = nchunk == 2 && sw.mt_acc2;
         if (acc2) {
             const long long nb2 = ((long long)lv_slots(fmeta.data() + cmeta[0].first_feat, cmeta[0].nfeat, 0) + lv_slots(fmeta.data() + cmeta[1].first_feat, cmeta[1].nfeat, 0)) * 16;
@@ -476,19 +486,17 @@
                              (long long)T * win * rot_node_bytes <= hist_room;
             if (rot && sw.mt_T < 1) T = (int)std::max<long long>(T, T_rot);
             const int G = (K + T - 1) / T;
-            if (ch == 0) G_first = G;
             for (int s0 = 0; s0 < worst; s0 += win)
                 P.mt[level].push_back(MtLaunch{ch, s0, win, (ch == 0 && s0 == 0) ? 1 : 0, T, G, 0, acc2 ? 1 : 0, rot ? 1 : 0});
         }
         const long long gmin = std::max<long long>(1, (N + (1ll << 22) - 1) >> 22);
         const long long nwt = (N + MT_WT_ROWS - 1) / MT_WT_ROWS;
         const long long gx_lo = std::max<long long>(8, (gmin + 7) / 8 * 8), gx_hi = std::max<long long>(gx_lo, std::min<long long>(512, (nwt / (4 * (LV_THREADS / 64)) + 7) / 8 * 8));
-        long long gx = gx_lo; double best = -1.0;
+        long long gx = gx_lo; double best = 0.0;
         for (long long g = gx_lo; g <= gx_hi; g += 8) {
-            const long long tot = g * G_first, rounds = (tot + 255) / 256;
-            const double eff = (double)tot / (double)(rounds * 256) - 0.01 * (double)rounds;
-            if (eff > best + 1e-9) { best = eff; gx = g; }
-            if (tot >= 256 && (double)tot / (double)(rounds * 256) >= 0.97) break;
+            double t = 0.0;
+            for (const auto& L : P.mt[level]) t += pass_model_us((long long)L.G * g, (double)N / (double)g, std::min(L.T, K), mt_pass_cost(L.acc2 != 0, L.rot != 0));
+            if (g == gx_lo || t < best * (1.0 - 1e-9)) { best = t; gx = g; }
         }
         if (sw.mt_blocks >= 1) gx = (sw.mt_blocks + 7) / 8 * 8;
         P.mt_gx[level] = (int)gx;
@@ -795,12 +803,18 @@
     const int score_gx = (int)std::max<long long>(1, std::min<long long>((st.N + 1023) / 1024, (2048 + st.K - 1) / st.K));
     LevelTrace trace;
     int32_t h_err = 0;
+    std::vector<rg::RootLayout> h_root_lay; std::vector<rg::MtLayout> h_mt_lay; std::vector<int> mt_lay_keys;
+    DevBuf<rg::RootLayout> root_lay; DevBuf<rg::MtLayout> mt_lay;
+    static int mt_lay_key(const MtLaunch& L) { return L.ch * 4 + (L.acc2 ? 2 : 0) + (L.rot ? 1 : 0); }
+    int mt_lay_index(const MtLaunch& L) const {
+        for (size_t i = 0; i < mt_lay_keys.size(); ++i) if (mt_lay_keys[i] == mt_lay_key(L)) return (int)i;
+        return -1;
+    }
 
     explicit LevelGrower(FitState& st_) : st(st_), s(st_.s), root_feats(st_.F), trace(true, st_.K, st_.s) {
         using namespace rg;
         memset(&lc, 0, sizeof(lc)); memset(&lcj, 0, sizeof(lcj));
-        lc.lds_bytes = LV_LDS_BYTES;
-        if (st.sw.lv_lds >= 65536 && st.sw.lv_lds <= LV_LDS_BYTES) lc.lds_bytes = st.sw.lv_lds;
+        lc.lds_bytes = level_lds_bytes(st.sw);
         lc.nchunk = st.h.nchunk; lc.K = st.K; lc.F = st.F; lc.totbins = st.h.tc.totbins;
         lc.num_leaves = st.NL; lc.max_depth = st.p.max_depth; lc.min_data_in_leaf = st.p.min_data_in_leaf; lc.N = st.N; lc.NS = (st.N + 255) & ~255ll; lc.NG = lc.NS;
         lc.sib_local = (st.dp && comm_rank() == 0) ? 1 : 0;
@@ -827,12 +841,29 @@
                 hipLaunchKernelGGL(k_pack_joint, dim3((unsigned)((st.N + 255) / 256)), dim3(256), 0, s, st.bins.rec.p, (long long)st.N, st.F, jf.p, rec_j.p, st.tab.has_mult ? st.h.nchunk - 1 : -1);
                 part_j.alloc((size_t)st.K * lc.gx * vtotbins); red_j.alloc((size_t)st.K * vtotbins + (size_t)st.K * 128 );
                 lcj = lc; lcj.nchunk = 1; lcj.F = VF; lcj.totbins = vtotbins; lcj.max_built = 1;
+                h_root_lay.resize(1); root_layout_fill(h_root_lay[0], jp.vfm.data(), VF, lc.lds_bytes);
                 use_reduce = true; root_feats = VF;
                 HIPCHK(hipStreamSynchronize(s));
             }
         }
         if (st.tab.has_mult && st.h.nchunk == 2 && !joint_root)
             throw std::invalid_argument("a two-chunk table with row multiplicities needs the joint-bin root pass (its record carries the multiplicity); this feature set does not pack into 15 groups");
+        if (!joint_root) {
+            h_root_lay.resize(st.h.nchunk);
+            for (int ch = 0; ch < st.h.nchunk; ++ch) root_layout_fill(h_root_lay[ch], st.h.fmeta.data() + st.h.cmeta[ch].first_feat, st.h.cmeta[ch].nfeat, lc.lds_bytes);
+        }
+        root_lay.alloc(h_root_lay.size()); root_lay.upload(h_root_lay.data(), h_root_lay.size(), s);
+        lc.root_lay = root_lay.p; lcj.root_lay = root_lay.p;
+        for (int level = 1; level < st.p.max_depth; ++level) for (const auto& L : passes.mt[level]) if (mt_lay_index(L) < 0) {
+            const bool acc2 = L.acc2 != 0;
+            const ChunkMeta& cm = st.h.cmeta[L.ch];
+            const int nf_last = acc2 ? st.h.cmeta[1].nfeat : cm.nfeat;
+            const bool li_in_rec = nf_last <= 15 && !st.tab.has_mult;
+            mt_lay_keys.push_back(mt_lay_key(L)); h_mt_lay.emplace_back();
+            mt_layout_fill(h_mt_lay.back(), st.h.fmeta.data() + cm.first_feat, cm.nfeat, acc2 ? st.h.fmeta.data() + st.h.cmeta[1].first_feat : nullptr, acc2 ? st.h.cmeta[1].nfeat : 0,
+                           cm.wide_bins, L.rot != 0, mt_hist_bytes(lc.lds_bytes, acc2 ? MT_THREADS_ACC2 : LV_THREADS, acc2, acc2, !li_in_rec));
+        }
+        if (!h_mt_lay.empty()) { mt_lay.alloc(h_mt_lay.size()); mt_lay.upload(h_mt_lay.data(), h_mt_lay.size(), s); }
         if (st.sw.timing) {
             fprintf(stderr, "[rgbm] root: gx %d joint %d groups %d\n", lc.gx, joint_root ? 1 : 0, joint_root ? lcj.F : 0);
             for (int level = 1; level < st.p.max_depth; ++level) for (const auto& L : passes.mt[level])
@@ -896,6 +927,7 @@
             for (const MtLaunch& L : passes.mt[level]) {
                 LevelConst l1 = lp;
                 l1.mt_T = L.T; l1.mt_G = L.G; l1.mt_ch = L.ch; l1.mt_slot0 = L.slot0; l1.mt_nslots = L.nslots; l1.mt_route = L.route; l1.mt_sparse = st.sw.mt_sparse ? 1 : 0;
+                l1.mt_lay = mt_lay.p + mt_lay_index(L);
                 const bool acc2 = L.acc2 != 0;
                 const MtForm form{acc2 ? 2 : (st.h.nchunk <= 2 ? st.h.nchunk : 0), acc2 ? MT_THREADS_ACC2 : LV_THREADS, acc2, acc2, L.rot != 0};
                 st.timers.timed(false, [&]() {
@@ -2086,6 +2118,40 @@
     });
 }
 
+RGBM_EXPORT int rgbm_level_pass_plan(const int32_t* nbins, int32_t f, int64_t n_rows, int32_t k, int32_t max_depth, int32_t with_mult, double* out, int32_t out_len, int32_t* n_out) {
+    if (!nbins || !out || !n_out || f < 1 || f > 255 || n_rows < 1 || k < 1 || max_depth < 1 || max_depth > rg::LV_MAX_DEPTH) return fail(RGBM_ERR_ARG, "rgbm_level_pass_plan: bad argument");
+    return guarded([&]() {
+        using namespace rg;
+        const RunSwitches sw = read_switches();
+        std::vector<FeatMeta> fmeta(f); std::vector<ChunkMeta> cmeta((f + 15) / 16);
+        int totbins = 0;
+        for (int j = 0; j < f; ++j) {
+            if (nbins[j] < 1 || nbins[j] > 256) return fail(RGBM_ERR_ARG, "rgbm_level_pass_plan: a feature has 1..256 bins");
+            FeatMeta& m = fmeta[j]; memset(&m, 0, sizeof(m)); m.nbins = nbins[j]; m.V = nbins[j]; m.hoff = totbins; totbins += nbins[j];
+        }
+        for (size_t ch = 0; ch < cmeta.size(); ++ch) {
+            ChunkMeta& cm = cmeta[ch]; cm.first_feat = (int)ch * 16; cm.nfeat = std::min(16, f - (int)ch * 16); cm.fast_slots = 0; cm.wide_bins = 0;
+            for (int j = 0; j < cm.nfeat; ++j) { fmeta[ch * 16 + j].wide_off = cm.wide_bins; cm.wide_bins += fmeta[ch * 16 + j].nbins; }
+        }
+        const LevelPassPlan P = plan_level_passes(sw, fmeta, cmeta, n_rows, k, max_depth, with_mult != 0, level_lds_bytes(sw));
+        std::vector<double> v;
+        const long long root_wg = (long long)P.root_gx * k * (long long)cmeta.size();
+        v.insert(v.end(), {(double)P.root_gx, (double)P.part_items, 0.0, (double)root_wg, ROOT_PASS_COST.t_fix_us, (double)n_rows / P.root_gx * ROOT_PASS_COST.t_row_ns * 1e-3});
+        int nl = 0;
+        for (int level = 1; level < max_depth; ++level) for (const MtLaunch& L : P.mt[level]) {
+            const PassCost& c = mt_pass_cost(L.acc2 != 0, L.rot != 0);
+            v.insert(v.end(), {(double)level, (double)L.ch, (double)L.slot0, (double)L.nslots, (double)L.route, (double)L.T, (double)L.G, (double)L.gx, (double)L.acc2, (double)L.rot,
+                               c.t_fix_us, (double)n_rows / L.gx * (c.t_row_ns + std::min(L.T, (int)k) * c.t_pair_ns) * 1e-3});
+            ++nl;
+        }
+        v[2] = (double)nl;
+        *n_out = (int32_t)v.size();
+        if ((size_t)out_len < v.size()) return fail(RGBM_ERR_ARG, "rgbm_level_pass_plan: output too small");
+        std::copy(v.begin(), v.end(), out);
+        return RGBM_OK;
+    });
+}
+
 RGBM_EXPORT int rgbm_model_importance(const rgbm_model* m, int32_t type, double* out) {
     if (!m || !out) return fail(RGBM_ERR_ARG, "rgbm_model_importance: bad argument");
     for (int f = 0; f < m->F; ++f) out[f] = 0.0;
diff --git a/spark-data-repair-plugin_amd/csrc/rgbm_level.h b/spark-data-repair-plugin_amd/csrc/rgbm_level.h
--- a/spark-data-repair-plugin_amd/csrc/rgbm_level.h
+++ b/spark-data-repair-plugin_amd/csrc/rgbm_level.h
@@ -49,7 +49,11 @@
     uint32_t route1[256];
 };
 
+struct MtLayout;
+struct RootLayout;
 struct LevelConst {
+    const MtLayout* mt_lay;
+    const RootLayout* root_lay;
     int32_t gx;
     int32_t max_built;
     int32_t nchunk, K, F, totbins, num_leaves, max_depth, min_data_in_leaf, lds_bytes;
@@ -104,6 +108,57 @@
     const long long x = hd < room_h ? hd : room_h;
     const long long a = lds_bytes - fixed;
     return a < 2 * x ? a : 2 * x;
+}
+
+constexpr int MT_LAY_Q = LV_MAX_Q + 1;
+struct MtLayout {
+    uint32_t q_spn[MT_MAX_NODES + 4];
+    int32_t wide[32], hdelta[32];
+    int32_t fb[MT_LAY_Q][32];
+    int32_t sh[MT_LAY_Q][32];
+    uint8_t bin_feat[32 * 256];
+};
+struct RootLayout { int32_t q, spn, pad0, pad1; int32_t sh[16], fbase[16]; };
+
+inline void mt_layout_fill(MtLayout& L, const FeatMeta* fm, int nfeat, const FeatMeta* fm1 , int nfeat1, int wide_bins0,
+                           bool rot, long long avail ) {
+    memset(&L, 0, sizeof(L));
+    const bool acc2 = fm1 != nullptr;
+    auto spn_of = [&](int q) { return mt_slots(fm, nfeat, q, rot) + (acc2 ? mt_slots(fm1, nfeat1, q, rot) : 0) + mt_rot_dummy(rot); };
+    for (int tot = 0; tot < MT_MAX_NODES + 4; ++tot) {
+        int q = mt_max_q(rot);
+        while (q > 0 && (long long)tot * spn_of(q) * 16 > avail) --q;
+        L.q_spn[tot] = (uint32_t)q | (uint32_t)spn_of(q) << 8;
+    }
+    for (int q = 0; q < MT_LAY_Q; ++q) {
+        int o = 0;
+        for (int a = 0; a < (acc2 ? 2 : 1); ++a) {
+            const FeatMeta* fa = a == 0 ? fm : fm1;
+            const int na = a == 0 ? nfeat : nfeat1;
+            for (int j = 0; j < 16; ++j) {
+                int shj = 0, fbj = 0;
+                if (j < na) { shj = mt_shift(fa[j].nbins, q, rot); fbj = o; o += fa[j].nbins << shj; }
+                L.fb[q][a * 16 + j] = fbj; L.sh[q][a * 16 + j] = shj;
+            }
+        }
+    }
+    for (int q = 0; q < 32; ++q) L.wide[q] = 0x7FFFFFFF;
+    for (int a = 0; a < (acc2 ? 2 : 1); ++a) {
+        const FeatMeta* fa = a == 0 ? fm : fm1;
+        const int na = a == 0 ? nfeat : nfeat1;
+        for (int j = 0; j < na && j < 16; ++j) {
+            const int wide = (a == 0 ? 0 : wide_bins0) + fa[j].wide_off;
+            L.wide[a * 16 + j] = wide; L.hdelta[a * 16 + j] = fa[j].hoff - wide;
+            for (int b = 0; b < fa[j].nbins && wide + b < 32 * 256; ++b) L.bin_feat[wide + b] = (uint8_t)(a * 16 + j);
+        }
+    }
+}
+inline void root_layout_fill(RootLayout& L, const FeatMeta* fm, int nfeat, int lds_bytes) {
+    memset(&L, 0, sizeof(L));
+    int q = LV_MAX_Q;
+    while (q > 0 && (long long)lv_slots(fm, nfeat, q) * 16 + LV_ROOT_FIXED > lds_bytes) --q;
+    L.q = q;
+    for (int j = 0; j < 16 && j < nfeat; ++j) { L.sh[j] = lv_shift(fm[j].nbins, q); L.fbase[j] = L.spn; L.spn += fm[j].nbins << L.sh[j]; }
 }
 
 __global__ __launch_bounds__(64) void k_level_init(LvPlan* __restrict__ plan, SNode* __restrict__ nodes, int32_t* __restrict__ count,
@@ -145,17 +200,14 @@
     const ChunkMeta cm = cmeta[ch];
     const FeatMeta* fm = fmeta + cm.first_feat;
     const int tid = threadIdx.x, lane = tid & 63, nfeat = cm.nfeat;
-    int s = LV_MAX_Q;
-    while (s > 0 && (long long)lv_slots(fm, nfeat, s) * 16 + LV_ROOT_FIXED > c.lds_bytes) --s;
-    int sh[16], fbase[16], spn = 0;
-#pragma unroll
-    for (int j = 0; j < 16; ++j) {
-        if (j < nfeat) { sh[j] = lv_shift(fm[j].nbins, s); fbase[j] = spn; spn += fm[j].nbins << sh[j]; }
-        else { sh[j] = 0; fbase[j] = 0; }
-    }
+    const RootLayout* lay = c.root_lay + ch;
+    int sh[16], fbase[16];
+    const int spn = lay->spn;
+#pragma unroll
+    for (int j = 0; j < 16; ++j) { sh[j] = lay->sh[j]; fbase[j] = lay->fbase[j]; }
     unsigned long long* hist_g = reinterpret_cast<unsigned long long*>(smem);
     unsigned long long* hist_h = hist_g + spn;
-    for (int i = tid; i < 2 * spn; i += LV_THREADS) hist_g[i] = 0ull;
+    for (int i = tid; i < spn; i += LV_THREADS) reinterpret_cast<uint4*>(smem)[i] = make_uint4(0u, 0u, 0u, 0u);
     int cj[16], sh3[16];
 #pragma unroll
     for (int j = 0; j < 16; ++j) { sh3[j] = sh[j] + 3; cj[j] = (fbase[j] + (lane & ((1 << sh[j]) - 1))) * 8; }
@@ -219,9 +271,7 @@
     __syncthreads();
     HistBin* dst = part + (((long long)k * c.gx + bx) * c.max_built) * c.totbins;
     for (int j = 0; j < nfeat; ++j) {
-        const int shj = lv_shift(fm[j].nbins, s);
-        int fb = 0;
-        for (int q = 0; q < j; ++q) fb += fm[q].nbins << lv_shift(fm[q].nbins, s);
+        const int shj = lay->sh[j], fb = lay->fbase[j];
         for (int b = tid; b < fm[j].nbins; b += LV_THREADS) {
             long long tg = 0, th = 0;
             const unsigned long long* sg_ = hist_g + fb + (b << shj); const unsigned long long* sh_ = hist_h + fb + (b << shj);
@@ -265,8 +315,6 @@
     constexpr bool route = ROUTE;
     const ChunkMeta cm = cmeta[ch];
     const ChunkMeta cm1 = cmeta[ACC2 ? 1 : ch];
-    const FeatMeta* fm = fmeta + cm.first_feat;
-    const FeatMeta* fm1 = fmeta + cm1.first_feat;
     const int nfeat = cm.nfeat, nfeat1 = ACC2 ? cm1.nfeat : 0;
     const int wb = cm.wide_bins + (ACC2 ? cm1.wide_bins : 0);
     const bool li_in_rec = (ACC2 ? nfeat1 : nfeat) <= 15 && !c.has_mult;
@@ -295,7 +343,9 @@
     const long long avail = mt_hist_bytes(c.lds_bytes, THREADS, ACC2, SPEC, !li_in_rec);
     if (tid == 0 && ((long long)off > mt_fixed_bytes(THREADS, ACC2, SPEC, !li_in_rec) || (long long)off + MT_HD + avail / 2 > (long long)LV_LDS_TOTAL)) atomicOr(err_flag, 2);
 
+    const MtLayout* __restrict__ lay = c.mt_lay;
     if (tid < 64) {
+        const uint32_t qs0 = lay->q_spn[lane], qs1 = lay->q_spn[64 + lane], qs2 = lay->q_spn[128 + (lane & 3)];
         MtTree t; t.base = 0; t.nlev = 0; t.nb = 0; t.live = 0; t.child_first = 0; t.k = k0 + lane; t.slot0 = 0; t.rt_off = 0;
         if (lane < nk) {
             const LvPlan* pp = &plan[k0 + lane];
@@ -332,11 +382,10 @@
         tpk[pos] = make_uint2((uint32_t)t.base | (uint32_t)t.nlev << 8 | (uint32_t)(ntab > 0 ? ntab - 1 : 0) << 17 | (t.live && lane < nk ? 1u << 31 : 0u), (uint32_t)t.rt_off | (uint32_t)t.k << 16);
         if (lane < 2) tpk[64 + lane] = make_uint2(0u, 0u);
         if (SPARSE) xmask[lane] = 0ull;
+        const int tot = ok ? total : 0;
+        const uint32_t qs = (uint32_t)__shfl((int)(tot < 64 ? qs0 : (tot < 128 ? qs1 : qs2)), tot & 63);
         if (lane == 0) {
-            int s = mt_max_q(ROT);
-            const int tot = ok ? total : 0;
-            while (s > 0 && (long long)tot * (mt_slots(fm, nfeat, s, ROT) + (ACC2 ? mt_slots(fm1, nfeat1, s, ROT) : 0) + mt_rot_dummy(ROT)) * 16 > avail) --s;
-            const int spn0 = mt_slots(fm, nfeat, s, ROT) + (ACC2 ? mt_slots(fm1, nfeat1, s, ROT) : 0) + mt_rot_dummy(ROT);
+            const int s = (int)(qs & 0xFFu), spn0 = (int)(qs >> 8);
             if ((long long)tot * spn0 * 16 > avail) atomicOr(err_flag, 2);
             scal[0] = tot; scal[1] = s; scal[2] = spn0; scal[3] = ((ok && livem != 0ull) ? 1 : 0) | nkd_ << 8 | (nkd_ + nks_) << 16;
         }
@@ -346,11 +395,11 @@
     const int total = __builtin_amdgcn_readfirstlane(scal[0]), s = __builtin_amdgcn_readfirstlane(scal[1]), spn = __builtin_amdgcn_readfirstlane(scal[2]);
     if (!route && total == 0) return;
     const int nkd = __builtin_amdgcn_readfirstlane((scal[3] >> 8) & 0xFF), nke = __builtin_amdgcn_readfirstlane((scal[3] >> 16) & 0xFF);
-    for (int kk = 0; kk < nk; ++kk) {
+    for (int kk = __builtin_amdgcn_readfirstlane(wave); kk < nk; kk += WAVES) {
         const MtTree t = ti[kk];
         const LvPlan* pp = &plan[t.k];
         const int ntab_k = (route ? (t.live ? t.child_first : 0) : t.nlev) + 1;
-        for (int i = tid; i < ntab_k; i += THREADS) {
+        for (int i = lane; i < ntab_k; i += 64) {
             const int n = route ? i : t.base + i;
             uint2 e;
             if (route) {
@@ -380,35 +429,33 @@
             rt[t.rt_off + i] = e;
         }
         const uint2 sc_k = make_uint2((uint32_t)__double2hiint(fxs[t.k].sg), (uint32_t)__double2hiint(fxs[t.k].sh));
-        for (int i = tid; i < t.nb; i += THREADS) { nd_tree[t.slot0 + i] = (uint8_t)kk; nd_sc[t.slot0 + i] = sc_k; }
+        for (int i = lane; i < t.nb; i += 64) { nd_tree[t.slot0 + i] = (uint8_t)kk; nd_sc[t.slot0 + i] = sc_k; }
     }
     for (int i = tid; i < total * MT_CNT_REP; i += THREADS) cnt[i] = 0;
     if (tid < 48) rsync[tid] = 0u;
     unsigned long long* hist_h = hist_g + MT_HD / 8;
-    for (int i = tid; i < total * spn; i += THREADS) { hist_g[i] = 0ull; hist_h[i] = 0ull; }
+    {
+        uint4* zg = reinterpret_cast<uint4*>(hist_g); uint4* zh = reinterpret_cast<uint4*>(hist_h);
+        const int n16 = (total * spn + 1) >> 1;
+        for (int i = tid; i < n16; i += THREADS) { zg[i] = make_uint4(0u, 0u, 0u, 0u); zh[i] = make_uint4(0u, 0u, 0u, 0u); }
+    }
     unsigned long long sh3p[NACC];
     int cj[NACC][16];
     {
-        int o = 0;
+        const int32_t* __restrict__ fb_s = lay->fb[s]; const int32_t* __restrict__ sh_s = lay->sh[s];
 #pragma unroll
         for (int a = 0; a < NACC; ++a) {
-            const FeatMeta* fa = a == 0 ? fm : fm1;
-            const int na = a == 0 ? nfeat : nfeat1;
             unsigned long long pk = 0ull;
 #pragma unroll
             for (int j = 0; j < 16; ++j) {
-                int shj = 0, fb = 0;
-                if (j < na) { shj = mt_shift(fa[j].nbins, s, ROT); fb = o; o += fa[j].nbins << shj; }
+                const int shj = sh_s[a * 16 + j], fb = fb_s[a * 16 + j];
                 pk |= (unsigned long long)(shj + 3) << (4 * j); cj[a][j] = (fb + (lane & ((1 << shj) - 1))) * 8;
-                if (tid == 0) {
-                    const int q = a * 16 + j;
-                    const int wide = (a == 0 ? 0 : cm.wide_bins) + (j < na ? fa[j].wide_off : 0);
-                    ftab[q] = j < na ? wide : 0x7FFFFFFF; ftab[32 + q] = fb; ftab[64 + q] = shj; ftab[96 + q] = j < na ? fa[j].hoff - wide : 0;
-                }
             }
             sh3p[a] = (unsigned long long)(unsigned)__builtin_amdgcn_readfirstlane((int)(unsigned)pk) |
                       (unsigned long long)(unsigned)__builtin_amdgcn_readfirstlane((int)(unsigned)(pk >> 32)) << 32;
         }
+        if (tid < 128) { const int q = tid & 31, r = tid >> 5; ftab[tid] = r == 0 ? lay->wide[q] : (r == 1 ? fb_s[q] : (r == 2 ? sh_s[q] : lay->hdelta[q])); }
+        if (tid == 0) { const unsigned long long la = (unsigned long long)reinterpret_cast<uintptr_t>(lay->bin_feat); rsync[48] = (uint32_t)la; rsync[49] = (uint32_t)(la >> 32); }
     }
     constexpr int hdelta = MT_HD / 8;
     __syncthreads();
@@ -798,13 +845,12 @@
 #undef RS_STORE
     else while (r_cnt > 0) run_batch(r_cnt < 64 ? r_cnt : 64);
     __syncthreads();
-    constexpr int NQ = NACC * 16;
+    const uint8_t* __restrict__ bin_feat = reinterpret_cast<const uint8_t*>((uintptr_t)((unsigned long long)(uint32_t)__builtin_amdgcn_readfirstlane((int)rsync[48]) |
+                                                                                      (unsigned long long)(uint32_t)__builtin_amdgcn_readfirstlane((int)rsync[49]) << 32));
     for (int i = tid; i < total * wb; i += THREADS) {
         const int ln = i / wb, b = i - ln * wb;
         const MtTree t = ti[nd_tree[ln]];
-        int j = 0;
-#pragma unroll
-        for (int q = 1; q < NQ; ++q) j += (b >= ftab[q]) ? 1 : 0;
+        const int j = bin_feat[b];
         const int shb = ftab[64 + j], s0 = ftab[32 + j] + ((b - ftab[j]) << shb);
         long long tg = 0, th = 0;
         const unsigned long long* sg_ = hist_g + (size_t)ln * spn + s0; const unsigned long long* sh_ = hist_h + (size_t)ln * spn + s0;
diff --git a/spark-data-repair-plugin_amd/repair/_native.py b/spark-data-repair-plugin_amd/repair/_native.py
--- a/spark-data-repair-plugin_amd/repair/_native.py
+++ b/spark-data-repair-plugin_amd/repair/_native.py
@@ -86,7 +86,7 @@
                      "rgbm_table_read_row_multiplicity", "rgbm_table_detect_dc", "rgbm_table_detect_row_bits",
                      "rgbm_table_kmeans_assign", "rgbm_table_kmeans_read", "rgbm_lof_1d", "rgbm_table_column_stats"):
             getattr(l, name).restype = C.c_int
-        for name in ("rgbm_table_distinct_view_info", "rgbm_distinct_view_eligible"):
+        for name in ("rgbm_table_distinct_view_info", "rgbm_distinct_view_eligible", "rgbm_level_pass_plan"):
             if hasattr(l, name):
                 getattr(l, name).restype = C.c_int
         l.rgbm_local_group_free.restype = None
@@ -113,7 +113,7 @@
     "rgbm_table_fd_map", "rgbm_table_rule_fill", "rgbm_nearest_values", "rgbm_table_detect_cells",
     "rgbm_table_distinct_rows", "rgbm_table_read_row_multiplicity", "rgbm_table_detect_dc", "rgbm_table_detect_row_bits", "rgbm_model_predict_form",
     "rgbm_table_kmeans_assign", "rgbm_table_kmeans_read", "rgbm_table_distinct_view_info", "rgbm_distinct_view_eligible",
-    "rgbm_table_column_stats",
+    "rgbm_table_column_stats", "rgbm_level_pass_plan",
 ]
 EXPORTED_SYMBOLS_WITH_DIGITS = ["rgbm_lof_1d"]
 
@@ -362,6 +362,20 @@
     _fields_ = [("table", C.c_void_p), ("target_col", C.c_int32), ("n_features", C.c_int32), ("feat_cols", C.POINTER(C.c_int32)),
                 ("y_value", C.POINTER(C.c_double)), ("class_weight", C.POINTER(C.c_double)), ("params", C.POINTER(RgbmParams)),
                 ("valid_table", C.c_void_p), ("valid_label_out", C.POINTER(C.c_int32)), ("valid_value_out", C.POINTER(C.c_double))]
+
+
+def level_pass_plan(nbins, rows, K, max_depth=7, with_mult=False):
+    nb = _i32(nbins)
+    out = np.zeros(6 + 12 * 4096, np.float64)
+    n = C.c_int32(0)
+    _check(lib().rgbm_level_pass_plan(_p(nb, C.c_int32), C.c_int32(len(nb)), C.c_int64(rows), C.c_int32(K), C.c_int32(max_depth), C.c_int32(1 if with_mult else 0),
+                                      _p(out, C.c_double), C.c_int32(len(out)), C.byref(n)), "rgbm_level_pass_plan")
+    keys = ("level", "ch", "slot0", "nslots", "route", "T", "G", "gx", "acc2", "rot")
+    launches = []
+    for i in range(int(out[2])):
+        v = out[6 + 12 * i: 18 + 12 * i]
+        launches.append(dict({k: int(x) for k, x in zip(keys, v)}, t_fix_us=float(v[10]), t_rows_us=float(v[11])))
+    return dict(root_gx=int(out[0]), part_items=int(out[1]), root_workgroups=int(out[3]), root_t_fix_us=float(out[4]), root_t_rows_us=float(out[5]), launches=launches)
 
 
 def distinct_view_eligible(rows, f, table_has_mult=False, min_rows=0, **params):
```

New measurement: 1.852 million (median of 6 runs). 1.09x the previous value.
